# sandyresearch/chipmunk

Measured on AMD Instinct MI355X. Metric: DiT denoise steps/sec at fixed sparsity, higher is better.
Workload: dtype bf16

## Files before the change

### chipmunk_amd/_native.py

```python
from __future__ import annotations

import ctypes
import os

_HERE = os.path.dirname(os.path.abspath(__file__))
LIB_PATH = os.environ.get("CHIPMUNK_HIP_LIB") or os.path.join(_HERE, "lib", "libchipmunk_hip.so")

SYMBOLS = [
    "chipmunk_last_error", "chipmunk_abi_version", "chipmunk_set_option", "chipmunk_set_random_seed",
    "chipmunk_csp_attn", "chipmunk_csp_attn_out", "chipmunk_csp_128_attn", "chipmunk_dense_attn", "chipmunk_dense_colsum_attn",
    "chipmunk_csp_mlp_mm1", "chipmunk_csp_mlp_mm1_scatter", "chipmunk_csp_mlp_mm1_fp8", "chipmunk_csp_mlp_mm2_and_scatter_add", "chipmunk_csp_scatter_add", "chipmunk_csp_mlp_mm2",
    "chipmunk_csp_mlp_mm1_ragged", "chipmunk_csp_mlp_mm1_scatter_ragged", "chipmunk_csp_mlp_mm1_fp8_ragged", "chipmunk_csp_mlp_mm2_ragged",
    "chipmunk_csp_mlp_mm2_and_scatter_add_ragged", "chipmunk_csp_scatter_add_ragged", "chipmunk_block_mean_ragged", "chipmunk_transpose16_pitched",
    "chipmunk_csp_mlp_mm1_batched", "chipmunk_csp_mlp_mm1_scatter_batched", "chipmunk_csp_mlp_mm1_fp8_batched", "chipmunk_csp_mlp_mm2_batched",
    "chipmunk_csp_mlp_mm2_and_scatter_add_batched", "chipmunk_csp_scatter_add_batched",
    "chipmunk_topk_indices", "chipmunk_topk_delta_indices", "chipmunk_topk_mask", "chipmunk_mask_to_indices", "chipmunk_mask_to_sorted_indices", "chipmunk_packed_mask_to_indices", "chipmunk_mask_row_counts", "chipmunk_mask_to_ragged_indices", "chipmunk_copy_indices",
    "chipmunk_bitpack", "chipmunk_bitunpack", "chipmunk_transpose16", "chipmunk_block_mean", "chipmunk_quantize_fp8", "chipmunk_gather_rows", "chipmunk_qkv_split_norm", "chipmunk_split_heads_rownorm", "chipmunk_dense_colsum_topk_mask", "chipmunk_dense_attn_strided", "chipmunk_csp_attn_out_ragged", "chipmunk_compact_indices", "chipmunk_residual_ln_modulate", "chipmunk_dense_colsum_attn_strided", "chipmunk_dense_colsum_topk_mask_strided", "chipmunk_release_scratch", "chipmunk_big_scratch_fallbacks",
    "chipmunk_host_alloc", "chipmunk_host_free", "chipmunk_copy_d2h_async", "chipmunk_copy_h2d_async", "chipmunk_host_bytes",
]

_lib = None


def lib() -> ctypes.CDLL:
    global _lib
    if _lib is None:
        if not os.path.exists(LIB_PATH):
            raise ImportError(
                f"{LIB_PATH} is missing: build it with `python -m chipmunk_amd.build` (hipcc --offload-arch=gfx950). "
                "chipmunk_amd has no CPU fallback.")
        _lib = ctypes.CDLL(LIB_PATH)
        _lib.chipmunk_last_error.restype = ctypes.c_char_p
        _lib.chipmunk_abi_version.restype = ctypes.c_int
        for item in filter(None, os.environ.get("CHIPMUNK_AMD_OPTIONS", "").split(",")):
            name, _, val = item.partition("=")
            if _lib.chipmunk_set_option(name.strip().encode(), int(val)) != 0:
                raise ValueError(f"CHIPMUNK_AMD_OPTIONS: {_lib.chipmunk_last_error().decode()}")
    return _lib


def last_error() -> str:
    return lib().chipmunk_last_error().decode()


def check(rc: int, what: str) -> None:
    if rc != 0:
        raise RuntimeError(f"{what}: {last_error()}")


def set_option(name: str, value: int) -> None:
    check(lib().chipmunk_set_option(name.encode(), int(value)), "chipmunk_set_option")


def manual_seed(seed: int) -> None:
    check(lib().chipmunk_set_random_seed(ctypes.c_uint64(int(seed) & 0xFFFFFFFFFFFFFFFF)), "chipmunk_set_random_seed")


class HostBuffer:

    def __init__(self, numel: int, dtype) -> None:
        import torch
        self.dtype = dtype
        self._numel = int(numel)
        self._itemsize = torch.empty(0, dtype=dtype).element_size()
        self.nbytes = self._numel * self._itemsize
        p = ctypes.c_void_p()
        check(lib().chipmunk_host_alloc(ctypes.c_size_t(max(self.nbytes, 1)), ctypes.byref(p)), "chipmunk_host_alloc")
        self.ptr = p.value

    def numel(self) -> int:
        return self._numel

    def element_size(self) -> int:
        return self._itemsize

    def is_pinned(self) -> bool:
        return True

    def free(self) -> None:
        if getattr(self, "ptr", None):
            lib().chipmunk_host_free(ctypes.c_void_p(self.ptr))
            self.ptr = None

    def __del__(self):
        try:
            self.free()
        except Exception:
            pass


def copy_d2h_async(host_ptr: int, dev_ptr: int, nbytes: int, stream: int) -> None:
    check(lib().chipmunk_copy_d2h_async(ctypes.c_void_p(host_ptr), ctypes.c_void_p(dev_ptr), ctypes.c_size_t(nbytes), ctypes.c_void_p(stream)),
          "chipmunk_copy_d2h_async")


def copy_h2d_async(dev_ptr: int, host_ptr: int, nbytes: int, stream: int) -> None:
    check(lib().chipmunk_copy_h2d_async(ctypes.c_void_p(dev_ptr), ctypes.c_void_p(host_ptr), ctypes.c_size_t(nbytes), ctypes.c_void_p(stream)),
          "chipmunk_copy_h2d_async")


def host_bytes() -> int:
    f = lib().chipmunk_host_bytes
    f.restype = ctypes.c_size_t
    return int(f())
```

### chipmunk_amd/csrc/attn.hip

```cpp
#include "common.h"
#include "attn_params.h"
#include <type_traits>

namespace {

constexpr int QG = 192;
constexpr int QW = 48;
constexpr int KVT = 32;
constexpr int NST = 4;
constexpr int KRING = 8;
constexpr int HD = 128;
constexpr int TILE_BYTES = KVT * HD * 2;
constexpr float SCALE_LOG2E = 0.08838834764f * 1.44269504089f;
constexpr int NSTV = NST + 1;
constexpr int KEY_RING_OFF = (NST + NSTV) * TILE_BYTES;
constexpr int CS_OFF = KEY_RING_OFF + KRING * 256;
constexpr int ATTN_LDS_BYTES = CS_OFF + 2 * 2 * 4 * KVT * 4;

__device__ __forceinline__ f32x4 mfma16(bf16x8 a, bf16x8 b, f32x4 c) {
    return __builtin_amdgcn_mfma_f32_16x16x32_bf16(a, b, c, 0, 0, 0);
}

#ifdef ATTN_PROF
__device__ unsigned long long g_attn_prof[8 * 8];
// ... 1101 lines not shown
    contiguous_strides(p.qs, H, Nq), contiguous_strides(p.os, H, Nq);
    contiguous_strides(p.ks, H, Nk), contiguous_strides(p.vs, H, Nk);
    p.indices = indices, p.counts = counts;
    p.B = B, p.H = H, p.Nq = Nq, p.Nk = Nk, p.G = (Nq + QG - 1) / QG, p.idx_stride = idx_stride;
    p.o_scale = 1.f;
    return launch_attn<true, false, false>(p, (hipStream_t)stream);
}

static int output_strides(int64_t os[3], const int64_t *o_strides, int H, int Nq) {
    if (!o_strides) {
        contiguous_strides(os, H, Nq);
        return CHIPMUNK_OK;
    }
    for (int i = 0; i < 3; ++i) os[i] = o_strides[i];
    return check_strides(o_strides, "o");
}

extern "C" int chipmunk_dense_attn_strided(const void *q, const void *k, const void *v, const int64_t q_strides[3],
                                           const int64_t k_strides[3], const int64_t v_strides[3], void *o,
                                           const int64_t *o_strides, float *l, int B, int H, int Nq, int Nk, void *stream) {
    if (int e = check_common(q, k, v, o, B, H, Nq, Nk)) return e;
    CM_CHECK(l != nullptr, "dense_attn: l output missing");
    if (int e = check_strides(q_strides, "q")) return e;
    if (int e = check_strides(k_strides, "k")) return e;
    if (int e = check_strides(v_strides, "v")) return e;
    AttnParams p = {};
    p.q = (const uint16_t *)q, p.k = (const uint16_t *)k, p.v = (const uint16_t *)v, p.o = (uint16_t *)o;
    for (int i = 0; i < 3; ++i) p.qs[i] = q_strides[i], p.ks[i] = k_strides[i], p.vs[i] = v_strides[i];
    if (int e = output_strides(p.os, o_strides, H, Nq)) return e;
    p.l_out = l;
    p.B = B, p.H = H, p.Nq = Nq, p.Nk = Nk, p.G = (Nq + QG - 1) / QG;
    p.o_scale = 1.f;
    if (use_dense64(B, H, Nq, Nk)) {
        CM_CHECK((int64_t)Nk * p.ks[2] * 2 < (1ll << 32) && (int64_t)Nk * p.vs[2] * 2 < (1ll << 32),
                 "attention: one head's K or V spans more than 4 GiB (32-bit DMA offsets)");
        return chipmunk_dense64_launch(q, k, v, o, l, p.qs, p.ks, p.vs, p.os, B, H, Nq, Nk, (hipStream_t)stream);
    }
    return launch_attn<false, false, true>(p, (hipStream_t)stream);
}

extern "C" int chipmunk_dense_attn(const void *q, const void *k, const void *v, const int64_t q_strides[3],
                                   const int64_t k_strides[3], const int64_t v_strides[3], void *o, float *l, int B,
                                   int H, int Nq, int Nk, void *stream) {
    return chipmunk_dense_attn_strided(q, k, v, q_strides, k_strides, v_strides, o, nullptr, l, B, H, Nq, Nk, stream);
}

extern "C" int chipmunk_dense_colsum_attn_strided(const void *q, const void *k, const void *v, const int64_t q_strides[3],
                                                  const int64_t k_strides[3], const int64_t v_strides[3], const float *pin,
                                                  void *o, const int64_t *o_strides, void *cs, float *l, int B, int H, int Nq,
                                                  int Nk, int cs_stride, void *stream) {
    if (int e = check_common(q, k, v, o, B, H, Nq, Nk)) return e;
    CM_CHECK(l && cs && pin, "dense_colsum_attn: p / cs / l missing");
    CM_CHECK(cs_stride >= Nk, "dense_colsum_attn: cs row stride %d < Nk %d", cs_stride, Nk);
    if (int e = check_strides(q_strides, "q")) return e;
    if (int e = check_strides(k_strides, "k")) return e;
    if (int e = check_strides(v_strides, "v")) return e;
    AttnParams p = {};
    p.q = (const uint16_t *)q, p.k = (const uint16_t *)k, p.v = (const uint16_t *)v, p.o = (uint16_t *)o;
    for (int i = 0; i < 3; ++i) p.qs[i] = q_strides[i], p.ks[i] = k_strides[i], p.vs[i] = v_strides[i];
    if (int e = output_strides(p.os, o_strides, H, Nq)) return e;
    p.l_out = l, p.p_in = pin, p.cs = (uint16_t *)cs, p.cs_stride = cs_stride;
    p.B = B, p.H = H, p.Nq = Nq, p.Nk = Nk, p.G = (Nq + QG - 1) / QG;
    p.o_scale = 1.f;
    hipStream_t st = (hipStream_t)stream;
    int rc;
    if (chipmunk_get_option("attn_fused_colsum") == 5) {
        if (use_colsum64(B, H, Nq, Nk)) return chipmunk_colsum64_launch(p, st);
        return launch_attn<false, false, false, true>(p, st);
    }
    if (use_dense64(B, H, Nq, Nk)) {
        CM_CHECK((int64_t)Nk * p.ks[2] * 2 < (1ll << 32) && (int64_t)Nk * p.vs[2] * 2 < (1ll << 32),
                 "attention: one head's K or V spans more than 4 GiB (32-bit DMA offsets)");
        if (chipmunk_get_option("attn_fused_colsum") != 2) {
            int hc = H;
            uint16_t *part = nullptr;
            const int hc_min = chipmunk_get_option("attn_fused_colsum") == 4 ? 1 : 0;
            if (hc_min) hc = 1;
            for (; hc >= 1; hc /= 2) {
                part = (uint16_t *)chipmunk_big_scratch(st, chipmunk_colsum_part_bytes(hc == H ? B : 1, hc, Nq, Nk));
                if (part) break;
            }
            if (part && hc == H) return chipmunk_dense64_colsum_launch(p, part, st);
            if (part) {
                for (int b = 0; b < B; ++b)
                    for (int h0 = 0; h0 < H; h0 += hc) {
                        AttnParams c = p;
                        const int hn = H - h0 < hc ? H - h0 : hc;
                        const int64_t bh0 = (int64_t)b * H + h0;
                        c.q += b * p.qs[0] + h0 * p.qs[1], c.k += b * p.ks[0] + h0 * p.ks[1], c.v += b * p.vs[0] + h0 * p.vs[1];
                        c.o += b * p.os[0] + h0 * p.os[1];
                        c.l_out += bh0 * Nq, c.p_in += bh0 * Nq, c.cs += bh0 * p.G * (int64_t)cs_stride;
                        c.B = 1, c.H = hn;
                        if (int e = chipmunk_dense64_colsum_launch(c, part, st)) return e;
                    }
                return CHIPMUNK_OK;
            }
        }
        rc = chipmunk_dense64_launch(q, k, v, o, l, p.qs, p.ks, p.vs, p.os, B, H, Nq, Nk, st);
    } else {
        rc = launch_attn<false, false, true>(p, st);
    }
    if (rc != CHIPMUNK_OK) return rc;
    if (use_colsum64(B, H, Nq, Nk)) return chipmunk_colsum64_launch(p, st);
    return launch_attn<false, false, false, true>(p, st);
}

extern "C" int chipmunk_dense_colsum_attn(const void *q, const void *k, const void *v, const int64_t q_strides[3],
                                          const int64_t k_strides[3], const int64_t v_strides[3], const float *pin,
                                          void *o, void *cs, float *l, int B, int H, int Nq, int Nk, int cs_stride,
                                          void *stream) {
    return chipmunk_dense_colsum_attn_strided(q, k, v, q_strides, k_strides, v_strides, pin, o, nullptr, cs, l, B, H, Nq, Nk,
                                              cs_stride, stream);
}

extern "C" int chipmunk_dense_colsum_topk_mask_strided(const void *q, const void *k, const void *v, const int64_t q_strides[3],
                                               const int64_t k_strides[3], const int64_t v_strides[3], const float *pin, void *o,
                                               const int64_t *o_strides, float *l, int B, int H, int Nq, int Nk, const void *static_mask,
                                               int64_t static_stride, int static_rows, const void *group_flags, void *mask,
                                               int topk, double random_amount, void *stream) {
    if (int e = check_common(q, k, v, o, B, H, Nq, Nk)) return e;
    CM_CHECK(l && pin && mask, "dense_colsum_topk_mask: p / l / mask missing");
    if (int e = check_strides(q_strides, "q")) return e;
    if (int e = check_strides(k_strides, "k")) return e;
    if (int e = check_strides(v_strides, "v")) return e;
    hipStream_t st = (hipStream_t)stream;
    if (!use_dense64(B, H, Nq, Nk) || chipmunk_get_option("attn_fused_colsum") == 2 || (Nk & 3) || Nk > CHIPMUNK_TOPK_MASK_MAX_N)
        return CHIPMUNK_ERR_UNSUPPORTED;
    AttnParams p = {};
    p.q = (const uint16_t *)q, p.k = (const uint16_t *)k, p.v = (const uint16_t *)v, p.o = (uint16_t *)o;
    for (int i = 0; i < 3; ++i) p.qs[i] = q_strides[i], p.ks[i] = k_strides[i], p.vs[i] = v_strides[i];
    CM_CHECK((int64_t)Nk * p.ks[2] * 2 < (1ll << 32) && (int64_t)Nk * p.vs[2] * 2 < (1ll << 32),
             "attention: one head's K or V spans more than 4 GiB (32-bit DMA offsets)");
    if (int e = output_strides(p.os, o_strides, H, Nq)) return e;
    p.l_out = l, p.p_in = pin, p.cs = nullptr, p.cs_stride = 0;
    p.B = B, p.H = H, p.Nq = Nq, p.Nk = Nk, p.G = (Nq + QG - 1) / QG;
    p.o_scale = 1.f;
    uint16_t *part = (uint16_t *)chipmunk_big_scratch(st, chipmunk_colsum_part_bytes(B, H, Nq, Nk));
    if (!part) return CHIPMUNK_ERR_UNSUPPORTED;
    if (int e = chipmunk_dense64_colsum_launch(p, part, st)) return e;
    const int nrb = ((Nq + 255) / 256) * 2;
    return chipmunk_topk_mask_parts(part, chipmunk_colsum_part_stride(Nk), nrb, p.G, Nq, static_mask, static_stride, static_rows, group_flags, mask, B * H * p.G, Nk,
                                    topk, random_amount, st);
}

extern "C" int chipmunk_dense_colsum_topk_mask(const void *q, const void *k, const void *v, const int64_t q_strides[3],
                                               const int64_t k_strides[3], const int64_t v_strides[3], const float *pin, void *o,
                                               float *l, int B, int H, int Nq, int Nk, const void *static_mask,
                                               int64_t static_stride, int static_rows, const void *group_flags, void *mask,
                                               int topk, double random_amount, void *stream) {
    return chipmunk_dense_colsum_topk_mask_strided(q, k, v, q_strides, k_strides, v_strides, pin, o, nullptr, l, B, H, Nq, Nk,
                                                   static_mask, static_stride, static_rows, group_flags, mask, topk, random_amount,
                                                   stream);
}
```

### chipmunk_amd/csrc/attn_params.h

```cpp
#pragma once
#include <stdint.h>
#include <hip/hip_runtime.h>

struct AttnParams {
    const uint16_t *q, *k, *v;
    uint16_t *o;
    const uint16_t *o_in;
    int64_t qs[3], ks[3], vs[3], os[3];
    const int32_t *indices, *counts;
    const int64_t *idx_off;
    float *l_out;
    const float *p_in;
    uint16_t *cs;
    int cs_stride;
    int B, H, Nq, Nk, G, idx_stride;
    float o_scale;
    int split_full, nsplit;
    float *ws;
    int32_t *tickets;
    const int32_t *plan;
    int xcd_chunks;
    const float *kmax;
    uint16_t *cs_part;
    int cs_pstride;
    int probe;
};


int chipmunk_csp64_launch(const AttnParams &p, int inplace, int grid, hipStream_t stream);
int chipmunk_dense64_colsum_launch(const AttnParams &p, uint16_t *part, hipStream_t stream);
int chipmunk_topk_mask_parts(const uint16_t *part, int part_stride, int nrb, int groups_per_bh, int Nq, const void *static_mask, int64_t static_stride,
                             int static_rows, const void *group_flags, void *mask, int rows, int n, int k, double random_amount,
                             hipStream_t stream);
size_t chipmunk_colsum_part_bytes(int B, int H, int Nq, int Nk);
int chipmunk_colsum_part_stride(int Nk);
int chipmunk_colsum64_launch(const AttnParams &p, hipStream_t stream);
int chipmunk_csp96_launch(const AttnParams &p, int inplace, int grid, hipStream_t stream);
const float *chipmunk_knorm_max(const uint16_t *k, const int64_t ks[3], int B, int H, int Nk, hipStream_t stream);

__host__ __device__ inline int colsum_part_rows(int j, int nwg, int &r0, int &r1) {
    const int a = (3 * j) >> 2, w0 = 3 * j - 4 * a;
    r0 = 2 * a + (w0 ? 1 : 0);
    r1 = 2 * (a + 1);
    return (w0 >= 2 && a + 1 < nwg) ? 2 : 1;
}

struct IndexRow {
    const int32_t *ptr;
    int width;
};
__device__ __forceinline__ IndexRow index_row(const AttnParams &p, int64_t item) {
    if (p.idx_off) {
        const int64_t o = p.idx_off[item];
        return {p.indices + o, (int)(p.idx_off[item + 1] - o)};
    }
    return {p.indices + item * p.idx_stride, p.idx_stride};
}
```

### chipmunk_amd/csrc/indexed_io.hip

```cpp
#include "common.h"
#include "attn_params.h"

namespace {

__device__ __forceinline__ uint32_t wave_incl_scan(uint32_t x) {
    x += (uint32_t)__builtin_amdgcn_update_dpp(0, (int)x, 0x111, 0xf, 0xf, true);
    x += (uint32_t)__builtin_amdgcn_update_dpp(0, (int)x, 0x112, 0xf, 0xf, true);
    x += (uint32_t)__builtin_amdgcn_update_dpp(0, (int)x, 0x114, 0xf, 0xf, true);
    x += (uint32_t)__builtin_amdgcn_update_dpp(0, (int)x, 0x118, 0xf, 0xf, true);
    x += (uint32_t)__builtin_amdgcn_update_dpp(0, (int)x, 0x142, 0xa, 0xf, false);
    x += (uint32_t)__builtin_amdgcn_update_dpp(0, (int)x, 0x143, 0xc, 0xf, false);
    return x;
}
struct M2IParams {
    const uint8_t *mask;
    int32_t *indices;
    int32_t *counts;
    int n, pad_n, multiple_of;
    const int64_t *offsets;
};

template <bool PACKED, bool SORTED = false, bool RAGGED = false>
__global__ __launch_bounds__(256) void mask_to_indices_kernel(const M2IParams p) {
    extern __shared__ __attribute__((aligned(16))) unsigned char smem[];
// ... 385 lines not shown
        base += tot[256];
        __syncthreads();
    }
    const int kept = base;
    const int mod = kept % p.multiple_of;
    const int pad = mod == 0 ? 0 : p.multiple_of - mod;
    if (tid == 0) p.counts[row] = kept + pad;
    if (pad > 0) {
        int pbase = 0;
        const int slot = compact_slot(my_last_invalid != -1, lane, w, wave_tot, pbase);
        if (slot >= 0 && slot < pad) {
            out[kept + slot] = my_last_invalid;
            if constexpr (DELTA) xc[my_last_invalid] = x[my_last_invalid];
        }
    }
}

template <typename T>
__global__ __launch_bounds__(256) void copy_indices_kernel(const T *src, T *dst, const int32_t *inds,
                                                           const int32_t *counts, int M, int R, int F) {
    const int64_t grow = blockIdx.x;
    const int64_t b = grow / ((int64_t)M * R);
    const int base_m = (int)((grow % ((int64_t)M * R)) / R);
    const int cnt = counts[b * M + base_m];
    const int32_t *ii = inds + (b * M + base_m) * (int64_t)F;
    for (int c = threadIdx.x; c < cnt; c += 256) {
        const int col = ii[c];
        dst[grow * F + col] = src[grow * F + col];
    }
}

__global__ __launch_bounds__(256) void bitpack_kernel(const uint8_t *mask, uint8_t *packed, int64_t n) {
    const int64_t nb = (n + 7) >> 3;
    for (int64_t i = (int64_t)blockIdx.x * 256 + threadIdx.x; i < nb; i += (int64_t)gridDim.x * 256) {
        uint8_t byte = 0;
        if (i * 8 + 8 <= n && ((((uintptr_t)mask) & 7) == 0)) {
            unsigned long long v = *(const unsigned long long *)(mask + i * 8);
#pragma unroll
            for (int j = 0; j < 8; ++j) byte |= (uint8_t)((((v >> (8 * j)) & 0xffull) != 0) << j);
        } else {
            for (int j = 0; j < 8 && i * 8 + j < n; ++j) byte |= (uint8_t)((mask[i * 8 + j] != 0) << j);
        }
        packed[i] = byte;
    }
}
__global__ __launch_bounds__(256) void bitunpack_kernel(const uint8_t *packed, uint8_t *mask, int64_t n) {
    const int64_t nb = (n + 7) >> 3;
    for (int64_t i = (int64_t)blockIdx.x * 256 + threadIdx.x; i < nb; i += (int64_t)gridDim.x * 256) {
        const uint8_t byte = packed[i];
        if (i * 8 + 8 <= n && ((((uintptr_t)mask) & 7) == 0)) {
            unsigned long long v = 0;
#pragma unroll
            for (int j = 0; j < 8; ++j) v |= (unsigned long long)((byte >> j) & 1u) << (8 * j);
            *(unsigned long long *)(mask + i * 8) = v;
        } else {
            for (int j = 0; j < 8 && i * 8 + j < n; ++j) mask[i * 8 + j] = (byte >> j) & 1u;
        }
    }
}

__global__ __launch_bounds__(256) void transpose16_kernel(const uint16_t *src, uint16_t *dst, int R, int C, int ld) {
    __shared__ __attribute__((aligned(16))) uint16_t tile[64][72];
    const int64_t boff = (int64_t)blockIdx.z * R * C;
    const int r0 = blockIdx.y * 64, c0 = blockIdx.x * 64;
    const int tid = threadIdx.x;
#pragma unroll
    for (int i = 0; i < 2; ++i) {
        const int item = i * 256 + tid, r = item >> 3, ch = item & 7;
        u32x4 v = {0u, 0u, 0u, 0u};
        if (r0 + r < R && c0 + ch * 8 + 8 <= C) v = *(const u32x4 *)(src + boff + (int64_t)(r0 + r) * C + c0 + ch * 8);
        else if (r0 + r < R)
            for (int e = 0; e < 8; ++e)
                if (c0 + ch * 8 + e < C) {
                    const uint32_t x = src[boff + (int64_t)(r0 + r) * C + c0 + ch * 8 + e];
                    v[e >> 1] |= x << (16 * (e & 1));
                }
#pragma unroll
        for (int e = 0; e < 4; ++e) {
            tile[ch * 8 + 2 * e][r] = (uint16_t)(v[e] & 0xffffu);
            tile[ch * 8 + 2 * e + 1][r] = (uint16_t)(v[e] >> 16);
        }
    }
    __syncthreads();
#pragma unroll
    for (int i = 0; i < 2; ++i) {
        const int item = i * 256 + tid, c = item >> 3, ch = item & 7;
        if (c0 + c >= C) continue;
        uint16_t *d = dst + (int64_t)blockIdx.z * C * ld + (int64_t)(c0 + c) * ld + r0 + ch * 8;
        if (r0 + ch * 8 + 8 <= ld && ((ld & 7) == 0)) *(u32x4 *)d = *(const u32x4 *)&tile[c][ch * 8];
        else
            for (int e = 0; e < 8; ++e)
                if (r0 + ch * 8 + e < ld) d[e] = tile[c][ch * 8 + e];
    }
}

__global__ __launch_bounds__(256) void compact_indices_kernel(const int32_t *indices, int64_t idx_stride, const int32_t *counts,
                                                             const int64_t *offsets, int32_t *flat) {
    const int64_t r = blockIdx.x;
    const int32_t *src = indices + r * idx_stride;
    const int64_t o = offsets[r];
    int32_t *dst = flat + o;
    const int width = (int)(offsets[r + 1] - o);
    int c = counts[r];
    c = c < 0 ? 0 : (c < width ? c : width);
    c = c < idx_stride ? c : (int)idx_stride;
    if ((((uintptr_t)src | (uintptr_t)dst) & 15) == 0) {
        const int c4 = c >> 2;
        for (int i = threadIdx.x; i < c4; i += 256) ((u32x4 *)dst)[i] = ((const u32x4 *)src)[i];
        for (int i = (c4 << 2) + threadIdx.x; i < c; i += 256) dst[i] = src[i];
    } else {
        for (int i = threadIdx.x; i < c; i += 256) dst[i] = src[i];
    }
    for (int i = c + threadIdx.x; i < width; i += 256) dst[i] = 0;
}

size_t m2i_lds_bytes(int n, bool sorted) {
    const int NI = (n + 31) >> 5, NB = (NI + 63) >> 6;
    if (sorted) return (size_t)NB * 64 * 4 + (size_t)(NB + 1) * 4 + 16;
    return (size_t)NB * 64 * 4 + (size_t)32 * NB * 8 + (size_t)32 * NB * 4 + 33 * 4 + 16;
}

template <bool PACKED, bool SORTED = false, bool RAGGED = false>
int launch_m2i(const void *mask, int32_t *indices, int32_t *counts, int64_t rows, int n, int pad_n, int multiple_of,
               void *stream, const int64_t *offsets = nullptr) {
    CM_CHECK(mask && indices && (RAGGED ? (const void *)offsets : (const void *)counts), "mask_to_indices: null pointer");
    CM_CHECK(rows >= 0 && n > 0 && pad_n >= n && multiple_of > 0, "mask_to_indices: bad sizes rows=%lld n=%d pad_n=%d multiple_of=%d",
             (long long)rows, n, pad_n, multiple_of);
    CM_CHECK(rows < (1ll << 31), "mask_to_indices: too many rows");
    if (PACKED) CM_CHECK(n % 8 == 0, "packed_mask_to_indices: n must be a multiple of 8 (got %d)", n);
    const size_t lds = m2i_lds_bytes(n, SORTED);
    CM_CHECK(lds <= 160 * 1024, "mask_to_indices: row length %d needs %zu B of LDS (> 160 KiB)", n, lds);
    if (rows == 0) return CHIPMUNK_OK;
    auto kern = mask_to_indices_kernel<PACKED, SORTED, RAGGED>;
    if (lds > 64 * 1024) (void)hipFuncSetAttribute((const void *)kern, hipFuncAttributeMaxDynamicSharedMemorySize, (int)lds);
    M2IParams p = {(const uint8_t *)mask, indices, counts, n, pad_n, multiple_of, offsets};
    hipLaunchKernelGGL(kern, dim3((unsigned)rows), dim3(256), lds, (hipStream_t)stream, p);
    CM_LAUNCH_CHECK();
    return CHIPMUNK_OK;
}


struct TopkMaskParams {
    const uint16_t *cs;
    const uint8_t *stat;
    const uint8_t *groups;
    uint8_t *mask;
    int64_t cs_stride, stat_stride;
    int rows, n, k, stat_rows;
    float random_amount;
    uint32_t salt;
    const uint16_t *parts;
    int64_t pstride;
    int nrb, ngroups, nq;
};

__device__ __forceinline__ uint32_t bf16_key(uint32_t u) {
    return (u & 0x8000u) ? (~u & 0xffffu) : (u | 0x8000u);
}

template <int KPT, bool ALIGNED, bool PARTS = false>
__global__ __launch_bounds__(1024) void topk_mask_kernel(const TopkMaskParams p) {
    constexpr int NV = KPT / 4;
    __shared__ int wave_cnt[16];
    const int tid = threadIdx.x, lane = tid & 63, w = tid >> 6;
    const int row = blockIdx.x;
    const int n = p.n;
    const uint16_t *x = nullptr;
    int prow = 1;
    int64_t row1 = 0;
    if constexpr (PARTS) {
        const int bh = row / p.ngroups, g = row - bh * p.ngroups;
        int r0, r1;
        prow = colsum_part_rows(g, p.nrb / 2, r0, r1);
        x = p.parts + ((int64_t)bh * p.nrb + r0) * p.pstride;
        row1 = (int64_t)(r1 - r0) * p.pstride;
    } else {
        x = p.cs + (int64_t)row * p.cs_stride;
    }
    const uint32_t lane_off8 = 8u * (uint32_t)tid;
    const uint32_t lane_off4 = 4u * (uint32_t)tid;
    uint32_t key[NV][2];
    constexpr int LB = NV % 10 == 0 ? 10 : (NV % 8 == 0 ? 8 : (NV % 6 == 0 ? 6 : 4));
    static_assert(NV % LB == 0, "NV must split into whole load batches");
#pragma unroll
    for (int j0 = 0; j0 < NV; j0 += LB) {
        uint32_t raw[LB][2];
#pragma unroll
        for (int jj = 0; jj < LB; ++jj) {
            const int c = 4 * tid + 4096 * (j0 + jj);
            uint32_t v0 = 0xffffffffu, v1 = 0xffffffffu;
            if constexpr (ALIGNED) {
                if (c < n) {
                    const u32x2 v = *(const u32x2 *)((const unsigned char *)(x + 4096 * (j0 + jj)) + lane_off8);
                    v0 = v[0], v1 = v[1];
                    if constexpr (PARTS) {
                        if (prow == 2) {
                            float a0 = __uint_as_float(v0 << 16), a1 = __uint_as_float(v0 & 0xffff0000u);
                            float a2 = __uint_as_float(v1 << 16), a3 = __uint_as_float(v1 & 0xffff0000u);
                            const u32x2 y = *(const u32x2 *)((const unsigned char *)(x + row1 + 4096 * (j0 + jj)) + lane_off8);
                            a0 += __uint_as_float(y[0] << 16), a1 += __uint_as_float(y[0] & 0xffff0000u);
                            a2 += __uint_as_float(y[1] << 16), a3 += __uint_as_float(y[1] & 0xffff0000u);
                            v0 = pack_bf16x2(a0, a1), v1 = pack_bf16x2(a2, a3);
                        }
                    }
                }
            } else if (c < n) {
                v0 = v1 = 0;
#pragma unroll
                for (int e = 0; e < 4; ++e) {
                    const uint32_t u = c + e < n ? x[c + e] : 0xffffu;
                    if (e < 2) v0 |= u << (16 * e);
                    else v1 |= u << (16 * (e - 2));
                }
            }
            raw[jj][0] = v0, raw[jj][1] = v1;
        }
#pragma unroll
        for (int jj = 0; jj < LB; ++jj) {
            key[j0 + jj][0] = bf16_key(raw[jj][0] & 0xffffu) | (bf16_key(raw[jj][0] >> 16) << 16);
            key[j0 + jj][1] = bf16_key(raw[jj][1] & 0xffffu) | (bf16_key(raw[jj][1] >> 16) << 16);
        }
        __builtin_amdgcn_sched_barrier(0);
    }
    auto block_count = [&](int mine) {
#pragma unroll
        for (int d = 32; d > 0; d >>= 1) mine += __shfl_xor(mine, d);
        if (lane == 0) wave_cnt[w] = mine;
        __syncthreads();
        int t = 0;
#pragma unroll
        for (int i = 0; i < 16; ++i) t += wave_cnt[i];
        __syncthreads();
        return t;
    };
    const bool active = p.groups == nullptr || p.groups[row] != 0;
    const int k = p.k < n ? p.k : n;
    uint32_t thr = 0x10000u;
    int ties_to_take = 0;
    if (active && k > 0) {
        uint32_t res = 0;
        for (int bit = 15; bit >= 0; --bit) {
            const uint32_t cand = res | (1u << bit);
            const uint32_t cm1 = (cand - 1u) | ((cand - 1u) << 16);
            const uint32_t one2 = 0x00010001u;
            uint32_t cnt2 = 0;
#pragma unroll
            for (int j = 0; j < NV; ++j)
#pragma unroll
                for (int h = 0; h < 2; ++h) {
                    uint32_t d;
                    asm volatile("v_pk_sub_u16 %0, %1, %2 clamp\n\tv_pk_min_u16 %0, %0, %3" : "=&v"(d) : "v"(key[j][h]), "v"(cm1), "v"(one2));
                    asm volatile("v_pk_add_u16 %0, %0, %1" : "+v"(cnt2) : "v"(d));
                }
            const int mine = (int)(cnt2 & 0xffffu) + (int)(cnt2 >> 16);
            if (block_count(mine) >= k) res = cand;
        }
        thr = res;
        int gt = 0;
#pragma unroll
        for (int j = 0; j < NV; ++j)
#pragma unroll
            for (int h = 0; h < 2; ++h) {
                uint32_t kw = key[j][h];
                asm volatile("" : "+v"(kw));
                gt += ((kw & 0xffffu) > thr ? 1 : 0) + ((kw >> 16) > thr ? 1 : 0);
            }
        ties_to_take = k - block_count(gt);
    }
    int my_ties = 0;
    if (ties_to_take > 0) {
#pragma unroll
        for (int j = 0; j < NV; ++j)
#pragma unroll
            for (int h = 0; h < 2; ++h) {
                uint32_t kw = key[j][h];
                asm volatile("" : "+v"(kw));
                my_ties += ((kw & 0xffffu) == thr ? 1 : 0) + ((kw >> 16) == thr ? 1 : 0);
            }
    }
    int tie_budget = 0;
    {
        int incl = my_ties;
#pragma unroll
        for (int d = 1; d < 64; d <<= 1) {
            const int o = __shfl_up(incl, d);
            if (lane >= d) incl += o;
        }
        if (lane == 63) wave_cnt[w] = incl;
        __syncthreads();
        int before = incl - my_ties;
#pragma unroll
        for (int i = 0; i < 16; ++i) before += i < w ? wave_cnt[i] : 0;
        __syncthreads();
        tie_budget = ties_to_take - before;
    }
    uint8_t *out = p.mask + (int64_t)row * n;
    const uint8_t *st = p.stat ? p.stat + (int64_t)(row % p.stat_rows) * p.stat_stride : nullptr;
    const bool rnd = active && p.random_amount > 0.f;
    auto combined4 = [&](int c0, uint32_t &v0, uint32_t &v1) {
        const u32x2 v = *(const u32x2 *)(x + c0);
        v0 = v[0], v1 = v[1];
        if constexpr (PARTS) {
            float a0 = __uint_as_float(v0 << 16), a1 = __uint_as_float(v0 & 0xffff0000u);
            float a2 = __uint_as_float(v1 << 16), a3 = __uint_as_float(v1 & 0xffff0000u);
            if (prow == 2) {
                const u32x2 y = *(const u32x2 *)(x + row1 + c0);
                a0 += __uint_as_float(y[0] << 16), a1 += __uint_as_float(y[0] & 0xffff0000u);
                a2 += __uint_as_float(y[1] << 16), a3 += __uint_as_float(y[1] & 0xffff0000u);
            }
            v0 = pack_bf16x2(a0, a1), v1 = pack_bf16x2(a2, a3);
        }
    };
    uint32_t first = x[0];
    if constexpr (PARTS) {
        uint32_t f0, f1;
        combined4(0, f0, f1);
        first = f0 & 0xffffu;
    }
    const uint32_t salt = p.salt ^ (first * 0x27D4EB2Fu);
    const int nsteps = (n + 4095) / 4096;
    auto emit = [&](auto keyed, int c, uint32_t v0, uint32_t v1, uint32_t sb) {
        uint32_t bytes = 0;
        if constexpr (decltype(keyed)::value) asm volatile("" : "+v"(v0), "+v"(v1));
#pragma unroll
        for (int e = 0; e < 4; ++e) {
            const uint32_t half = ((e < 2 ? v0 : v1) >> (16 * (e & 1))) & 0xffffu;
            const uint32_t kv = decltype(keyed)::value ? half : bf16_key(half);
            bool keep = kv > thr;
            const bool tie = kv == thr && tie_budget > 0 && c + e < n;
            tie_budget -= tie ? 1 : 0;
            keep = keep || tie;
            if (rnd && !keep) keep = hash_uniform(row, c + e, salt) < p.random_amount;
            keep = keep || ((sb >> (8 * e)) & 0xffu) != 0;
            bytes |= (keep ? 1u : 0u) << (8 * e);
        }
        if constexpr (ALIGNED) {
            *(uint32_t *)(out + c) = bytes;
        } else {
#pragma unroll
            for (int e = 0; e < 4; ++e)
                if (c + e < n) out[c + e] = (uint8_t)(bytes >> (8 * e));
        }
    };
    if constexpr (ALIGNED) {
        constexpr int OB = 5;
#pragma unroll
        for (int j0 = 0; j0 < NV; j0 += OB) {
            uint32_t sbv[OB];
#pragma unroll
            for (int jj = 0; jj < OB; ++jj) {
                const int c = 4 * tid + 4096 * (j0 + jj);
                sbv[jj] = (j0 + jj < NV && st && c < n) ? *(const uint32_t *)(st + c) : 0u;
            }
            __builtin_amdgcn_sched_barrier(0);
#pragma unroll
            for (int jj = 0; jj < OB; ++jj) {
                if constexpr (true) {
                    const int c = 4 * tid + 4096 * (j0 + jj);
                    if (j0 + jj < NV && c < n) emit(std::integral_constant<int, 1>{}, c, key[(j0 + jj) < NV ? (j0 + jj) : 0][0], key[(j0 + jj) < NV ? (j0 + jj) : 0][1], sbv[jj]);
                    asm volatile("" ::: "memory");
                }
            }
            __builtin_amdgcn_sched_barrier(0);
        }
    } else {
        for (int j = 0; j < nsteps; ++j) {
            const int c = 4 * tid + 4096 * j;
            if (c >= n) break;
            uint32_t v0 = 0, v1 = 0, sb = 0;
#pragma unroll
            for (int e = 0; e < 4; ++e) {
                const uint32_t u = c + e < n ? x[c + e] : 0xffffu;
                if (e < 2) v0 |= u << (16 * e);
                else v1 |= u << (16 * (e - 2));
                if (st && c + e < n) sb |= (uint32_t)st[c + e] << (8 * e);
            }
            emit(std::integral_constant<int, 0>{}, c, v0, v1, sb);
        }
    }
}

__device__ __forceinline__ uint32_t bf16_key2(uint32_t u) {
    uint32_t s;
    const uint32_t fifteen2 = 0x000f000fu;
    asm("v_pk_ashrrev_i16 %0, %1, %2" : "=v"(s) : "v"(fifteen2), "v"(u));
    return u ^ (s | 0x80008000u);
}

template <bool ALIGNED, bool PARTS>
__global__ __launch_bounds__(1024) void topk_mask_stream_kernel(const TopkMaskParams p) {
    __shared__ int wave_cnt[16];
    const int tid = threadIdx.x, lane = tid & 63, w = tid >> 6;
    const int row = blockIdx.x;
    const int n = p.n;
    const uint16_t *x = nullptr;
    int prow = 1;
    int64_t row1 = 0;
    if constexpr (PARTS) {
        const int bh = row / p.ngroups, g = row - bh * p.ngroups;
        int r0, r1;
        prow = colsum_part_rows(g, p.nrb / 2, r0, r1);
        x = p.parts + ((int64_t)bh * p.nrb + r0) * p.pstride;
        row1 = (int64_t)(r1 - r0) * p.pstride;
    } else {
        x = p.cs + (int64_t)row * p.cs_stride;
    }
    const uint32_t lane_off8 = 8u * (uint32_t)tid;
    const int nsteps = (n + 4095) / 4096;
    const bool active = p.groups == nullptr || p.groups[row] != 0;
    const int k = p.k < n ? p.k : n;
    const bool select = active && k > 0;
    const bool rnd = active && p.random_amount > 0.f;

    auto combined4 = [&](int c0, uint32_t &v0, uint32_t &v1) {
        const u32x2 v = *(const u32x2 *)(x + c0);
        v0 = v[0], v1 = v[1];
        if constexpr (PARTS) {
            if (prow == 2) {
                float a0 = __uint_as_float(v0 << 16), a1 = __uint_as_float(v0 & 0xffff0000u);
                float a2 = __uint_as_float(v1 << 16), a3 = __uint_as_float(v1 & 0xffff0000u);
                const u32x2 y = *(const u32x2 *)(x + row1 + c0);
                a0 += __uint_as_float(y[0] << 16), a1 += __uint_as_float(y[0] & 0xffff0000u);
                a2 += __uint_as_float(y[1] << 16), a3 += __uint_as_float(y[1] & 0xffff0000u);
                v0 = pack_bf16x2(a0, a1), v1 = pack_bf16x2(a2, a3);
            }
        }
    };
    uint32_t first = 0;
    if (rnd) {
        first = x[0];
        if constexpr (PARTS) {
            uint32_t f0, f1;
            combined4(0, f0, f1);
            first = f0 & 0xffffu;
        }
    }
    const uint32_t salt = p.salt ^ (first * 0x27D4EB2Fu);
    if constexpr (PARTS) {
        __syncthreads();
        if (select) {
            uint16_t *xk = const_cast<uint16_t *>(x);
            for (int j = 0; j < nsteps; ++j) {
                const int c = 4 * tid + 4096 * j;
                if (c < n) {
                    uint32_t v0, v1;
                    combined4(c, v0, v1);
                    u32x2 kk = {bf16_key2(v0), bf16_key2(v1)};
                    *(u32x2 *)(xk + c) = kk;
                }
            }
        }
        __syncthreads();
    }
    auto load_raw = [&](int j, uint32_t &v0, uint32_t &v1) {
        const int c = 4 * tid + 4096 * j;
        if constexpr (ALIGNED) {
            v0 = v1 = PARTS ? 0u : 0xffffffffu;
            if (c < n) {
                const u32x2 v = *(const u32x2 *)((const unsigned char *)(x + 4096 * j) + lane_off8);
                v0 = v[0], v1 = v[1];
            }
        } else {
            v0 = v1 = 0xffffffffu;
            if (c < n) {
                v0 = v1 = 0;
#pragma unroll
                for (int e = 0; e < 4; ++e) {
                    const uint32_t u = c + e < n ? x[c + e] : 0xffffu;
                    if (e < 2) v0 |= u << (16 * e);
                    else v1 |= u << (16 * (e - 2));
                }
            }
        }
    };
    auto to_keys = [&](uint32_t &v0, uint32_t &v1) {
        if constexpr (!PARTS) v0 = bf16_key2(v0), v1 = bf16_key2(v1);
    };
    auto block_count = [&](int mine) {
#pragma unroll
        for (int d = 32; d > 0; d >>= 1) mine += __shfl_xor(mine, d);
        if (lane == 0) wave_cnt[w] = mine;
        __syncthreads();
        int t = 0;
#pragma unroll
        for (int i = 0; i < 16; ++i) t += wave_cnt[i];
        __syncthreads();
        return t;
    };
    constexpr int U = ALIGNED ? 8 : 2;
    uint32_t thr = 0x10000u;
    int ties_to_take = 0, my_ties = 0;
    if (select) {
        uint32_t res = 0;
        for (int bit = 15; bit >= 0; --bit) {
            const uint32_t cand = res | (1u << bit);
            const uint32_t cm1 = (cand - 1u) | ((cand - 1u) << 16);
            const uint32_t one2 = 0x00010001u;
            uint32_t cnt2 = 0;
            for (int j0 = 0; j0 < nsteps; j0 += U) {
                uint32_t kw[U][2];
#pragma unroll
                for (int jj = 0; jj < U; ++jj) load_raw(j0 + jj, kw[jj][0], kw[jj][1]);
#pragma unroll
                for (int jj = 0; jj < U; ++jj) {
                    to_keys(kw[jj][0], kw[jj][1]);
#pragma unroll
                    for (int h = 0; h < 2; ++h) {
                        uint32_t d;
                        asm volatile("v_pk_sub_u16 %0, %1, %2 clamp\n\tv_pk_min_u16 %0, %0, %3" : "=&v"(d) : "v"(kw[jj][h]), "v"(cm1), "v"(one2));
                        asm volatile("v_pk_add_u16 %0, %0, %1" : "+v"(cnt2) : "v"(d));
                    }
                }
            }
            const int mine = (int)(cnt2 & 0xffffu) + (int)(cnt2 >> 16);
            if (block_count(mine) >= k) res = cand;
        }
        thr = res;
        int gt = 0;
        for (int j0 = 0; j0 < nsteps; j0 += U) {
            uint32_t kw[U][2];
#pragma unroll
            for (int jj = 0; jj < U; ++jj) load_raw(j0 + jj, kw[jj][0], kw[jj][1]);
#pragma unroll
            for (int jj = 0; jj < U; ++jj) {
                to_keys(kw[jj][0], kw[jj][1]);
#pragma unroll
                for (int h = 0; h < 2; ++h) {
                    const uint32_t lo = kw[jj][h] & 0xffffu, hi = kw[jj][h] >> 16;
                    gt += (lo > thr ? 1 : 0) + (hi > thr ? 1 : 0);
                    my_ties += (lo == thr ? 1 : 0) + (hi == thr ? 1 : 0);
                }
            }
        }
        ties_to_take = k - block_count(gt);
    }
    int tie_budget = 0;
    {
        int incl = my_ties;
#pragma unroll
        for (int d = 1; d < 64; d <<= 1) {
            const int o = __shfl_up(incl, d);
            if (lane >= d) incl += o;
        }
        if (lane == 63) wave_cnt[w] = incl;
        __syncthreads();
        int before = incl - my_ties;
#pragma unroll
        for (int i = 0; i < 16; ++i) before += i < w ? wave_cnt[i] : 0;
        __syncthreads();
        tie_budget = ties_to_take - before;
    }
    uint8_t *out = p.mask + (int64_t)row * n;
    const uint8_t *st = p.stat ? p.stat + (int64_t)(row % p.stat_rows) * p.stat_stride : nullptr;
    for (int j0 = 0; j0 < nsteps; j0 += U) {
        uint32_t kw[U][2], sbv[U];
#pragma unroll
        for (int jj = 0; jj < U; ++jj) {
            const int c = 4 * tid + 4096 * (j0 + jj);
            kw[jj][0] = kw[jj][1] = 0;
            if (select) load_raw(j0 + jj, kw[jj][0], kw[jj][1]);
            sbv[jj] = 0;
            if constexpr (ALIGNED) {
                if (st && c < n) sbv[jj] = *(const uint32_t *)(st + c);
            } else if (st) {
#pragma unroll
                for (int e = 0; e < 4; ++e)
                    if (c + e < n) sbv[jj] |= (uint32_t)st[c + e] << (8 * e);
            }
        }
#pragma unroll
        for (int jj = 0; jj < U; ++jj) {
            const int c = 4 * tid + 4096 * (j0 + jj);
            if (c >= n) continue;
            if (select) to_keys(kw[jj][0], kw[jj][1]);
            uint32_t bytes = 0;
#pragma unroll
            for (int e = 0; e < 4; ++e) {
                const uint32_t kv = (kw[jj][e >> 1] >> (16 * (e & 1))) & 0xffffu;
                bool keep = kv > thr;
                const bool tie = kv == thr && tie_budget > 0 && c + e < n;
                tie_budget -= tie ? 1 : 0;
                keep = keep || tie;
                if (rnd && !keep) keep = hash_uniform(row, c + e, salt) < p.random_amount;
                keep = keep || ((sbv[jj] >> (8 * e)) & 0xffu) != 0;
                bytes |= (keep ? 1u : 0u) << (8 * e);
            }
            if constexpr (ALIGNED) {
                *(uint32_t *)(out + c) = bytes;
            } else {
#pragma unroll
                for (int e = 0; e < 4; ++e)
                    if (c + e < n) out[c + e] = (uint8_t)(bytes >> (8 * e));
            }
        }
    }
}

}

extern "C" int chipmunk_mask_to_indices(const void *mask, int32_t *indices, int32_t *counts, int64_t rows, int n,
                                        int pad_n, int multiple_of, void *stream) {
    return launch_m2i<false>(mask, indices, counts, rows, n, pad_n, multiple_of, stream);
}

extern "C" int chipmunk_packed_mask_to_indices(const void *packed, int32_t *indices, int32_t *counts, int64_t rows,
                                               int n, int pad_n, int multiple_of, void *stream) {
    return launch_m2i<true>(packed, indices, counts, rows, n, pad_n, multiple_of, stream);
}

static int launch_topk(const void *activation, void *cache, int dtype, int32_t *indices, int32_t *counts, int rows,
                       int cols, double sparsity_amount, int multiple_of, double random_amount, void *stream) {
    CM_CHECK(activation && indices && counts, "topk_indices: null pointer");
    CM_CHECK(rows >= 0 && cols >= 1024, "topk_indices: rows >= 0 and cols >= 1024 required (the quantile is taken over the first 1024 columns); got rows=%d cols=%d", rows, cols);
    CM_CHECK(multiple_of > 0, "topk_indices: multiple_of must be positive");
    CM_CHECK(sparsity_amount >= 0.0 && sparsity_amount <= 1.0, "topk_indices: sparsity_amount must be in [0,1]");
    if (rows == 0) return CHIPMUNK_OK;
    TopkParams p = {activation, cache, indices, counts, rows, cols, multiple_of, (float)sparsity_amount, (float)random_amount,
                    random_amount > 0.0 ? chipmunk_next_random_salt() : 0u};
    hipStream_t s = (hipStream_t)stream;
#define LAUNCH_TOPK(T)                                                                                           \
    do {                                                                                                         \
        if (cache) hipLaunchKernelGGL((topk_indices_kernel<T, true>), dim3(rows), dim3(1024), 0, s, p);          \
        else hipLaunchKernelGGL((topk_indices_kernel<T, false>), dim3(rows), dim3(1024), 0, s, p);               \
    } while (0)
    switch (dtype) {
        case CHIPMUNK_DTYPE_BF16: LAUNCH_TOPK(uint16_t); break;
        case CHIPMUNK_DTYPE_FP16: LAUNCH_TOPK(_Float16); break;
        case CHIPMUNK_DTYPE_FP32: LAUNCH_TOPK(float); break;
        default: CM_CHECK(false, "topk_indices: unsupported dtype code %d", dtype);
    }
#undef LAUNCH_TOPK
    CM_LAUNCH_CHECK();
    return CHIPMUNK_OK;
}

extern "C" int chipmunk_mask_to_sorted_indices(const void *mask, int packed, int32_t *indices, int32_t *counts,
                                               int64_t rows, int n, int pad_n, int multiple_of, void *stream) {
    return packed ? launch_m2i<true, true>(mask, indices, counts, rows, n, pad_n, multiple_of, stream)
                  : launch_m2i<false, true>(mask, indices, counts, rows, n, pad_n, multiple_of, stream);
}

extern "C" int chipmunk_mask_row_counts(const void *mask, int packed, int32_t *counts, int64_t *lengths, int64_t rows, int n,
                                        int pad_n, int multiple_of, void *stream) {
    CM_CHECK(mask && counts && lengths, "mask_row_counts: null pointer");
    CM_CHECK(rows >= 0 && n > 0 && pad_n >= n && multiple_of > 0, "mask_row_counts: bad sizes rows=%lld n=%d pad_n=%d multiple_of=%d",
             (long long)rows, n, pad_n, multiple_of);
    CM_CHECK(rows < (1ll << 31), "mask_row_counts: too many rows");
    CM_CHECK(!packed || n % 8 == 0, "mask_row_counts: n must be a multiple of 8 for a packed mask (got %d)", n);
    const size_t lds = m2i_lds_bytes(n, true);
    CM_CHECK(lds <= 160 * 1024, "mask_to_indices: row length %d needs %zu B of LDS (> 160 KiB)", n, lds);
    if (rows == 0) return CHIPMUNK_OK;
    RowCountParams p = {(const uint8_t *)mask, counts, lengths, rows, n, pad_n, multiple_of};
    const dim3 grid((unsigned)((rows + 3) / 4));
    if (packed) hipLaunchKernelGGL(mask_row_counts_kernel<true>, grid, dim3(256), 0, (hipStream_t)stream, p);
    else hipLaunchKernelGGL(mask_row_counts_kernel<false>, grid, dim3(256), 0, (hipStream_t)stream, p);
    CM_LAUNCH_CHECK();
    return CHIPMUNK_OK;
}

extern "C" int chipmunk_mask_to_ragged_indices(const void *mask, int packed, int sorted, const int64_t *offsets, int32_t *flat,
                                               int64_t rows, int n, int multiple_of, void *stream) {
    if (packed) return sorted ? launch_m2i<true, true, true>(mask, flat, nullptr, rows, n, n, multiple_of, stream, offsets)
                              : launch_m2i<true, false, true>(mask, flat, nullptr, rows, n, n, multiple_of, stream, offsets);
    return sorted ? launch_m2i<false, true, true>(mask, flat, nullptr, rows, n, n, multiple_of, stream, offsets)
                  : launch_m2i<false, false, true>(mask, flat, nullptr, rows, n, n, multiple_of, stream, offsets);
}

extern "C" int chipmunk_topk_indices(const void *activation, int dtype, int32_t *indices, int32_t *counts, int rows,
                                     int cols, double sparsity_amount, int multiple_of, double random_amount,
                                     void *stream) {
    return launch_topk(activation, nullptr, dtype, indices, counts, rows, cols, sparsity_amount, multiple_of,
                       random_amount, stream);
}

extern "C" int chipmunk_topk_delta_indices(const void *activation, void *cache, int dtype, int32_t *indices,
                                           int32_t *counts, int rows, int cols, double sparsity_amount,
                                           int multiple_of, double random_amount, void *stream) {
    CM_CHECK(cache != nullptr, "topk_delta_indices: cache missing");
    return launch_topk(activation, cache, dtype, indices, counts, rows, cols, sparsity_amount, multiple_of,
                       random_amount, stream);
}

extern "C" int chipmunk_copy_indices(const void *src, void *dst, const int32_t *inds, const int32_t *counts, int B,
                                     int M, int R, int F, int elem_size, void *stream) {
    CM_CHECK(src && dst && inds && counts, "copy_indices: null pointer");
    CM_CHECK(B >= 0 && M > 0 && R > 0 && F > 0, "copy_indices: bad sizes");
    CM_CHECK(elem_size == 2 || elem_size == 4, "copy_indices: element size must be 2 or 4 bytes (got %d)", elem_size);
    const int64_t rows = (int64_t)B * M * R;
    if (rows == 0) return CHIPMUNK_OK;
    CM_CHECK(rows < (1ll << 31), "copy_indices: too many rows");
    hipStream_t s = (hipStream_t)stream;
    if (elem_size == 2)
        hipLaunchKernelGGL(copy_indices_kernel<uint16_t>, dim3((unsigned)rows), dim3(256), 0, s, (const uint16_t *)src,
                           (uint16_t *)dst, inds, counts, M, R, F);
    else
        hipLaunchKernelGGL(copy_indices_kernel<uint32_t>, dim3((unsigned)rows), dim3(256), 0, s, (const uint32_t *)src,
                           (uint32_t *)dst, inds, counts, M, R, F);
    CM_LAUNCH_CHECK();
    return CHIPMUNK_OK;
}

extern "C" int chipmunk_bitpack(const void *mask, void *packed, int64_t n, void *stream) {
    CM_CHECK(mask && packed && n >= 0, "bitpack: bad arguments");
    if (n == 0) return CHIPMUNK_OK;
    const int64_t nb = (n + 7) >> 3;
    const unsigned grid = (unsigned)((nb + 255) / 256 < 8192 ? (nb + 255) / 256 : 8192);
    hipLaunchKernelGGL(bitpack_kernel, dim3(grid), dim3(256), 0, (hipStream_t)stream, (const uint8_t *)mask,
                       (uint8_t *)packed, n);
    CM_LAUNCH_CHECK();
    return CHIPMUNK_OK;
}

extern "C" int chipmunk_bitunpack(const void *packed, void *mask, int64_t n, void *stream) {
    CM_CHECK(mask && packed && n >= 0, "bitunpack: bad arguments");
    if (n == 0) return CHIPMUNK_OK;
    const int64_t nb = (n + 7) >> 3;
    const unsigned grid = (unsigned)((nb + 255) / 256 < 8192 ? (nb + 255) / 256 : 8192);
    hipLaunchKernelGGL(bitunpack_kernel, dim3(grid), dim3(256), 0, (hipStream_t)stream, (const uint8_t *)packed,
                       (uint8_t *)mask, n);
    CM_LAUNCH_CHECK();
    return CHIPMUNK_OK;
}

extern "C" int chipmunk_transpose16(const void *src, void *dst, int B, int R, int C, void *stream) {
    CM_CHECK(src && dst && B > 0 && R > 0 && C > 0, "transpose16: bad arguments");
    CM_CHECK((C & 7) == 0 || true, "unreachable");
    hipLaunchKernelGGL(transpose16_kernel, dim3((C + 63) / 64, (R + 63) / 64, B), dim3(256), 0, (hipStream_t)stream,
                       (const uint16_t *)src, (uint16_t *)dst, R, C, R);
    CM_LAUNCH_CHECK();
    return CHIPMUNK_OK;
}

extern "C" int chipmunk_transpose16_pitched(const void *src, void *dst, int B, int R, int C, int ld, void *stream) {
    CM_CHECK(src && dst && B > 0 && R > 0 && C > 0, "transpose16: bad arguments");
    CM_CHECK(ld >= R, "transpose16: the output pitch ld (%d) must be at least R (%d)", ld, R);
    hipLaunchKernelGGL(transpose16_kernel, dim3((C + 63) / 64, (ld + 63) / 64, B), dim3(256), 0, (hipStream_t)stream,
                       (const uint16_t *)src, (uint16_t *)dst, R, C, ld);
    CM_LAUNCH_CHECK();
    return CHIPMUNK_OK;
}

template <typename V>
__global__ __launch_bounds__(256) void gather_rows_kernel(const V *src, V *dst, const int32_t *map, int64_t n_out,
                                                          int64_t n_src, int64_t cpr, int64_t total) {
    for (int64_t idx = (int64_t)blockIdx.x * 256 + threadIdx.x; idx < total; idx += (int64_t)gridDim.x * 256) {
        const int64_t row = idx / cpr, c = idx - row * cpr;
        const int64_t o = row / n_out, r = row - o * n_out;
        dst[idx] = src[(o * n_src + map[r]) * cpr + c];
    }
}

extern "C" int chipmunk_gather_rows(const void *src, void *dst, const int32_t *map, int64_t outer, int64_t n_src,
                                    int64_t n_out, int64_t row_bytes, void *stream) {
    CM_CHECK(src && dst && map, "gather_rows: null pointer");
    CM_CHECK(outer >= 0 && n_src > 0 && n_out >= 0 && row_bytes > 0, "gather_rows: bad sizes");
    if (outer == 0 || n_out == 0) return CHIPMUNK_OK;
    hipStream_t s = (hipStream_t)stream;
    const uintptr_t align = (uintptr_t)src | (uintptr_t)dst | (uintptr_t)row_bytes;
#define LAUNCH_GATHER(V)                                                                                              \
    do {                                                                                                              \
        const int64_t cpr = row_bytes / (int64_t)sizeof(V), total = outer * n_out * cpr;                               \
        const int64_t blocks = (total + 255) / 256;                                                                    \
        hipLaunchKernelGGL((gather_rows_kernel<V>), dim3((unsigned)(blocks > 65536 * 16 ? 65536 * 16 : blocks)),       \
                           dim3(256), 0, s, (const V *)src, (V *)dst, map, n_out, n_src, cpr, total);                  \
    } while (0)
    if ((align & 15) == 0) LAUNCH_GATHER(u32x4);
    else if ((align & 3) == 0) LAUNCH_GATHER(uint32_t);
    else if ((align & 1) == 0) LAUNCH_GATHER(uint16_t);
    else LAUNCH_GATHER(uint8_t);
#undef LAUNCH_GATHER
    CM_LAUNCH_CHECK();
    return CHIPMUNK_OK;
}

int chipmunk_topk_mask_parts(const uint16_t *part, int part_stride, int nrb, int groups_per_bh, int Nq, const void *static_mask, int64_t static_stride,
                             int static_rows, const void *group_flags, void *mask, int rows, int n, int k, double random_amount,
                             hipStream_t s) {
    CM_CHECK(part && mask && rows >= 0 && n > 0 && (n & 3) == 0 && n <= CHIPMUNK_TOPK_MASK_MAX_N && k >= 0 && part_stride >= n && (part_stride & 3) == 0, "topk_mask_parts: bad arguments");
    CM_CHECK(!static_mask || (static_rows > 0 && static_stride >= n && (static_stride & 3) == 0 && ((uintptr_t)static_mask & 3) == 0),
             "topk_mask_parts: bad static mask geometry");
    CM_CHECK(((uintptr_t)mask & 3) == 0 && ((uintptr_t)part & 7) == 0, "topk_mask_parts: unaligned buffers");
    if (rows == 0) return CHIPMUNK_OK;
    TopkMaskParams p = {nullptr, (const uint8_t *)static_mask, (const uint8_t *)group_flags, (uint8_t *)mask, 0, static_stride,
                        rows, n, k, static_mask ? static_rows : 1, (float)random_amount,
                        random_amount > 0.0 ? chipmunk_next_random_salt() : 0u};
    p.parts = part, p.pstride = part_stride, p.nrb = nrb, p.ngroups = groups_per_bh, p.nq = Nq;
    if (n > 1024 * 120 || chipmunk_get_option("topk_mask_stream") == 1) hipLaunchKernelGGL((topk_mask_stream_kernel<true, true>), dim3(rows), dim3(1024), 0, s, p);
    else if (n <= 1024 * 16) hipLaunchKernelGGL((topk_mask_kernel<16, true, true>), dim3(rows), dim3(1024), 0, s, p);
    else if (n <= 1024 * 48) hipLaunchKernelGGL((topk_mask_kernel<48, true, true>), dim3(rows), dim3(1024), 0, s, p);
    else hipLaunchKernelGGL((topk_mask_kernel<120, true, true>), dim3(rows), dim3(1024), 0, s, p);
    CM_LAUNCH_CHECK();
    return CHIPMUNK_OK;
}

__global__ __launch_bounds__(256) void qkv_split_norm_kernel(const uint16_t *qkv, int64_t row_stride, const uint16_t *qw,
                                                             const uint16_t *kw, uint16_t *q, uint16_t *k, uint16_t *v, int64_t n,
                                                             int H, float eps, int64_t segments, const float *fcos, const float *fsin,
                                                             int64_t rope_rows) {
    const int l15 = threadIdx.x & 15;
    u32x4 wq = {0x3f803f80u, 0x3f803f80u, 0x3f803f80u, 0x3f803f80u}, wk = wq;
    if (qw) wq = *(const u32x4 *)(qw + l15 * 8);
    if (kw) wk = *(const u32x4 *)(kw + l15 * 8);
    for (int64_t seg = ((int64_t)blockIdx.x * 256 + threadIdx.x) >> 4; seg < segments; seg += ((int64_t)gridDim.x * 256) >> 4) {
        const int64_t tok = seg / (3 * H);
        const int rem = (int)(seg - tok * 3 * H), which = rem / H, h = rem - which * H;
        u32x4 x = *(const u32x4 *)(qkv + tok * row_stride + (int64_t)rem * 128 + l15 * 8);
        uint16_t *dst = (which == 0 ? q : which == 1 ? k : v) + ((int64_t)h * n + tok) * 128 + l15 * 8;
        if (which < 2) {
            float f[8], ss = 0.f;
#pragma unroll
            for (int e = 0; e < 4; ++e) {
                f[2 * e] = __uint_as_float(x[e] << 16), f[2 * e + 1] = __uint_as_float(x[e] & 0xffff0000u);
                ss = __builtin_fmaf(f[2 * e], f[2 * e], ss);
                ss = __builtin_fmaf(f[2 * e + 1], f[2 * e + 1], ss);
            }
            ss = row16_sum(ss);
            const float r = 1.0f / __builtin_sqrtf(ss * (1.0f / 128.0f) + eps);
            const u32x4 w = which == 0 ? wq : wk;
#pragma unroll
            for (int e = 0; e < 4; ++e) {
                float a = f[2 * e] * r, b = f[2 * e + 1] * r;
                round_bf16_pair(a, b);
                x[e] = pack_bf16x2(a * __uint_as_float(w[e] << 16), b * __uint_as_float(w[e] & 0xffff0000u));
            }
            if (fcos && tok < rope_rows) {
                const f32x4 c0 = *(const f32x4 *)(fcos + tok * 128 + l15 * 8), c1 = *(const f32x4 *)(fcos + tok * 128 + l15 * 8 + 4);
                const f32x4 s0 = *(const f32x4 *)(fsin + tok * 128 + l15 * 8), s1 = *(const f32x4 *)(fsin + tok * 128 + l15 * 8 + 4);
#pragma unroll
                for (int e = 0; e < 4; ++e) {
                    const float re = __uint_as_float(x[e] << 16), im = __uint_as_float(x[e] & 0xffff0000u);
                    const float cr = e < 2 ? c0[2 * e] : c1[2 * e - 4], ci = e < 2 ? c0[2 * e + 1] : c1[2 * e - 3];
                    const float sr = e < 2 ? s0[2 * e] : s1[2 * e - 4], si = e < 2 ? s0[2 * e + 1] : s1[2 * e - 3];
                    x[e] = pack_bf16x2(re * cr + (-im) * sr, im * ci + re * si);
                }
            }
        }
        *(u32x4 *)dst = x;
    }
}

extern "C" int chipmunk_qkv_split_norm(const void *qkv, int64_t row_stride, const void *q_weight, const void *k_weight, void *q,
                                       void *k, void *v, int64_t n, int heads, float eps, const float *freqs_cos,
                                       const float *freqs_sin, int64_t rope_rows, void *stream) {
    CM_CHECK(qkv && q && k && v, "qkv_split_norm: null pointer");
    CM_CHECK(n >= 0 && heads > 0 && row_stride >= (int64_t)3 * heads * 128, "qkv_split_norm: bad sizes");
    CM_CHECK((((uintptr_t)qkv | (uintptr_t)q | (uintptr_t)k | (uintptr_t)v | (uintptr_t)q_weight | (uintptr_t)k_weight) & 15) == 0 &&
                 (row_stride & 7) == 0 && (((uintptr_t)freqs_cos | (uintptr_t)freqs_sin) & 15) == 0,
             "qkv_split_norm: pointers and the row stride must be 16-byte aligned");
    CM_CHECK((freqs_cos == nullptr) == (freqs_sin == nullptr) && rope_rows >= 0 && rope_rows <= n, "qkv_split_norm: bad rotary arguments");
    if (n == 0) return CHIPMUNK_OK;
    const int64_t segments = n * 3 * heads, blocks = (segments + 15) / 16;
    hipLaunchKernelGGL(qkv_split_norm_kernel, dim3((unsigned)(blocks > 256 * 64 ? 256 * 64 : blocks)), dim3(256), 0, (hipStream_t)stream,
                       (const uint16_t *)qkv, row_stride, (const uint16_t *)q_weight, (const uint16_t *)k_weight, (uint16_t *)q,
                       (uint16_t *)k, (uint16_t *)v, n, heads, eps, segments, freqs_cos, freqs_sin, freqs_cos ? rope_rows : 0);
    CM_LAUNCH_CHECK();
    return CHIPMUNK_OK;
}

extern "C" int chipmunk_topk_mask(const void *cs, int64_t cs_stride, const void *static_mask, int64_t static_stride,
                                  int static_rows, const void *group_flags, void *mask, int rows, int n, int k,
                                  double random_amount, void *stream) {
    CM_CHECK(cs && mask, "topk_mask: null pointer");
    CM_CHECK(rows >= 0 && n > 0 && k >= 0, "topk_mask: bad sizes (rows=%d n=%d k=%d)", rows, n, k);
    CM_CHECK(cs_stride >= n, "topk_mask: cs row stride %lld < n %d", (long long)cs_stride, n);
    CM_CHECK(n <= CHIPMUNK_TOPK_MASK_MAX_N, "topk_mask: rows of more than %d columns are not supported (got %d)", CHIPMUNK_TOPK_MASK_MAX_N, n);
    CM_CHECK(!static_mask || (static_rows > 0 && static_stride >= n), "topk_mask: bad static mask geometry");
    CM_CHECK(random_amount >= 0.0 && random_amount <= 1.0, "topk_mask: random_amount must be in [0,1]");
    if (rows == 0) return CHIPMUNK_OK;
    TopkMaskParams p = {(const uint16_t *)cs, (const uint8_t *)static_mask, (const uint8_t *)group_flags, (uint8_t *)mask,
                        cs_stride, static_stride, rows, n, k, static_mask ? static_rows : 1, (float)random_amount,
                        random_amount > 0.0 ? chipmunk_next_random_salt() : 0u};
    hipStream_t s = (hipStream_t)stream;
    const bool aligned = n % 4 == 0 && (((uintptr_t)cs) & 7) == 0 && (cs_stride * 2) % 8 == 0 && (((uintptr_t)mask) & 3) == 0 &&
                         (!static_mask || ((((uintptr_t)static_mask) & 3) == 0 && static_stride % 4 == 0));
#define LAUNCH_TM(KPT)                                                                                       \
    do {                                                                                                     \
        if (aligned) hipLaunchKernelGGL((topk_mask_kernel<KPT, true>), dim3(rows), dim3(1024), 0, s, p);     \
        else hipLaunchKernelGGL((topk_mask_kernel<KPT, false>), dim3(rows), dim3(1024), 0, s, p);            \
    } while (0)
    if (n > 1024 * 120 || chipmunk_get_option("topk_mask_stream") == 1) {
        if (aligned) hipLaunchKernelGGL((topk_mask_stream_kernel<true, false>), dim3(rows), dim3(1024), 0, s, p);
        else hipLaunchKernelGGL((topk_mask_stream_kernel<false, false>), dim3(rows), dim3(1024), 0, s, p);
    } else if (n <= 1024 * 16) LAUNCH_TM(16);
    else if (n <= 1024 * 48) LAUNCH_TM(48);
    else LAUNCH_TM(120);
#undef LAUNCH_TM
    CM_LAUNCH_CHECK();
    return CHIPMUNK_OK;
}

extern "C" int chipmunk_compact_indices(const int32_t *indices, int64_t idx_stride, const int32_t *counts, const int64_t *offsets,
                                        int32_t *flat, int64_t rows, void *stream) {
    CM_CHECK(indices && counts && offsets && flat, "compact_indices: null pointer");
    CM_CHECK(rows >= 0 && rows < (1ll << 31) && idx_stride > 0, "compact_indices: bad sizes rows=%lld idx_stride=%lld", (long long)rows,
             (long long)idx_stride);
    if (rows == 0) return CHIPMUNK_OK;
    hipLaunchKernelGGL(compact_indices_kernel, dim3((unsigned)rows), dim3(256), 0, (hipStream_t)stream, indices, idx_stride, counts,
                       offsets, flat);
    CM_LAUNCH_CHECK();
    return CHIPMUNK_OK;
}
```

### chipmunk_amd/csrc/torch_registry.cpp

```cpp
#include <ATen/ATen.h>
#include <ATen/hip/impl/HIPStreamMasqueradingAsCUDA.h>
#include <Python.h>
#include <c10/core/DeviceGuard.h>
#include <torch/library.h>

#include <vector>

#include "../../include/chipmunk_hip.h"

extern "C" {
PyObject *PyInit_cuda(void) {
    static struct PyModuleDef module_def = {PyModuleDef_HEAD_INIT, "cuda", NULL, -1, NULL};
    return PyModule_Create(&module_def);
}
}

namespace chipmunk {
namespace {

void *cur_stream(const at::Tensor &t) {
    return (void *)c10::hip::getCurrentHIPStreamMasqueradingAsCUDA(t.device().index()).stream();
}
void check(int rc, const char *op) { TORCH_CHECK(rc == 0, "chipmunk::", op, ": ", chipmunk_last_error()); }

// ... 490 lines not shown
    TORCH_CHECK(indices.sizes() == activation.sizes(), "indices must have the shape of activation");
    TORCH_CHECK(counts.numel() == activation.size(0) * activation.size(1), "counts must be [batch, rows]");
    int dtype;
    switch (activation.scalar_type()) {
        case at::kBFloat16: dtype = CHIPMUNK_DTYPE_BF16; break;
        case at::kHalf: dtype = CHIPMUNK_DTYPE_FP16; break;
        case at::kFloat: dtype = CHIPMUNK_DTYPE_FP32; break;
        default: TORCH_CHECK(false, "Unsupported dtype for topk_indices");
    }
    c10::DeviceGuard guard(activation.device());
    check(chipmunk_topk_indices(activation.data_ptr(), dtype, indices.data_ptr<int>(), counts.data_ptr<int>(),
                                (int)(activation.size(0) * activation.size(1)), (int)activation.size(2),
                                sparsity_amount, (int)multiple_of, random_amount, cur_stream(activation)),
          "topk_indices");
}

void topk_delta_indices(at::Tensor activation, at::Tensor cache, at::Tensor indices, at::Tensor counts,
                        double sparsity_amount, int64_t multiple_of, double random_amount) {
    CHECK_DEV(activation); CHECK_DEV(cache); CHECK_DEV(indices); CHECK_DEV(counts);
    CHECK_CONTIG(activation); CHECK_CONTIG(cache); CHECK_CONTIG(indices); CHECK_CONTIG(counts);
    TORCH_CHECK(activation.dim() == 3 && cache.sizes() == activation.sizes(), "activation and cache must be [batch, rows, cols]");
    TORCH_CHECK(cache.scalar_type() == activation.scalar_type(), "activation and cache must have the same dtype");
    CHECK_I32(indices); CHECK_I32(counts);
    TORCH_CHECK(indices.sizes() == activation.sizes(), "indices must have the shape of activation");
    TORCH_CHECK(counts.numel() == activation.size(0) * activation.size(1), "counts must be [batch, rows]");
    int dtype;
    switch (activation.scalar_type()) {
        case at::kBFloat16: dtype = CHIPMUNK_DTYPE_BF16; break;
        case at::kHalf: dtype = CHIPMUNK_DTYPE_FP16; break;
        case at::kFloat: dtype = CHIPMUNK_DTYPE_FP32; break;
        default: TORCH_CHECK(false, "Unsupported dtype for topk_delta_indices");
    }
    c10::DeviceGuard guard(activation.device());
    check(chipmunk_topk_delta_indices(activation.data_ptr(), cache.data_ptr(), dtype, indices.data_ptr<int>(),
                                      counts.data_ptr<int>(), (int)(activation.size(0) * activation.size(1)),
                                      (int)activation.size(2), sparsity_amount, (int)multiple_of, random_amount,
                                      cur_stream(activation)),
          "topk_delta_indices");
}

std::vector<at::Tensor> mask_to_indices(at::Tensor mask, int64_t multiple_of, int64_t pad_to_multiple_of) {
    TORCH_CHECK(mask.dim() == 4, "mask must be 4-dimensional [b, h, m, n]");
    TORCH_CHECK(mask.scalar_type() == at::kBool, "mask must be bool type");
    CHECK_DEV(mask);
    TORCH_CHECK(multiple_of > 0 && pad_to_multiple_of > 0, "multiple_of and pad_to_multiple_of must be positive");
    mask = mask.contiguous();
    const int64_t b = mask.size(0), h = mask.size(1), m = mask.size(2), n = mask.size(3);
    const int64_t pad_n = ((n + pad_to_multiple_of - 1) / pad_to_multiple_of) * pad_to_multiple_of;
    c10::DeviceGuard guard(mask.device());
    at::Tensor indices = at::empty({b, h, m, pad_n}, mask.options().dtype(at::kInt));
    at::Tensor counts = at::empty({b, h, m}, mask.options().dtype(at::kInt));
    check(chipmunk_mask_to_indices(mask.data_ptr(), indices.data_ptr<int>(), counts.data_ptr<int>(), b * h * m, (int)n,
                                   (int)pad_n, (int)multiple_of, cur_stream(mask)),
          "mask_to_indices");
    return {indices, counts};
}

std::vector<at::Tensor> packed_mask_to_indices(at::Tensor packed, at::IntArrayRef shape, int64_t multiple_of,
                                               int64_t pad_to_multiple_of) {
    TORCH_CHECK(packed.scalar_type() == at::kByte && packed.is_contiguous(), "packed must be a contiguous uint8 tensor");
    CHECK_DEV(packed);
    TORCH_CHECK(shape.size() == 4, "shape must be [b, h, m, n]");
    const int64_t b = shape[0], h = shape[1], m = shape[2], n = shape[3];
    TORCH_CHECK(n % 8 == 0, "n must be a multiple of 8");
    TORCH_CHECK(packed.numel() * 8 >= b * h * m * n, "packed is too short for the given shape");
    const int64_t pad_n = ((n + pad_to_multiple_of - 1) / pad_to_multiple_of) * pad_to_multiple_of;
    c10::DeviceGuard guard(packed.device());
    at::Tensor indices = at::empty({b, h, m, pad_n}, packed.options().dtype(at::kInt));
    at::Tensor counts = at::empty({b, h, m}, packed.options().dtype(at::kInt));
    check(chipmunk_packed_mask_to_indices(packed.data_ptr(), indices.data_ptr<int>(), counts.data_ptr<int>(),
                                          b * h * m, (int)n, (int)pad_n, (int)multiple_of, cur_stream(packed)),
          "packed_mask_to_indices");
    return {indices, counts};
}

at::Tensor transpose_last2(at::Tensor x) {
    CHECK_DEV(x);
    TORCH_CHECK(x.dim() >= 2 && x.element_size() == 2, "transpose_last2: need a >=2-D tensor of a 16-bit dtype");
    x = x.contiguous();
    const int64_t R = x.size(-2), C = x.size(-1), B = x.numel() / (R * C);
    auto sizes = x.sizes().vec();
    std::swap(sizes[sizes.size() - 1], sizes[sizes.size() - 2]);
    c10::DeviceGuard guard(x.device());
    at::Tensor out = at::empty(sizes, x.options());
    check(chipmunk_transpose16(x.data_ptr(), out.data_ptr(), (int)B, (int)R, (int)C, cur_stream(x)), "transpose_last2");
    return out;
}

at::Tensor transpose_last2_pitched(at::Tensor x, int64_t ld) {
    CHECK_DEV(x);
    TORCH_CHECK(x.dim() >= 2 && x.element_size() == 2, "transpose_last2_pitched: need a >=2-D tensor of a 16-bit dtype");
    x = x.contiguous();
    const int64_t R = x.size(-2), C = x.size(-1), B = x.numel() / (R * C);
    TORCH_CHECK(ld >= R, "transpose_last2_pitched: ld must be at least the row count");
    auto sizes = x.sizes().vec();
    sizes[sizes.size() - 2] = C;
    sizes[sizes.size() - 1] = ld;
    c10::DeviceGuard guard(x.device());
    at::Tensor out = at::empty(sizes, x.options());
    check(chipmunk_transpose16_pitched(x.data_ptr(), out.data_ptr(), (int)B, (int)R, (int)C, (int)ld, cur_stream(x)), "transpose_last2_pitched");
    return out;
}

at::Tensor block_mean(at::Tensor x, int64_t mbm) {
    CHECK_DEV(x);
    TORCH_CHECK(x.dim() == 3 && x.scalar_type() == at::kBFloat16, "block_mean: need a [b, n, c] bfloat16 tensor");
    TORCH_CHECK(mbm > 0 && x.size(1) > 0, "block_mean: mbm and n must be positive");
    x = x.contiguous();
    c10::DeviceGuard guard(x.device());
    const int64_t n = x.size(1), blocks = (n + mbm - 1) / mbm;
    at::Tensor out = at::empty({x.size(0), blocks, x.size(2)}, x.options());
    if (n % mbm == 0) {
        check(chipmunk_block_mean(x.data_ptr(), out.data_ptr(), x.size(0) * n, (int)x.size(2), (int)mbm, cur_stream(x)), "block_mean");
    } else {
        for (int64_t b = 0; b < x.size(0); ++b)
            check(chipmunk_block_mean_ragged(x[b].data_ptr(), out[b].data_ptr(), n, (int)x.size(2), (int)mbm, cur_stream(x)), "block_mean");
    }
    return out;
}

at::Tensor quantize_fp8(at::Tensor x, at::Tensor scale, double max_value) {
    CHECK_DEV(x); CHECK_DEV(scale);
    TORCH_CHECK(x.scalar_type() == at::kBFloat16, "quantize_fp8: x must be bfloat16");
    TORCH_CHECK(scale.scalar_type() == at::kFloat && scale.numel() == 1, "quantize_fp8: scale must be a one-element float32 tensor");
    TORCH_CHECK(x.numel() % 8 == 0, "quantize_fp8: the element count must be a multiple of 8");
    x = x.contiguous();
    c10::DeviceGuard guard(x.device());
    at::Tensor out = at::empty(x.sizes(), x.options().dtype(at::kFloat8_e4m3fn));
    check(chipmunk_quantize_fp8(x.data_ptr(), scale.data_ptr<float>(), out.data_ptr(), x.numel(), (float)max_value, cur_stream(x)), "quantize_fp8");
    return out;
}

std::vector<at::Tensor> mask_to_sorted_indices(at::Tensor mask, at::IntArrayRef shape, int64_t multiple_of,
                                               int64_t pad_to_multiple_of) {
    CHECK_DEV(mask);
    const bool packed = mask.scalar_type() == at::kByte;
    TORCH_CHECK(packed || mask.scalar_type() == at::kBool, "mask must be bool, or uint8 bit-packed with a shape");
    mask = mask.contiguous();
    std::vector<int64_t> shp = packed ? shape.vec() : mask.sizes().vec();
    TORCH_CHECK(shp.size() == 4, "shape must be [b, h, m, n]");
    const int64_t b = shp[0], h = shp[1], m = shp[2], n = shp[3];
    if (packed) TORCH_CHECK(n % 8 == 0 && mask.numel() * 8 >= b * h * m * n, "bad packed mask");
    const int64_t pad_n = ((n + pad_to_multiple_of - 1) / pad_to_multiple_of) * pad_to_multiple_of;
    c10::DeviceGuard guard(mask.device());
    at::Tensor indices = at::empty({b, h, m, pad_n}, mask.options().dtype(at::kInt));
    at::Tensor counts = at::empty({b, h, m}, mask.options().dtype(at::kInt));
    check(chipmunk_mask_to_sorted_indices(mask.data_ptr(), packed ? 1 : 0, indices.data_ptr<int>(),
                                          counts.data_ptr<int>(), b * h * m, (int)n, (int)pad_n, (int)multiple_of,
                                          cur_stream(mask)),
          "mask_to_sorted_indices");
    return {indices, counts};
}

std::vector<at::Tensor> mask_to_ragged_indices(at::Tensor mask, at::IntArrayRef shape, int64_t multiple_of, int64_t pad_to_multiple_of,
                                               bool sorted) {
    CHECK_DEV(mask);
    const bool packed = mask.scalar_type() == at::kByte;
    TORCH_CHECK(packed || mask.scalar_type() == at::kBool, "mask must be bool, or uint8 bit-packed with a shape");
    TORCH_CHECK(multiple_of > 0 && pad_to_multiple_of > 0, "multiple_of and pad_to_multiple_of must be positive");
    mask = mask.contiguous();
    std::vector<int64_t> shp = packed ? shape.vec() : mask.sizes().vec();
    TORCH_CHECK(shp.size() == 4, "shape must be [b, h, m, n]");
    const int64_t b = shp[0], h = shp[1], m = shp[2], n = shp[3], rows = b * h * m;
    if (packed) TORCH_CHECK(n % 8 == 0 && mask.numel() * 8 >= rows * n, "bad packed mask");
    const int64_t pad_n = ((n + pad_to_multiple_of - 1) / pad_to_multiple_of) * pad_to_multiple_of;
    TORCH_CHECK(n > 0 && pad_n <= INT_MAX, "rows must have between 1 and 2^31 - 1 columns");
    c10::DeviceGuard guard(mask.device());
    at::Tensor counts = at::empty({b, h, m}, mask.options().dtype(at::kInt));
    at::Tensor len = at::empty({rows}, mask.options().dtype(at::kLong));
    check(chipmunk_mask_row_counts(mask.data_ptr(), packed ? 1 : 0, counts.data_ptr<int>(), len.data_ptr<int64_t>(), rows, (int)n,
                                   (int)pad_n, (int)multiple_of, cur_stream(mask)),
          "mask_to_ragged_indices");
    at::Tensor offsets = at::zeros({rows + 1}, len.options());
    if (rows) offsets.narrow(0, 1, rows).copy_(len.cumsum(0));
    const int64_t total = rows ? offsets[rows].item<int64_t>() : 0;
    at::Tensor flat = at::empty({total + 64}, counts.options());
    flat.narrow(0, total, 64).zero_();
    check(chipmunk_mask_to_ragged_indices(mask.data_ptr(), packed ? 1 : 0, sorted ? 1 : 0, offsets.data_ptr<int64_t>(), flat.data_ptr<int>(),
                                          rows, (int)n, (int)multiple_of, cur_stream(mask)),
          "mask_to_ragged_indices");
    return {flat, offsets, counts};
}

std::vector<at::Tensor> dense_colsum_attn_layout(at::Tensor q, at::Tensor k, at::Tensor v, at::Tensor p, bool token_major_o);
at::Tensor topk_mask(at::Tensor cs, int64_t k, double random_amount, const c10::optional<at::Tensor> &groups,
                     const c10::optional<at::Tensor> &static_mask);
std::vector<at::Tensor> dense_colsum_topk_mask(at::Tensor q, at::Tensor k, at::Tensor v, at::Tensor p, int64_t k_top, double random_amount,
                                               const c10::optional<at::Tensor> &groups, const c10::optional<at::Tensor> &static_mask,
                                               bool token_major_o) {
    CHECK_DEV(q); CHECK_DEV(k); CHECK_DEV(v); CHECK_DEV(p);
    CHECK_BF16(q); CHECK_BF16(k); CHECK_BF16(v);
    const bool shapes_ok = q.dim() == 4 && k.dim() == 4 && v.dim() == 4 && q.size(3) == 128 && q.stride(3) == 1 && k.stride(3) == 1 &&
                           v.stride(3) == 1 && p.scalar_type() == at::kFloat && p.is_contiguous();
    if (shapes_ok) {
        const int64_t B = q.size(0), H = q.size(1), Nq = q.size(2), Nk = k.size(2), G = (Nq + 191) / 192;
        const void *st = nullptr, *gf = nullptr;
        int64_t st_stride = 0, st_rows = 1;
        at::Tensor stc, gfc;
        bool ok = p.numel() == B * H * Nq;
        if (ok && static_mask.has_value() && static_mask->defined()) {
            stc = *static_mask;
            ok = stc.is_cuda() && stc.scalar_type() == at::kBool && stc.dim() == 4 && stc.size(3) == Nk && stc.size(2) == G && stc.size(1) == H &&
                 (stc.size(0) == 1 || stc.size(0) == B) && stc.stride(3) == 1 && stc.stride(1) == G * stc.stride(2) &&
                 (stc.size(0) == 1 || stc.stride(0) == H * stc.stride(1));
            if (ok) st = stc.data_ptr(), st_stride = stc.stride(2), st_rows = stc.size(0) * H * G;
        }
        if (ok && groups.has_value() && groups->defined()) {
            gfc = *groups;
            ok = gfc.is_cuda() && gfc.scalar_type() == at::kBool && gfc.dim() == 4 && gfc.size(3) == 1 && gfc.size(2) == G && gfc.size(1) == H &&
                 (gfc.size(0) == 1 || gfc.size(0) == B);
            if (ok) {
                gfc = gfc.expand({B, H, G, 1}).contiguous();
                gf = gfc.data_ptr();
            }
        }
        if (ok) {
            c10::DeviceGuard guard(q.device());
            at::Tensor o = alloc_o(q, q, token_major_o);
            const int64_t os[3] = {o.stride(0), o.stride(1), o.stride(2)};
            at::Tensor l = at::empty({B, H, Nq, 1}, q.options().dtype(at::kFloat));
            at::Tensor mask = at::empty({B, H, G, Nk}, q.options().dtype(at::kBool));
            const int64_t qs[3] = {q.stride(0), q.stride(1), q.stride(2)}, ks[3] = {k.stride(0), k.stride(1), k.stride(2)},
                          vs[3] = {v.stride(0), v.stride(1), v.stride(2)};
            const int rc = chipmunk_dense_colsum_topk_mask_strided(q.data_ptr(), k.data_ptr(), v.data_ptr(), qs, ks, vs, p.data_ptr<float>(), o.data_ptr(),
                                                           os, l.data_ptr<float>(), (int)B, (int)H, (int)Nq, (int)Nk, st, st_stride, (int)st_rows, gf,
                                                           mask.data_ptr(), (int)k_top, random_amount, cur_stream(q));
            if (rc == CHIPMUNK_OK) return {o, mask, l};
            if (rc != CHIPMUNK_ERR_UNSUPPORTED) check(rc, "dense_colsum_topk_mask");
        }
    }
    auto ocl = dense_colsum_attn_layout(q, k, v, p, token_major_o);
    at::Tensor cs = ocl[1];
    const int64_t Nk = k.size(2), G = (q.size(2) + 191) / 192;
    if (cs.size(-1) != Nk || cs.size(-2) != G) cs = cs.slice(-2, 0, G).slice(-1, 0, Nk);
    return {ocl[0], topk_mask(cs, k_top, random_amount, groups, static_mask), ocl[2]};
}

at::Tensor topk_mask(at::Tensor cs, int64_t k, double random_amount, const c10::optional<at::Tensor> &groups,
                     const c10::optional<at::Tensor> &static_mask) {
    CHECK_DEV(cs); CHECK_BF16(cs);
    TORCH_CHECK(cs.dim() == 4 && cs.stride(3) == 1, "cs must be [B, H, G, N] with a contiguous last dim");
    const int64_t B = cs.size(0), H = cs.size(1), G = cs.size(2), N = cs.size(3);
    if (!(cs.stride(1) == G * cs.stride(2) && (B == 1 || cs.stride(0) == H * cs.stride(1)))) cs = cs.contiguous();
    const int64_t rows = B * H * G;
    c10::DeviceGuard guard(cs.device());
    at::Tensor mask = at::empty({B, H, G, N}, cs.options().dtype(at::kBool));
    const void *st = nullptr, *gf = nullptr;
    int64_t st_stride = 0, st_rows = 1;
    at::Tensor stc, gfc;
    if (static_mask.has_value() && static_mask->defined()) {
        stc = *static_mask;
        CHECK_DEV(stc);
        TORCH_CHECK(stc.scalar_type() == at::kBool && stc.dim() == 4 && stc.size(3) == N && stc.size(2) == G &&
                    stc.size(1) == H && (stc.size(0) == 1 || stc.size(0) == B), "static_mask must be bool [1|B, H, G, N]");
        if (!(stc.stride(3) == 1 && stc.stride(1) == G * stc.stride(2) && (stc.size(0) == 1 || stc.stride(0) == H * stc.stride(1))))
            stc = stc.contiguous();
        st = stc.data_ptr(), st_stride = stc.stride(2), st_rows = stc.size(0) * H * G;
    }
    if (groups.has_value() && groups->defined()) {
        gfc = *groups;
        CHECK_DEV(gfc);
        TORCH_CHECK(gfc.scalar_type() == at::kBool && gfc.dim() == 4 && gfc.size(3) == 1 && gfc.size(2) == G &&
                    gfc.size(1) == H && (gfc.size(0) == 1 || gfc.size(0) == B), "groups must be bool [1|B, H, G, 1]");
        gfc = gfc.expand({B, H, G, 1}).contiguous();
        gf = gfc.data_ptr();
    }
    check(chipmunk_topk_mask(cs.data_ptr(), cs.stride(2), st, st_stride, (int)st_rows, gf, mask.data_ptr(), (int)rows, (int)N,
                             (int)k, random_amount, cur_stream(cs)),
          "topk_mask");
    return mask;
}

at::Tensor bitpack(at::Tensor mask) {
    TORCH_CHECK(mask.scalar_type() == at::kBool, "mask must be bool type");
    CHECK_DEV(mask);
    mask = mask.contiguous();
    c10::DeviceGuard guard(mask.device());
    at::Tensor packed = at::empty({(mask.numel() + 7) / 8}, mask.options().dtype(at::kByte));
    check(chipmunk_bitpack(mask.data_ptr(), packed.data_ptr(), mask.numel(), cur_stream(mask)), "bitpack");
    return packed;
}
at::Tensor bitunpack(at::Tensor packed, at::IntArrayRef shape) {
    TORCH_CHECK(packed.scalar_type() == at::kByte && packed.is_contiguous(), "packed must be a contiguous uint8 tensor");
    CHECK_DEV(packed);
    int64_t n = 1;
    for (auto d : shape) n *= d;
    TORCH_CHECK(packed.numel() * 8 >= n, "packed is too short for the given shape");
    c10::DeviceGuard guard(packed.device());
    at::Tensor mask = at::empty(shape, packed.options().dtype(at::kBool));
    check(chipmunk_bitunpack(packed.data_ptr(), mask.data_ptr(), n, cur_stream(packed)), "bitunpack");
    return mask;
}

std::vector<at::Tensor> qkv_split_norm(at::Tensor qkv, const c10::optional<at::Tensor> &q_weight, const c10::optional<at::Tensor> &k_weight,
                                       int64_t heads, double eps, const c10::optional<at::Tensor> &freqs_cos,
                                       const c10::optional<at::Tensor> &freqs_sin) {
    CHECK_DEV(qkv); CHECK_BF16(qkv);
    TORCH_CHECK(qkv.dim() == 2 && qkv.stride(1) == 1 && qkv.size(1) >= 3 * heads * 128, "qkv_split_norm: qkv must be [n, >= 3*heads*128] with a contiguous last dim");
    const void *qw = nullptr, *kw = nullptr;
    at::Tensor qwc, kwc;
    if (q_weight.has_value() && q_weight->defined()) { qwc = q_weight->contiguous(); CHECK_DEV(qwc); CHECK_BF16(qwc); TORCH_CHECK(qwc.numel() == 128); qw = qwc.data_ptr(); }
    if (k_weight.has_value() && k_weight->defined()) { kwc = k_weight->contiguous(); CHECK_DEV(kwc); CHECK_BF16(kwc); TORCH_CHECK(kwc.numel() == 128); kw = kwc.data_ptr(); }
    const int64_t n = qkv.size(0);
    const float *fc = nullptr, *fs = nullptr;
    int64_t rope_rows = 0;
    at::Tensor fcc, fsc;
    if (freqs_cos.has_value() && freqs_cos->defined()) {
        TORCH_CHECK(freqs_sin.has_value() && freqs_sin->defined(), "qkv_split_norm: freqs_cos without freqs_sin");
        fcc = freqs_cos->contiguous(), fsc = freqs_sin->contiguous();
        CHECK_DEV(fcc); CHECK_DEV(fsc);
        TORCH_CHECK(fcc.scalar_type() == at::kFloat && fsc.scalar_type() == at::kFloat && fcc.dim() == 2 && fcc.size(1) == 128 &&
                    fsc.sizes() == fcc.sizes() && fcc.size(0) <= n, "qkv_split_norm: freqs must be float32 [rows <= n, 128]");
        fc = fcc.data_ptr<float>(), fs = fsc.data_ptr<float>(), rope_rows = fcc.size(0);
    }
    c10::DeviceGuard guard(qkv.device());
    at::Tensor out = at::empty({3, 1, heads, n, 128}, qkv.options());
    check(chipmunk_qkv_split_norm(qkv.data_ptr(), qkv.stride(0), qw, kw, out[0].data_ptr(), out[1].data_ptr(), out[2].data_ptr(), n,
                                  (int)heads, (float)eps, fc, fs, rope_rows, cur_stream(qkv)),
          "qkv_split_norm");
    return {out[0], out[1], out[2]};
}

std::vector<at::Tensor> split_heads_rownorm(at::Tensor x, int64_t heads, int64_t parts, const c10::optional<at::Tensor> &w0,
                                            const c10::optional<at::Tensor> &w1, const c10::optional<at::Tensor> &w2, int64_t norm_mask,
                                            int64_t rope_mask, double eps, const c10::optional<at::Tensor> &freqs_cos,
                                            const c10::optional<at::Tensor> &freqs_sin) {
    CHECK_DEV(x); CHECK_BF16(x);
    TORCH_CHECK(parts >= 1 && parts <= 3 && heads >= 1 && heads <= 64, "split_heads_rownorm: parts must be in 1 .. 3 and heads in 1 .. 64");
    TORCH_CHECK((x.dim() == 2 || x.dim() == 3) && x.stride(-1) == 1 && x.size(-1) >= parts * heads * 128,
                "split_heads_rownorm: x must be [B, n, >= parts*heads*128] or [n, >= parts*heads*128] with a contiguous last dim");
    TORCH_CHECK(norm_mask >= 0 && rope_mask >= 0 && (norm_mask >> parts) == 0 && (rope_mask >> parts) == 0, "split_heads_rownorm: a mask names a part past parts");
    const int64_t B = x.dim() == 3 ? x.size(0) : 1, n = x.size(-2), C = heads * 128;
    TORCH_CHECK(B >= 1, "split_heads_rownorm: empty batch");
    const c10::optional<at::Tensor> *ws[3] = {&w0, &w1, &w2};
    at::Tensor wc[3];
    const void *wp[3] = {nullptr, nullptr, nullptr};
    int wd[3] = {0, 0, 0};
    for (int p = 0; p < 3; ++p) {
        if (!(ws[p]->has_value() && (*ws[p])->defined())) continue;
        TORCH_CHECK(p < parts && (norm_mask >> p & 1), "split_heads_rownorm: weight ", p, " belongs to a part that is not normalised");
        wc[p] = (*ws[p])->contiguous();
        CHECK_DEV(wc[p]);
        TORCH_CHECK((wc[p].scalar_type() == at::kBFloat16 || wc[p].scalar_type() == at::kFloat) && wc[p].numel() == C,
                    "split_heads_rownorm: a weight must be bfloat16 or float32 with heads*128 entries");
        wp[p] = wc[p].data_ptr(), wd[p] = wc[p].scalar_type() == at::kFloat ? 2 : 1;
    }
    const float *fc = nullptr, *fs = nullptr;
    int64_t rope_rows = 0;
    at::Tensor fcc, fsc;
    const bool has_cos = freqs_cos.has_value() && freqs_cos->defined(), has_sin = freqs_sin.has_value() && freqs_sin->defined();
    TORCH_CHECK(has_cos == has_sin, "split_heads_rownorm: freqs_cos and freqs_sin come together");
    TORCH_CHECK(rope_mask == 0 || has_cos, "split_heads_rownorm: a rotated part needs freqs_cos / freqs_sin");
    if (has_cos) {
        fcc = freqs_cos->contiguous(), fsc = freqs_sin->contiguous();
        CHECK_DEV(fcc); CHECK_DEV(fsc);
        TORCH_CHECK(fcc.scalar_type() == at::kFloat && fsc.scalar_type() == at::kFloat && fcc.dim() == 2 && fcc.size(1) == 128 &&
                    fsc.sizes() == fcc.sizes() && fcc.size(0) <= n, "split_heads_rownorm: freqs must be float32 [rows <= n, 128]");
        fc = fcc.data_ptr<float>(), fs = fsc.data_ptr<float>(), rope_rows = fcc.size(0);
    }
    c10::DeviceGuard guard(x.device());
    at::Tensor out = at::empty({parts, B, heads, n, 128}, x.options());
    void *op[3] = {nullptr, nullptr, nullptr};
    std::vector<at::Tensor> res;
    for (int p = 0; p < parts; ++p) res.push_back(out[p]), op[p] = res.back().data_ptr();
    if (n == 0) return res;
    check(chipmunk_split_heads_rownorm(x.data_ptr(), x.dim() == 3 ? x.stride(0) : 0, x.stride(-2), (int)parts, wp[0], wd[0], wp[1], wd[1], wp[2],
                                       wd[2], op[0], op[1], op[2], (unsigned)norm_mask, (unsigned)rope_mask, B, n, (int)heads, (float)eps, fc,
                                       fs, rope_rows, cur_stream(x)),
          "split_heads_rownorm");
    return res;
}

at::Tensor gather_rows(at::Tensor src, at::Tensor map) {
    CHECK_DEV(src);
    CHECK_DEV(map);
    TORCH_CHECK(src.dim() >= 2, "gather_rows: src must be [..., n, d]");
    TORCH_CHECK(map.scalar_type() == at::kInt && map.dim() == 1 && map.is_contiguous(), "gather_rows: map must be a contiguous int32 vector");
    src = src.contiguous();
    const int64_t n_src = src.size(-2), d = src.size(-1), n_out = map.numel();
    const int64_t outer = n_src * d == 0 ? 0 : src.numel() / (n_src * d);
    auto sizes = src.sizes().vec();
    sizes[sizes.size() - 2] = n_out;
    c10::DeviceGuard guard(src.device());
    at::Tensor dst = at::empty(sizes, src.options());
    if (dst.numel() == 0) return dst;
    check(chipmunk_gather_rows(src.data_ptr(), dst.data_ptr(), map.data_ptr<int>(), outer, n_src, n_out,
                               d * (int64_t)src.element_size(), cur_stream(src)),
          "gather_rows");
    return dst;
}

}

TORCH_LIBRARY(chipmunk, m) {
    m.def("csp_mlp_mm1(Tensor a, Tensor b_colmajor, Tensor(c!) c, Tensor bias, Tensor pa_cache_colmajor, Tensor indices, Tensor indices_counts) -> ()");
    m.def("csp_mlp_mm2_and_scatter_add(Tensor packed, Tensor(unpacked_colmajor!) unpacked_colmajor, Tensor sp_inds, Tensor sp_counts, Tensor mma_a, Tensor mma_b, Tensor mma_c, int num_sms_scatter_add, int matmul_kernel) -> ()");

    m.def("csp_attn(Tensor q, Tensor k, Tensor v, Tensor o, Tensor indices, Tensor indices_counts, int o_scale) -> ()");
    m.def("csp_128_attn(Tensor q, Tensor k, Tensor v, Tensor indices, Tensor indices_counts) -> Tensor");
    m.def("dense_attn(Tensor q, Tensor k, Tensor v) -> Tensor[]");
    m.def("dense_colsum_attn(Tensor q, Tensor k, Tensor v, Tensor p) -> Tensor[]");

    m.def("copy_indices(Tensor bmfc1, Tensor(bm_mid_cache!) bm_mid_cache, Tensor sp_inds, Tensor sp_counts) -> ()");
    m.def("topk_indices(Tensor activation, Tensor(indices!) indices, Tensor counts, float sparsity_amount, int multiple_of, float random_amount) -> ()");
    m.def("csp_scatter_add(Tensor packed, Tensor(unpacked_colmajor!) unpacked_colmajor, Tensor sp_inds, Tensor sp_counts, int num_sms) -> ()");
    m.def("mask_to_indices(Tensor mask, int multiple_of, int pad_to_multiple_of) -> Tensor[]");

    m.def("csp_attn_out(Tensor q, Tensor k, Tensor v, Tensor o_in, Tensor indices, Tensor indices_counts, int o_scale) -> Tensor");
    m.def("csp_mlp_mm1_scatter(Tensor a, Tensor b_colmajor, Tensor(c!) c, Tensor bias, Tensor(pa_cache_colmajor!) pa_cache_colmajor, Tensor indices, Tensor indices_counts) -> ()");
    m.def("csp_mlp_mm2(Tensor mma_a, Tensor mma_b, Tensor indices, Tensor counts, Tensor(mma_c!) mma_c) -> ()");
    m.def("csp_mlp_mm1_fp8(Tensor a, Tensor b, Tensor(c!) c, Tensor bias, Tensor(pa_cache_colmajor!) pa_cache_colmajor, Tensor indices, Tensor indices_counts, Tensor scale_a, Tensor scale_b, bool update_cache) -> ()");
    m.def("csp_mlp_mm1_fp8_scatter(Tensor a, Tensor b, Tensor(c!) c, Tensor bias, Tensor(pa_cache_colmajor!) pa_cache_colmajor, Tensor indices, Tensor indices_counts, Tensor scale_a, Tensor scale_b) -> ()");
    m.def("topk_delta_indices(Tensor activation, Tensor(cache!) cache, Tensor(indices!) indices, Tensor(counts!) counts, float sparsity_amount, int multiple_of, float random_amount) -> ()");
    m.def("packed_mask_to_indices(Tensor packed, int[] shape, int multiple_of, int pad_to_multiple_of) -> Tensor[]");
    m.def("mask_to_sorted_indices(Tensor mask, int[] shape, int multiple_of, int pad_to_multiple_of) -> Tensor[]");
    m.def("topk_mask(Tensor cs, int k, float random_amount, Tensor? groups, Tensor? static_mask) -> Tensor");
    m.def("dense_colsum_topk_mask(Tensor q, Tensor k, Tensor v, Tensor p, int k_top, float random_amount, Tensor? groups, Tensor? static_mask, bool token_major_o=False) -> Tensor[]");
    m.def("dense_attn_layout(Tensor q, Tensor k, Tensor v, bool token_major_o) -> Tensor[]");
    m.def("dense_colsum_attn_layout(Tensor q, Tensor k, Tensor v, Tensor p, bool token_major_o) -> Tensor[]");
    m.def("compact_indices(Tensor indices, Tensor counts) -> Tensor[]");
    m.def("mask_to_ragged_indices(Tensor mask, int[] shape, int multiple_of, int pad_to_multiple_of, bool sorted) -> Tensor[]");
    m.def("csp_attn_out_ragged(Tensor q, Tensor k, Tensor v, Tensor o_in, Tensor indices, Tensor offsets, Tensor indices_counts, int o_scale) -> Tensor");
    m.def("residual_ln_modulate(Tensor x, Tensor? y, Tensor? gate, Tensor shift, Tensor scale, float eps) -> Tensor[]");
    m.def("transpose_last2(Tensor x) -> Tensor");
    m.def("transpose_last2_pitched(Tensor x, int ld) -> Tensor");
    m.def("block_mean(Tensor x, int mbm) -> Tensor");
    m.def("quantize_fp8(Tensor x, Tensor scale, float max_value) -> Tensor");
    m.def("bitpack(Tensor mask) -> Tensor");
    m.def("bitunpack(Tensor packed, int[] shape) -> Tensor");
    m.def("gather_rows(Tensor src, Tensor map) -> Tensor");
    m.def("qkv_split_norm(Tensor qkv, Tensor? q_weight, Tensor? k_weight, int heads, float eps, Tensor? freqs_cos=None, Tensor? freqs_sin=None) -> Tensor[]");
    m.def("split_heads_rownorm(Tensor x, int heads, int parts, Tensor? w0, Tensor? w1, Tensor? w2, int norm_mask, int rope_mask, float eps, Tensor? freqs_cos=None, Tensor? freqs_sin=None) -> Tensor[]");
}

TORCH_LIBRARY_IMPL(chipmunk, CUDA, m) {
    m.impl("qkv_split_norm", &qkv_split_norm);
    m.impl("split_heads_rownorm", &split_heads_rownorm);
    m.impl("csp_mlp_mm1_fp8_scatter", &csp_mlp_mm1_fp8_scatter);
    m.impl("dense_colsum_topk_mask", &dense_colsum_topk_mask);
    m.impl("csp_mlp_mm1", &csp_mlp_mm1);
    m.impl("csp_mlp_mm2_and_scatter_add", &csp_mlp_mm2_and_scatter_add);
    m.impl("copy_indices", &copy_indices);
    m.impl("topk_indices", &topk_indices);
    m.impl("csp_scatter_add", &csp_scatter_add);
    m.impl("mask_to_indices", &mask_to_indices);
    m.impl("csp_attn", &csp_attn);
    m.impl("csp_128_attn", &csp_128_attn);
    m.impl("dense_attn", &dense_attn);
    m.impl("dense_colsum_attn", &dense_colsum_attn);
    m.impl("compact_indices", &compact_indices);
    m.impl("residual_ln_modulate", &residual_ln_modulate);
    m.impl("csp_attn_out_ragged", &csp_attn_out_ragged);
    m.impl("dense_attn_layout", &dense_attn_layout);
    m.impl("dense_colsum_attn_layout", &dense_colsum_attn_layout);
    m.impl("csp_attn_out", &csp_attn_out);
    m.impl("csp_mlp_mm1_scatter", &csp_mlp_mm1_scatter);
    m.impl("csp_mlp_mm2", &csp_mlp_mm2);
    m.impl("csp_mlp_mm1_fp8", &csp_mlp_mm1_fp8);
    m.impl("topk_delta_indices", &topk_delta_indices);
    m.impl("packed_mask_to_indices", &packed_mask_to_indices);
    m.impl("mask_to_sorted_indices", &mask_to_sorted_indices);
    m.impl("mask_to_ragged_indices", &mask_to_ragged_indices);
    m.impl("topk_mask", &topk_mask);
    m.impl("transpose_last2", &transpose_last2);
    m.impl("transpose_last2_pitched", &transpose_last2_pitched);
    m.impl("block_mean", &block_mean);
    m.impl("quantize_fp8", &quantize_fp8);
    m.impl("bitpack", &bitpack);
    m.impl("bitunpack", &bitunpack);
    m.impl("gather_rows", &gather_rows);
}

}
```

### chipmunk_amd/modules/attn.py

```python
from __future__ import annotations

from typing import Optional, Tuple

import torch
import torch.nn.functional as F
from torch import Tensor, nn

from .. import ops
from ..ops.voxel import get_local_indices_with_text
from ..util.config import GLOBAL_CONFIG, amd_key
from ..util.layer_counter import LayerCounter
from ..util.storage import AttnStorage
from ..util.storage.offloaded_tensor import release_kept_offloaded, release_resident, reserve_kept_offloaded, reserve_resident

singleton_static_mask: Optional[Tensor] = None
singleton_video_query_groups: Optional[Tensor] = None


def _cdiv(a: int, b: int) -> int:
    return (a + b - 1) // b


def _dense_attn_raw(q: Tensor, k: Tensor, v: Tensor, token_major_o: bool):
    return torch.ops.chipmunk.dense_attn_layout(q, k, v, True) if token_major_o else torch.ops.chipmunk.dense_attn(q, k, v)


class SparseDiffAttn(nn.Module):
    def __init__(self, layer_num: int, layer_counter: LayerCounter, storage_slot: int = 0, query_group_offset: int = 0):
        super().__init__()
        self.layer_num = layer_num
        self.layer_counter = layer_counter
        self.query_group_offset = query_group_offset
        self.storage = AttnStorage(layer_num, init_names=["indices", "out_cache"], slot=storage_slot)
        self.mask_shape = [None] * GLOBAL_CONFIG["num_model_invocations_per_inference_step"]
        self._unpacked = [None] * GLOBAL_CONFIG["num_model_invocations_per_inference_step"]

    def initialize_static_mask(self, seq_shape: Tuple, txt_len: int, local_heads_num: int, device: torch.device):
        if len(seq_shape) == 2:
            raise NotImplementedError("Not yet implemented for 2D sequences")
        tt, th, tw = seq_shape
        cfg = GLOBAL_CONFIG["attn"]
        n_video = tt * th * tw
        topk = int(cfg["top_keys"] * n_video)
        lv = cfg["local_voxels"]
        mask, _, _ = get_local_indices_with_text(vid_shape=(tt, th, tw), txt_len=txt_len, voxel_shape=(4, 6, 8),
                                                 local_shape=(lv, lv, lv), rk=cfg["random_keys"], device=device)
        if cfg["local_1d_window"] > 0:
            window = int(cfg["local_1d_window"] * n_video)
            for qg in range(n_video // 192):
                centre = qg * 192 + 96
                mask[qg, max(0, centre - window // 2):min(n_video, centre + window // 2)] = True
        mask = mask[None, None, :, :].expand(1, local_heads_num, -1, -1).contiguous()
        sparse_groups = (mask.sum(dim=-1, keepdim=True) + topk) < (n_video + txt_len)
        global singleton_static_mask, singleton_video_query_groups
        singleton_static_mask = mask
        singleton_video_query_groups = sparse_groups

    def _static(self, heads: int, qg: int, n: int):
        g0 = self.query_group_offset
        assert heads <= singleton_static_mask.shape[1] or singleton_static_mask.shape[1] == 1, (
            f"this module serves {heads} heads but initialize_static_mask() built {singleton_static_mask.shape[1]} head planes "
            "(local_heads_num): build the static mask for the largest head chunk")
        h = min(heads, singleton_static_mask.shape[1])
        return (singleton_static_mask[:, :h, g0:g0 + qg, :n], singleton_video_query_groups[:, :h, g0:g0 + qg, :])

    def random_and_topk(self, cs: Tensor, topk: int) -> Tensor:
        cfg = GLOBAL_CONFIG["attn"]
        qg, n = cs.shape[-2], cs.shape[-1]
        static, groups = self._static(cs.shape[1], qg, n)
        if cs.is_cuda and amd_key("attn", "fused_topk_mask") and cs.dtype == torch.bfloat16 and n <= ops.TOPK_MASK_MAX_N:
            return ops.topk_mask(cs, topk, 0.01, groups, static)
        mask = torch.randint(0, 100, cs.shape, device=cs.device, dtype=torch.uint8) == 0
        mask.scatter_(-1, cs.topk(k=topk, dim=-1).indices, True)
        mask.logical_and_(groups)
        mask.logical_or_(static)
        return mask

    def release_kept_indices(self) -> None:
        for inv, old in enumerate(self._unpacked):
            if old is not None:
                self._release_kept(old)
                self._unpacked[inv] = None

    @staticmethod
    def _release_kept(kept) -> None:
        release_resident(kept[3])
        if kept[4]:
            release_kept_offloaded(kept[3])

    def __del__(self):
        try:
            self.release_kept_indices()
        except Exception:
            pass

    @torch.compiler.disable
    def _remember_indices(self, inds: Optional[Tensor], counts: Tensor, ragged=None) -> None:
        inv = self.layer_counter.cur_model_invocation_per_step
        old, self._unpacked[inv] = self._unpacked[inv], None
        if old is not None:
            self._release_kept(old)
        self.storage.indices.suppress_current(False)
        if not (counts.is_cuda and amd_key("attn", "keep_unpacked_indices") and amd_key("attn", "fused_residual")
                and (self.storage.indices.is_resident() or amd_key("attn", "keep_unpacked_indices_offloaded"))):
            return
        if not reserve_resident(0):
            return
        flat, offsets = ragged if ragged is not None else ops.compact_indices(inds, counts)
        nbytes = 4 * flat.numel() + 8 * offsets.numel() + 4 * counts.numel()
        off_mode = not self.storage.indices.is_resident()
        if off_mode and not reserve_kept_offloaded(nbytes):
            return
        if not reserve_resident(nbytes):
            if off_mode:
                release_kept_offloaded(nbytes)
            return
        self._unpacked[inv] = (flat, offsets, counts, nbytes, off_mode)
        self.storage.indices.suppress_current(off_mode and bool(GLOBAL_CONFIG["attn"]["recompute_mask"]))

    def _kept_indices(self):
        kept = self._unpacked[self.layer_counter.cur_model_invocation_per_step]
        if kept is not None and GLOBAL_CONFIG["attn"]["should_compress_indices"] and (
                self.storage.indices.is_resident() or amd_key("attn", "keep_unpacked_indices_offloaded")):
            return kept[:3]
        return None

    def _stored_mask(self):
        if self.storage.indices.is_suppressed():
            self.storage.indices.suppress_current(False)
            self.storage.indices.load_async()
            self.storage.indices.load_async_wait()
        return self.storage.get_indices(), self.mask_shape[self.layer_counter.cur_model_invocation_per_step]

    @staticmethod
    def _ragged_enabled(x: Tensor) -> bool:
        return bool(x.is_cuda and GLOBAL_CONFIG["attn"]["should_compress_indices"] and amd_key("attn", "fused_residual")
                    and amd_key("attn", "fused_packed_mask_to_indices") and amd_key("attn", "ragged_mask_to_indices"))

    @torch.compiler.disable
    def _ragged_indices(self, packed: Tensor, shape, multiple_of: int, bm: int, mask: Optional[Tensor] = None):
        if shape[-1] % 8 != 0:
            packed = mask if mask is not None else ops.bitunpack(packed, shape)
        return ops.mask_to_ragged_indices(packed, shape, multiple_of, bm, bool(amd_key("attn", "sorted_indices")))

    def _stored_indices(self, multiple_of: int, bm: int):
        cfg = GLOBAL_CONFIG["attn"]
        if cfg["should_compress_indices"]:
            packed, shape = self._stored_mask()
            if amd_key("attn", "fused_packed_mask_to_indices") and packed.is_cuda and shape[-1] % 8 == 0:
                if amd_key("attn", "sorted_indices"):
                    return ops.mask_to_sorted_indices(packed, shape, multiple_of, bm)
                return ops.packed_mask_to_indices(packed, shape, multiple_of, bm)
            return ops.mask_to_indices(ops.bitunpack(packed, shape), multiple_of, bm)
        return self.storage.get_indices(), self.storage.get_counts()

    def _fast_attention(self, q: Tensor, k: Tensor, v: Tensor, inference_step: int, do_full_step: bool) -> Tensor:
        cfg = GLOBAL_CONFIG["attn"]
        bm = cfg["mbm"]
        assert bm == 192, "The kernel was written for BM=192. You may need to change the kernel."
        do_padding = cfg["pad_qkv_before_kernel"]
        multiple_of = 128 if do_padding else cfg["counts_multiple_of"]

        tm = bool(q.is_cuda and amd_key("attn", "token_major_output"))
        use_ragged = self._ragged_enabled(q)
        if self.layer_num < cfg["first_n_dense_layers"]:
            o, _ = ops.dense_attn(q, k, v, tm)
            return o

        if do_full_step:
            if inference_step == 0:
                o, lse = ops.dense_attn(q, k, v, tm) if do_padding else _dense_attn_raw(q, k, v, tm)
                lse[..., k.shape[-2]:, :] = 0
                self.storage.set_lse_constants(lse)
                return o

            ragged = None
            if inference_step == 1 or cfg["recompute_mask"]:
                prev_lse = self.storage.get_lse_constants()
                tk = int(multiple_of * round((cfg["top_keys"] * k.shape[-2]) / multiple_of))
                mask = bs = None
                if (q.is_cuda and cfg["should_compress_indices"] and tk > 0 and amd_key("attn", "fused_colsum_topk")
                        and amd_key("attn", "fused_topk_mask") and k.shape[-2] <= ops.TOPK_MASK_MAX_N):
                    static, groups = self._static(q.shape[1], _cdiv(q.shape[-2], bm), k.shape[-2])
                    o, mask, lse = ops.dense_colsum_topk_mask(q, k, v, prev_lse, tk, 0.01, groups, static, tm)
                elif do_padding:
                    o, bs, lse = ops.dense_colsum_attn(q, k, v, prev_lse, tm)
                else:
                    o, bs, lse = (torch.ops.chipmunk.dense_colsum_attn_layout(q, k, v, prev_lse, True) if tm else
                                  torch.ops.chipmunk.dense_colsum_attn(q, k, v, prev_lse))
                lse[..., k.shape[-2]:, :] = 0
                self.storage.set_lse_constants(lse)
                if cfg["should_compress_indices"]:
                    if mask is not None:
                        pass
                    elif tk > 0:
                        mask = self.random_and_topk(bs, tk)
                    else:
                        mask = self._static(bs.shape[1], bs.shape[-2], bs.shape[-1])[0]
                    packed, mask_shape = ops.bitpack(mask)
                    self.mask_shape[self.layer_counter.cur_model_invocation_per_step] = mask_shape
                    self.storage.set_indices(packed)
                    if use_ragged:
                        ragged = self._ragged_indices(packed, mask_shape, multiple_of, bm, mask)
                        self._remember_indices(None, ragged[2], ragged[:2])
                    else:
                        if mask.is_cuda and amd_key("attn", "fused_packed_mask_to_indices") and amd_key("attn", "sorted_indices"):
                            inds, counts = ops.mask_to_sorted_indices(mask, mask.shape, multiple_of, bm)
                        else:
                            inds, counts = ops.mask_to_indices(mask, multiple_of, bm)
                        self._remember_indices(inds, counts)
                else:
                    kseq = k.shape[-2]
                    bs = bs[..., :_cdiv(kseq, bm), :kseq]
                    inds = torch.topk(bs, k=tk, dim=-1).indices
                    counts = torch.full((q.shape[0], q.shape[1], _cdiv(q.shape[-2], bm)), tk, device=q.device,
                                        dtype=torch.int32)
                    pad = torch.empty((*counts.shape, q.shape[-2] - tk), device=q.device, dtype=torch.int32)
                    inds = torch.cat([inds, pad], dim=-1).to(torch.int32)
                    self.storage.set_indices(inds)
                    self.storage.set_counts(counts)
            else:
                o, _ = ops.dense_attn(q, k, v, tm)

            if use_ragged:
                if ragged is None:
                    ragged = self._ragged_indices(*self._stored_mask(), multiple_of, bm)
            elif not cfg["recompute_mask"]:
                inds, counts = self._stored_indices(multiple_of, bm)

            if ragged is not None:
                o_cache = ops.csp_attn_out_ragged(q, k, v, o, ragged[0], ragged[1], ragged[2], -1)
            elif o.is_cuda and amd_key("attn", "fused_residual"):
                o_cache = ops.csp_attn_out(q, k, v, o, inds, counts, -1)
            elif do_padding:
                o_cache = o - ops.csp_attn(q, k, v, inds, counts)
            else:
                o_cache = o.clone()
                ops.csp_attn_inplace(q, k, v, o_cache, inds, counts, -1)
            self.storage.set_out_cache(o_cache)
            return o

        o = self.storage.get_out_cache()
        kept = self._kept_indices() if (o.is_cuda and amd_key("attn", "fused_residual")) else None
        if kept is not None:
            return ops.csp_attn_out_ragged(q, k, v, o, kept[0], kept[1], kept[2], 1)
        if use_ragged:
            flat, offsets, counts = self._ragged_indices(*self._stored_mask(), multiple_of, bm)
            return ops.csp_attn_out_ragged(q, k, v, o, flat, offsets, counts, 1)
        inds, counts = self._stored_indices(multiple_of, bm)
        if do_padding:
            if o.is_cuda and amd_key("attn", "fused_residual"):
                return ops.csp_attn_out(q, k, v, o, inds, counts, 1)
            return o + ops.csp_attn(q, k, v, inds, counts)
        persistent = self.storage.out_cache.is_resident()
        if o.is_cuda and amd_key("attn", "fused_residual") and persistent:
            return ops.csp_attn_out(q, k, v, o, inds, counts, 1)
        if persistent:
            o = o.clone()
        ops.csp_attn_inplace(q, k, v, o, inds, counts, 1)
        return o

    def forward(self, q: Tensor, k: Tensor, v: Tensor) -> Tensor:
        if not GLOBAL_CONFIG["attn"]["is_enabled"]:
            return F.scaled_dot_product_attention(q, k, v)
        do_full_step = self.layer_counter.should_do_full_attn_step()
        out = self._fast_attention(q, k, v, self.layer_counter.cur_inference_step, do_full_step)
        self.layer_counter.increment()
        return out

    def __call__(self, *args, **kwargs):
        return self.forward(*args, **kwargs)
```

### chipmunk_amd/ops/_fake.py

```python
import torch


def _o_like(q, token_major):
    B, H, N, D = q.shape
    return q.new_empty((B, N, H, D)).permute(0, 2, 1, 3) if token_major else q.new_empty((B, H, N, D))


def _register():
    lib = torch.library

    @lib.register_fake("chipmunk::csp_128_attn")
    def _(q, k, v, indices, indices_counts):
        return torch.empty_like(q)

    @lib.register_fake("chipmunk::csp_attn_out")
    def _(q, k, v, o_in, indices, indices_counts, o_scale):
        return torch.empty_like(o_in)

    @lib.register_fake("chipmunk::residual_ln_modulate")
    def _(x, y, gate, shift, scale, eps):
        return [torch.empty_like(x), torch.empty_like(x)] if y is not None else [torch.empty_like(x)]

    @lib.register_fake("chipmunk::csp_attn_out_ragged")
    def _(q, k, v, o_in, indices, offsets, indices_counts, o_scale):
        return torch.empty_like(o_in)

    @lib.register_fake("chipmunk::dense_attn")
    def _(q, k, v):
        return [_o_like(q, False), q.new_empty((q.shape[0], q.shape[1], q.shape[2], 1), dtype=torch.float32)]

    @lib.register_fake("chipmunk::dense_attn_layout")
    def _(q, k, v, token_major_o):
        return [_o_like(q, token_major_o), q.new_empty((q.shape[0], q.shape[1], q.shape[2], 1), dtype=torch.float32)]

    @lib.register_fake("chipmunk::dense_colsum_attn_layout")
    def _(q, k, v, p, token_major_o):
        groups = (q.shape[2] + 191) // 192
        return [_o_like(q, token_major_o),
                q.new_empty((q.shape[0], q.shape[1], groups, max(q.shape[2], k.shape[2]))),
                q.new_empty((q.shape[0], q.shape[1], q.shape[2], 1), dtype=torch.float32)]

    @lib.register_fake("chipmunk::dense_colsum_attn")
    def _(q, k, v, p):
        groups = (q.shape[2] + 191) // 192
        return [_o_like(q, False),
                q.new_empty((q.shape[0], q.shape[1], groups, max(q.shape[2], k.shape[2]))),
                q.new_empty((q.shape[0], q.shape[1], q.shape[2], 1), dtype=torch.float32)]

    @lib.register_fake("chipmunk::mask_to_indices")
    def _(mask, multiple_of, pad_to_multiple_of):
        b, h, m, n = mask.shape
        pad_n = (n + pad_to_multiple_of - 1) // pad_to_multiple_of * pad_to_multiple_of
        return [mask.new_empty((b, h, m, pad_n), dtype=torch.int32), mask.new_empty((b, h, m), dtype=torch.int32)]

    @lib.register_fake("chipmunk::packed_mask_to_indices")
    def _(packed, shape, multiple_of, pad_to_multiple_of):
        b, h, m, n = shape
        pad_n = (n + pad_to_multiple_of - 1) // pad_to_multiple_of * pad_to_multiple_of
        return [packed.new_empty((b, h, m, pad_n), dtype=torch.int32), packed.new_empty((b, h, m), dtype=torch.int32)]

    @lib.register_fake("chipmunk::topk_mask")
    def _(cs, k, random_amount, groups, static_mask):
        return cs.new_empty(cs.shape, dtype=torch.bool)

    @lib.register_fake("chipmunk::block_mean")
    def _(x, mbm):
        return x.new_empty((x.shape[0], (x.shape[1] + mbm - 1) // mbm, x.shape[2]))

    @lib.register_fake("chipmunk::transpose_last2")
    def _(x):
        return x.new_empty(x.shape[:-2] + (x.shape[-1], x.shape[-2]))

    @lib.register_fake("chipmunk::transpose_last2_pitched")
    def _(x, ld):
        return x.new_empty(x.shape[:-2] + (x.shape[-1], ld))

    @lib.register_fake("chipmunk::quantize_fp8")
    def _(x, scale, max_value):
        return x.new_empty(x.shape, dtype=torch.float8_e4m3fn)

    @lib.register_fake("chipmunk::bitpack")
    def _(mask):
        return mask.new_empty(((mask.numel() + 7) // 8,), dtype=torch.uint8)

    @lib.register_fake("chipmunk::bitunpack")
    def _(packed, shape):
        return packed.new_empty(tuple(shape), dtype=torch.bool)

    @lib.register_fake("chipmunk::gather_rows")
    def _(src, map):
        shape = list(src.shape)
        shape[-2] = map.shape[0]
        return src.new_empty(shape)

    @lib.register_fake("chipmunk::dense_colsum_topk_mask")
    def _(q, k, v, p, k_top, random_amount, groups, static_mask, token_major_o=False):
        B, H, Nq, D = q.shape
        G = (Nq + 191) // 192
        return [_o_like(q, token_major_o), q.new_empty((B, H, G, k.shape[2]), dtype=torch.bool),
                q.new_empty((B, H, Nq, 1), dtype=torch.float32)]

    @lib.register_fake("chipmunk::qkv_split_norm")
    def _(qkv, q_weight, k_weight, heads, eps, freqs_cos=None, freqs_sin=None):
        out = qkv.new_empty((3, 1, heads, qkv.shape[0], 128))
        return [out[0], out[1], out[2]]

    @lib.register_fake("chipmunk::split_heads_rownorm")
    def _(x, heads, parts, w0, w1, w2, norm_mask, rope_mask, eps, freqs_cos=None, freqs_sin=None):
        out = x.new_empty((parts, x.shape[0] if x.dim() == 3 else 1, heads, x.shape[-2], 128))
        return [out[p] for p in range(parts)]


_register()
```

### chipmunk_amd/ops/attn.py

```python
from __future__ import annotations

from typing import Tuple

import torch
import torch.nn.functional as F

PM = 192


def _pad_len(n: int) -> int:
    return ((n + PM - 1) // PM) * PM


def _last_dim_contiguous(t: torch.Tensor) -> torch.Tensor:
    return t if t.stride(-1) == 1 else t.contiguous()


def dense_attn(q: torch.Tensor, k: torch.Tensor, v: torch.Tensor, token_major_o: bool = False) -> Tuple[torch.Tensor, torch.Tensor]:
    n = q.shape[-2]
    q, k, v = _last_dim_contiguous(q), _last_dim_contiguous(k), _last_dim_contiguous(v)
    o, l = torch.ops.chipmunk.dense_attn_layout(q, k, v, True) if token_major_o else torch.ops.chipmunk.dense_attn(q, k, v)
    padded = _pad_len(n)
    if padded != n:
        l = F.pad(l, (0, 0, 0, padded - n))
    return o, l


def dense_colsum_attn(q: torch.Tensor, k: torch.Tensor, v: torch.Tensor, p: torch.Tensor, token_major_o: bool = False
                      ) -> Tuple[torch.Tensor, torch.Tensor, torch.Tensor]:
    n = q.shape[-2]
    padded = _pad_len(n)
    assert p.shape[-2] in (n, padded), "p must be the l vector of the previous full step"
    p_rows = p[..., :n, :].contiguous()
    q, k, v = _last_dim_contiguous(q), _last_dim_contiguous(k), _last_dim_contiguous(v)
    if token_major_o:
        o, cs, l = torch.ops.chipmunk.dense_colsum_attn_layout(q, k, v, p_rows, True)
    else:
        o, cs, l = torch.ops.chipmunk.dense_colsum_attn(q, k, v, p_rows)
    if padded != n:
        l = F.pad(l, (0, 0, 0, padded - n))
    kseq = k.shape[-2]
    kgroups = (kseq + PM - 1) // PM
    if cs.shape[-2] != kgroups or cs.shape[-1] != kseq:
        cs = cs[..., :kgroups, :kseq]
    return o, cs, l


def dense_colsum_topk_mask(q: torch.Tensor, k: torch.Tensor, v: torch.Tensor, p: torch.Tensor, k_top: int, random_amount: float,
                           groups, static_mask, token_major_o: bool = False) -> Tuple[torch.Tensor, torch.Tensor, torch.Tensor]:
    n = q.shape[-2]
    padded = _pad_len(n)
    assert p.shape[-2] in (n, padded), "p must be the l vector of the previous full step"
    o, mask, l = torch.ops.chipmunk.dense_colsum_topk_mask(_last_dim_contiguous(q), _last_dim_contiguous(k), _last_dim_contiguous(v),
                                                           p[..., :n, :].contiguous(), k_top, random_amount, groups, static_mask,
                                                           token_major_o)
    if padded != n:
        l = F.pad(l, (0, 0, 0, padded - n))
    return o, mask, l


def csp_attn(q: torch.Tensor, k: torch.Tensor, v: torch.Tensor, indices: torch.Tensor,
             indices_counts: torch.Tensor) -> torch.Tensor:
    return torch.ops.chipmunk.csp_128_attn(q.contiguous(), k.contiguous(), v.contiguous(), indices.contiguous(),
                                           indices_counts.contiguous())


def csp_attn_inplace(q: torch.Tensor, k: torch.Tensor, v: torch.Tensor, o: torch.Tensor, indices: torch.Tensor,
                     indices_counts: torch.Tensor, o_scale: int) -> None:
    torch.ops.chipmunk.csp_attn(q, k, v, o, indices, indices_counts, o_scale)


def csp_attn_out(q: torch.Tensor, k: torch.Tensor, v: torch.Tensor, o_in: torch.Tensor, indices: torch.Tensor,
                 indices_counts: torch.Tensor, o_scale: int) -> torch.Tensor:
    return torch.ops.chipmunk.csp_attn_out(q, k, v, o_in, indices, indices_counts, o_scale)


def compact_indices(indices: torch.Tensor, indices_counts: torch.Tensor) -> Tuple[torch.Tensor, torch.Tensor]:
    return tuple(torch.ops.chipmunk.compact_indices(indices.contiguous(), indices_counts.contiguous()))


def csp_attn_out_ragged(q: torch.Tensor, k: torch.Tensor, v: torch.Tensor, o_in: torch.Tensor, indices: torch.Tensor,
                        offsets: torch.Tensor, indices_counts: torch.Tensor, o_scale: int) -> torch.Tensor:
    return torch.ops.chipmunk.csp_attn_out_ragged(q, k, v, o_in, indices, offsets, indices_counts, o_scale)


__all__ = ["csp_attn", "csp_attn_inplace", "csp_attn_out", "csp_attn_out_ragged", "compact_indices", "dense_attn", "dense_colsum_attn",
           "dense_colsum_topk_mask"]
```

### chipmunk_amd/ops/indexed_io.py

```python
from __future__ import annotations

from typing import List, Optional, Sequence

import torch

TOPK_MASK_MAX_N = 1024 * 512


def copy_indices(bm_fc1: torch.Tensor, bm_mid_cache: torch.Tensor, indices: torch.Tensor, counts: torch.Tensor) -> None:
    torch.ops.chipmunk.copy_indices(bm_fc1, bm_mid_cache, indices, counts)


def topk_indices(activations: torch.Tensor, indices_out: torch.Tensor, counts_out: torch.Tensor,
                 sparsity_amount: float, multiple_of: int, rk: float) -> None:
    torch.ops.chipmunk.topk_indices(activations, indices_out, counts_out, sparsity_amount, multiple_of, rk)


def scatter_add(packed: torch.Tensor, unpacked: torch.Tensor, indices: torch.Tensor, counts: torch.Tensor,
                num_sms: int) -> None:
    if packed.ndim == 3:
        torch.ops.chipmunk.csp_scatter_add(packed, unpacked, indices, counts, num_sms)
        return
    torch.ops.chipmunk.csp_scatter_add(packed.unsqueeze(0), unpacked.unsqueeze(0), indices.unsqueeze(0),
                                       counts.unsqueeze(0), num_sms)


def mask_to_indices(mask: torch.Tensor, multiple_of: int, pad_to_multiple_of: int) -> List[torch.Tensor]:
    return torch.ops.chipmunk.mask_to_indices(mask, multiple_of, pad_to_multiple_of)


def packed_mask_to_indices(packed: torch.Tensor, shape: Sequence[int], multiple_of: int,
                           pad_to_multiple_of: int) -> List[torch.Tensor]:
    return torch.ops.chipmunk.packed_mask_to_indices(packed, list(shape), multiple_of, pad_to_multiple_of)


def mask_to_sorted_indices(mask: torch.Tensor, shape: Sequence[int], multiple_of: int,
                           pad_to_multiple_of: int) -> List[torch.Tensor]:
    return torch.ops.chipmunk.mask_to_sorted_indices(mask, list(shape), multiple_of, pad_to_multiple_of)


def mask_to_ragged_indices(mask: torch.Tensor, shape: Sequence[int], multiple_of: int, pad_to_multiple_of: int,
                           sorted: bool = True) -> List[torch.Tensor]:
    if mask.is_cuda:
        return torch.ops.chipmunk.mask_to_ragged_indices(mask, list(shape), multiple_of, pad_to_multiple_of, sorted)
    if mask.dtype == torch.uint8:
        from .bitpack import bitunpack
        mask = bitunpack(mask, shape)
    b, h, m, n = mask.shape
    pad_n = (n + pad_to_multiple_of - 1) // pad_to_multiple_of * pad_to_multiple_of
    rows = mask.reshape(-1, n) != 0
    kept = rows.sum(dim=1)
    counts = (kept + multiple_of - 1) // multiple_of * multiple_of
    lengths = (counts.clamp(max=pad_n) + 31) // 32 * 32
    offsets = torch.zeros(rows.shape[0] + 1, dtype=torch.int64)
    offsets[1:] = lengths.cumsum(0)
    flat = torch.zeros(int(offsets[-1]) + 64, dtype=torch.int32)
    cols = torch.arange(n, dtype=torch.int32)
    for r in range(rows.shape[0]):
        true = cols[rows[r]]
        if not sorted:
            true = true[torch.argsort(true % 32, stable=True)]
        row = torch.cat([true, cols[~rows[r]][:int(counts[r] - kept[r])]])
        flat[int(offsets[r]):int(offsets[r]) + row.numel()] = row
    return [flat, offsets, counts.to(torch.int32).view(b, h, m)]


def topk_mask(cs: torch.Tensor, k: int, random_amount: float = 0.0, groups: Optional[torch.Tensor] = None,
              static_mask: Optional[torch.Tensor] = None) -> torch.Tensor:
    return torch.ops.chipmunk.topk_mask(cs, k, random_amount, groups, static_mask)


def manual_seed(seed: int) -> None:
    from .._native import manual_seed as _seed
    _seed(seed)
```

### chipmunk_amd/util/config.py

```python
from __future__ import annotations

import copy
from typing import Any, Dict

import yaml

BASE_CONFIG: Dict[str, Any] = {
    "num_model_invocations_per_inference_step": 1,
    "should_profile": False,
    "generation_index": 0,
    "steps": 50,
    "world_size": 1,
    "mlp": {
        "is_enabled": True,
        "is_fp8": False,
        "top_keys": "dd",
        "random_keys": 0.05,
        "full_step_every": 10,
        "block_mask_cache": 2,
        "first_n_dense_layers": 2,
        "counts_multiple_of": 256,
        "bm": 128,
        "mbm": 128,
    },
    "patchify": {
        "is_enabled": True,
        "chunk_size_1": 8,
        "chunk_size_2": 4,
    },
    "attn": {
        "is_enabled": True,
        "top_keys": 0.05,
        "random_keys": 0.01,
        "local_voxels": 0,
        "local_1d_window": 0,
        "first_n_dense_layers": 2,
        "full_step_every": 10,
        "full_step_schedule": None,
        "recompute_mask": True,
        "should_compress_indices": True,
        "counts_multiple_of": 128,
        "pad_qkv_before_kernel": True,
        "mbm": 192,
    },
    "offloading": {
        "global_disable_offloading": False,
        "mlp.out_cache": False,
        "mlp.indices": False,
        "mlp.counts": False,
        "mlp.sparse_act_T": False,
        "mlp.blockmean_mid_cache": False,
        "attn.out_cache": True,
        "attn.indices": True,
        "attn.counts": False,
        "attn.lse_constants": False,
        "text_encoders": True,
    },
    "step_caching": {
        "is_enabled": True,
        "skip_step_schedule": {7, 11, 13, 14, 15, 17, 18, 19, 21, 22, 23, 25, 26, 27, 29, 31, 33, 34, 35, 37, 38, 39,
                               41, 42, 43},
    },
}

AMD_EXTRA_KEYS: Dict[str, Any] = {
    "offloading.keep_resident_if_fits": False,
    "offloading.hbm_budget_gb": 200.0,
    "offloading.native_host_pool": True,
    "attn.fused_packed_mask_to_indices": True,
    "attn.sorted_indices": True,
    "mlp.fused_topk_delta": True,
    "mlp.fused_block_mean": True,
    "mlp.fused_fp8_quantize": True,
    "attn.fused_residual": True,
    "attn.fused_topk_mask": True,
    "attn.fused_colsum_topk": True,
    "mlp.fused_scatter": True,
    "attn.token_major_output": False,
    "attn.keep_unpacked_indices": True,
    "attn.keep_unpacked_indices_offloaded": True,
    "attn.kept_indices_offloaded_budget_gb": 8.0,
    "attn.ragged_mask_to_indices": True,
}
BASE_CONFIG["offloading"]["keep_resident_if_fits"] = AMD_EXTRA_KEYS["offloading.keep_resident_if_fits"]
BASE_CONFIG["offloading"]["hbm_budget_gb"] = AMD_EXTRA_KEYS["offloading.hbm_budget_gb"]
BASE_CONFIG["offloading"]["native_host_pool"] = AMD_EXTRA_KEYS["offloading.native_host_pool"]
BASE_CONFIG["attn"]["fused_packed_mask_to_indices"] = AMD_EXTRA_KEYS["attn.fused_packed_mask_to_indices"]
BASE_CONFIG["attn"]["sorted_indices"] = AMD_EXTRA_KEYS["attn.sorted_indices"]
BASE_CONFIG["mlp"]["fused_topk_delta"] = AMD_EXTRA_KEYS["mlp.fused_topk_delta"]
BASE_CONFIG["attn"]["fused_residual"] = AMD_EXTRA_KEYS["attn.fused_residual"]
BASE_CONFIG["attn"]["fused_topk_mask"] = AMD_EXTRA_KEYS["attn.fused_topk_mask"]
BASE_CONFIG["attn"]["fused_colsum_topk"] = AMD_EXTRA_KEYS["attn.fused_colsum_topk"]
BASE_CONFIG["mlp"]["fused_scatter"] = AMD_EXTRA_KEYS["mlp.fused_scatter"]
BASE_CONFIG["attn"]["token_major_output"] = AMD_EXTRA_KEYS["attn.token_major_output"]
BASE_CONFIG["attn"]["keep_unpacked_indices"] = AMD_EXTRA_KEYS["attn.keep_unpacked_indices"]
BASE_CONFIG["attn"]["keep_unpacked_indices_offloaded"] = AMD_EXTRA_KEYS["attn.keep_unpacked_indices_offloaded"]
BASE_CONFIG["attn"]["kept_indices_offloaded_budget_gb"] = AMD_EXTRA_KEYS["attn.kept_indices_offloaded_budget_gb"]
BASE_CONFIG["attn"]["ragged_mask_to_indices"] = AMD_EXTRA_KEYS["attn.ragged_mask_to_indices"]

GLOBAL_CONFIG: Dict[str, Any] = copy.deepcopy(BASE_CONFIG)


def amd_key(section: str, key: str) -> Any:
    return GLOBAL_CONFIG.get(section, {}).get(key, AMD_EXTRA_KEYS[f"{section}.{key}"])


def update_global_config(config: Dict[str, Any]) -> None:
    GLOBAL_CONFIG.update(config)


def _deep_update(dst: Dict[str, Any], src: Dict[str, Any]) -> None:
    for key, value in src.items():
        if isinstance(value, dict) and isinstance(dst.get(key), dict):
            _deep_update(dst[key], value)
        else:
            dst[key] = value


def load_from_file(config_file: str) -> None:
    with open(config_file, "r") as f:
        loaded = yaml.safe_load(f)
    if loaded:
        _deep_update(GLOBAL_CONFIG, loaded)
        print(f"CHIPMUNK: using config file {config_file}")


def reset_to_base() -> None:
    fresh = copy.deepcopy(BASE_CONFIG)
    GLOBAL_CONFIG.clear()
    GLOBAL_CONFIG.update(fresh)
```

### include/chipmunk_hip.h

```cpp
#ifndef CHIPMUNK_HIP_H
#define CHIPMUNK_HIP_H

#include <stdint.h>

#ifdef __cplusplus
extern "C" {
#endif

#define CHIPMUNK_OK 0
#define CHIPMUNK_ERR_INVALID 1
#define CHIPMUNK_ERR_LAUNCH 2
#define CHIPMUNK_ERR_UNSUPPORTED 3

#define CHIPMUNK_DTYPE_BF16 0
#define CHIPMUNK_DTYPE_FP16 1
#define CHIPMUNK_DTYPE_FP32 2

const char *chipmunk_last_error(void);
int chipmunk_abi_version(void);
int chipmunk_set_option(const char *name, int value);
int chipmunk_set_random_seed(uint64_t seed);

int chipmunk_csp_attn(const void *q, const void *k, const void *v, void *o, const int64_t q_strides[3],
                      const int64_t k_strides[3], const int64_t v_strides[3], const int64_t o_strides[3],
                      const int32_t *indices, const int32_t *counts, int B, int H, int Nq, int Nk, int idx_stride,
                      int o_scale, void *stream);

int chipmunk_csp_attn_out(const void *q, const void *k, const void *v, const void *o_in, void *o_out,
                          const int64_t q_strides[3], const int64_t k_strides[3], const int64_t v_strides[3],
                          const int64_t o_strides[3], const int32_t *indices, const int32_t *counts, int B, int H,
                          int Nq, int Nk, int idx_stride, int o_scale, void *stream);

int chipmunk_csp_attn_out_ragged(const void *q, const void *k, const void *v, const void *o_in, void *o_out,
                                 const int64_t q_strides[3], const int64_t k_strides[3], const int64_t v_strides[3],
                                 const int64_t o_strides[3], const int32_t *indices, const int64_t *idx_offsets,
                                 const int32_t *counts, int B, int H, int Nq, int Nk, int o_scale, void *stream);
int chipmunk_compact_indices(const int32_t *indices, int64_t idx_stride, const int32_t *counts, const int64_t *offsets,
                             int32_t *flat, int64_t rows, void *stream);

int chipmunk_csp_128_attn(const void *q, const void *k, const void *v, void *o, const int32_t *indices,
                          const int32_t *counts, int B, int H, int Nq, int Nk, int idx_stride, void *stream);

int chipmunk_dense_attn(const void *q, const void *k, const void *v, const int64_t q_strides[3],
                        const int64_t k_strides[3], const int64_t v_strides[3], void *o, float *l, int B, int H,
                        int Nq, int Nk, void *stream);

int chipmunk_dense_attn_strided(const void *q, const void *k, const void *v, const int64_t q_strides[3],
                                const int64_t k_strides[3], const int64_t v_strides[3], void *o, const int64_t *o_strides,
                                float *l, int B, int H, int Nq, int Nk, void *stream);
int chipmunk_dense_colsum_attn_strided(const void *q, const void *k, const void *v, const int64_t q_strides[3],
                                       const int64_t k_strides[3], const int64_t v_strides[3], const float *p, void *o,
                                       const int64_t *o_strides, void *cs, float *l, int B, int H, int Nq, int Nk,
                                       int cs_stride, void *stream);
int chipmunk_dense_colsum_topk_mask_strided(const void *q, const void *k, const void *v, const int64_t q_strides[3],
                                            const int64_t k_strides[3], const int64_t v_strides[3], const float *p, void *o,
                                            const int64_t *o_strides, float *l, int B, int H, int Nq, int Nk,
                                            const void *static_mask, int64_t static_stride, int static_rows,
                                            const void *group_flags, void *mask, int k_top, double random_amount, void *stream);

int chipmunk_dense_colsum_attn(const void *q, const void *k, const void *v, const int64_t q_strides[3],
                               const int64_t k_strides[3], const int64_t v_strides[3], const float *p, void *o,
                               void *cs, float *l, int B, int H, int Nq, int Nk, int cs_stride, void *stream);

int chipmunk_residual_ln_modulate(const void *x, const void *y, const void *gate, const void *shift, const void *scale,
                                  void *x_out, void *xm, int64_t rows, int cols, double eps, void *stream);

int chipmunk_csp_mlp_mm1(const void *a, const void *b, void *c, const void *bias, const void *pa_cache,
                         const int32_t *indices, const int32_t *counts, int M, int K, int F, void *stream);

int chipmunk_csp_mlp_mm1_scatter(const void *a, const void *b, void *c, const void *bias, void *pa_cache,
                                 const int32_t *indices, const int32_t *counts, int M, int K, int F, void *stream);

int chipmunk_csp_mlp_mm1_fp8(const void *a, const void *b, void *c, const void *bias, void *pa_cache,
                             const int32_t *indices, const int32_t *counts, const float *scale_a,
                             const float *scale_b, int M, int K, int F, int update_cache, void *stream);

int chipmunk_csp_mlp_mm2_and_scatter_add(const void *packed, void *unpacked_colmajor, const int32_t *indices,
                                         const int32_t *counts, const void *mma_a, const void *mma_b, void *mma_c,
                                         int M, int F, int N2, int num_sms_scatter_add, void *stream);

int chipmunk_csp_scatter_add(const void *packed, void *unpacked_colmajor, const int32_t *indices,
                             const int32_t *counts, int M, int F, int num_sms, void *stream);

int chipmunk_csp_mlp_mm2(const void *mma_a, const void *mma_b, void *mma_c, const int32_t *indices,
                         const int32_t *counts, int M, int F, int N2, void *stream);

int chipmunk_csp_mlp_mm1_ragged(const void *a, const void *b, void *c, const void *bias, const void *pa_cache,
                                const int32_t *indices, const int32_t *counts, int M, int K, int F, int ldc, void *stream);
int chipmunk_csp_mlp_mm1_scatter_ragged(const void *a, const void *b, void *c, const void *bias, void *pa_cache,
                                        const int32_t *indices, const int32_t *counts, int M, int K, int F, int ldc,
                                        void *stream);
int chipmunk_csp_mlp_mm1_fp8_ragged(const void *a, const void *b, void *c, const void *bias, void *pa_cache,
                                    const int32_t *indices, const int32_t *counts, const float *scale_a,
                                    const float *scale_b, int M, int K, int F, int ldc, int update_cache, void *stream);
int chipmunk_csp_mlp_mm2_ragged(const void *mma_a, const void *mma_b, void *mma_c, const int32_t *indices,
                                const int32_t *counts, int M, int F, int N2, void *stream);
int chipmunk_csp_mlp_mm2_and_scatter_add_ragged(const void *packed, void *unpacked_colmajor, const int32_t *indices,
                                                const int32_t *counts, const void *mma_a, const void *mma_b, void *mma_c,
                                                int M, int F, int N2, int ldc, void *stream);
int chipmunk_csp_scatter_add_ragged(const void *packed, void *unpacked_colmajor, const int32_t *indices,
                                    const int32_t *counts, int M, int F, int ldc, void *stream);

int chipmunk_csp_mlp_mm1_batched(const void *a, const void *b, void *c, const void *bias, const void *pa_cache,
                                 const int32_t *indices, const int32_t *counts, int M, int K, int F, int ldc, int B,
                                 int64_t cache_batch_stride, void *stream);
int chipmunk_csp_mlp_mm1_scatter_batched(const void *a, const void *b, void *c, const void *bias, void *pa_cache,
                                         const int32_t *indices, const int32_t *counts, int M, int K, int F, int ldc, int B,
                                         int64_t cache_batch_stride, void *stream);
int chipmunk_csp_mlp_mm1_fp8_batched(const void *a, const void *b, void *c, const void *bias, void *pa_cache,
                                     const int32_t *indices, const int32_t *counts, const float *scale_a, const float *scale_b,
                                     int M, int K, int F, int ldc, int update_cache, int B, int64_t cache_batch_stride,
                                     void *stream);
int chipmunk_csp_mlp_mm2_batched(const void *mma_a, const void *mma_b, void *mma_c, const int32_t *indices,
                                 const int32_t *counts, int M, int F, int N2, int B, void *stream);
int chipmunk_csp_mlp_mm2_and_scatter_add_batched(const void *packed, void *unpacked_colmajor, const int32_t *indices,
                                                 const int32_t *counts, const void *mma_a, const void *mma_b, void *mma_c,
                                                 int M, int F, int N2, int ldc, int B, int64_t cache_batch_stride,
                                                 void *stream);
int chipmunk_csp_scatter_add_batched(const void *packed, void *unpacked_colmajor, const int32_t *indices,
                                     const int32_t *counts, int M, int F, int ldc, int B, int64_t cache_batch_stride,
                                     void *stream);

int chipmunk_topk_indices(const void *activation, int dtype, int32_t *indices, int32_t *counts, int rows, int cols,
                          double sparsity_amount, int multiple_of, double random_amount, void *stream);

int chipmunk_topk_delta_indices(const void *activation, void *cache, int dtype, int32_t *indices, int32_t *counts,
                                int rows, int cols, double sparsity_amount, int multiple_of, double random_amount,
                                void *stream);

int chipmunk_dense_colsum_topk_mask(const void *q, const void *k, const void *v, const int64_t q_strides[3],
                                    const int64_t k_strides[3], const int64_t v_strides[3], const float *p, void *o, float *l,
                                    int B, int H, int Nq, int Nk, const void *static_mask, int64_t static_stride, int static_rows,
                                    const void *group_flags, void *mask, int k_top, double random_amount, void *stream);

int chipmunk_topk_mask(const void *cs, int64_t cs_stride, const void *static_mask, int64_t static_stride,
                       int static_rows, const void *group_flags, void *mask, int rows, int n, int k,
                       double random_amount, void *stream);

int chipmunk_mask_to_indices(const void *mask, int32_t *indices, int32_t *counts, int64_t rows, int n, int pad_n,
                             int multiple_of, void *stream);

int chipmunk_packed_mask_to_indices(const void *packed, int32_t *indices, int32_t *counts, int64_t rows, int n,
                                    int pad_n, int multiple_of, void *stream);

int chipmunk_mask_to_sorted_indices(const void *mask, int packed, int32_t *indices, int32_t *counts, int64_t rows,
                                    int n, int pad_n, int multiple_of, void *stream);

int chipmunk_mask_row_counts(const void *mask, int packed, int32_t *counts, int64_t *lengths, int64_t rows, int n, int pad_n,
                             int multiple_of, void *stream);
int chipmunk_mask_to_ragged_indices(const void *mask, int packed, int sorted, const int64_t *offsets, int32_t *flat, int64_t rows,
                                    int n, int multiple_of, void *stream);

int chipmunk_copy_indices(const void *src, void *dst, const int32_t *inds, const int32_t *counts, int B, int M, int R,
                          int F, int elem_size, void *stream);

int chipmunk_transpose16(const void *src, void *dst, int B, int R, int C, void *stream);
int chipmunk_transpose16_pitched(const void *src, void *dst, int B, int R, int C, int ld, void *stream);

int chipmunk_block_mean(const void *x, void *out, int64_t rows, int C, int mbm, void *stream);
int chipmunk_block_mean_ragged(const void *x, void *out, int64_t rows, int C, int mbm, void *stream);

int chipmunk_quantize_fp8(const void *x, const float *scale, void *out, int64_t n, float max_value, void *stream);

int chipmunk_bitpack(const void *mask, void *packed, int64_t n, void *stream);
int chipmunk_bitunpack(const void *packed, void *mask, int64_t n, void *stream);

int chipmunk_gather_rows(const void *src, void *dst, const int32_t *map, int64_t outer, int64_t n_src, int64_t n_out,
                         int64_t row_bytes, void *stream);

int chipmunk_host_alloc(size_t bytes, void **host_ptr);
int chipmunk_host_free(void *host_ptr);
int chipmunk_copy_d2h_async(void *host_dst, const void *dev_src, size_t bytes, void *stream);
int chipmunk_copy_h2d_async(void *dev_dst, const void *host_src, size_t bytes, void *stream);
size_t chipmunk_host_bytes(void);

int chipmunk_release_scratch(void);
int chipmunk_big_scratch_fallbacks(void);

int chipmunk_qkv_split_norm(const void *qkv, int64_t row_stride, const void *q_weight, const void *k_weight, void *q, void *k,
                            void *v, int64_t n, int heads, float eps, const float *freqs_cos, const float *freqs_sin,
                            int64_t rope_rows, void *stream);

int chipmunk_split_heads_rownorm(const void *x, int64_t batch_stride, int64_t row_stride, int parts, const void *w0, int w0_dtype,
                                 const void *w1, int w1_dtype, const void *w2, int w2_dtype, void *out0, void *out1, void *out2,
                                 unsigned norm_mask, unsigned rope_mask, int64_t B, int64_t n, int heads, float eps,
                                 const float *freqs_cos, const float *freqs_sin, int64_t rope_rows, void *stream);

#ifdef __cplusplus
}
#endif
#endif
```

Baseline: 0.5759.

## Emit bit-packed top-k mask with row counts directly from fused colsum kernel

Adds packed variants of the top-k mask kernels that write a 1-bit-per-key mask using DPP nibble merging and also compute per-row padded counts and lengths. The fused dense colsum attention path now produces this packed mask when ragged indices are in use. A counted mask-to-ragged-indices op then consumes it without a separate row-count pass. This is meant to cut mask memory traffic eightfold and remove the bool-mask, pack and count steps, at the cost of more kernel variants and new ABI entry points.

```diff
diff --git a/chipmunk_amd/_native.py b/chipmunk_amd/_native.py
--- a/chipmunk_amd/_native.py
+++ b/chipmunk_amd/_native.py
@@ -15,7 +15,7 @@
     "chipmunk_csp_mlp_mm1_batched", "chipmunk_csp_mlp_mm1_scatter_batched", "chipmunk_csp_mlp_mm1_fp8_batched", "chipmunk_csp_mlp_mm2_batched",
     "chipmunk_csp_mlp_mm2_and_scatter_add_batched", "chipmunk_csp_scatter_add_batched",
     "chipmunk_topk_indices", "chipmunk_topk_delta_indices", "chipmunk_topk_mask", "chipmunk_mask_to_indices", "chipmunk_mask_to_sorted_indices", "chipmunk_packed_mask_to_indices", "chipmunk_mask_row_counts", "chipmunk_mask_to_ragged_indices", "chipmunk_copy_indices",
-    "chipmunk_bitpack", "chipmunk_bitunpack", "chipmunk_transpose16", "chipmunk_block_mean", "chipmunk_quantize_fp8", "chipmunk_gather_rows", "chipmunk_qkv_split_norm", "chipmunk_split_heads_rownorm", "chipmunk_dense_colsum_topk_mask", "chipmunk_dense_attn_strided", "chipmunk_csp_attn_out_ragged", "chipmunk_compact_indices", "chipmunk_residual_ln_modulate", "chipmunk_dense_colsum_attn_strided", "chipmunk_dense_colsum_topk_mask_strided", "chipmunk_release_scratch", "chipmunk_big_scratch_fallbacks",
+    "chipmunk_bitpack", "chipmunk_bitunpack", "chipmunk_transpose16", "chipmunk_block_mean", "chipmunk_quantize_fp8", "chipmunk_gather_rows", "chipmunk_qkv_split_norm", "chipmunk_split_heads_rownorm", "chipmunk_dense_colsum_topk_mask", "chipmunk_dense_attn_strided", "chipmunk_csp_attn_out_ragged", "chipmunk_compact_indices", "chipmunk_residual_ln_modulate", "chipmunk_dense_colsum_attn_strided", "chipmunk_dense_colsum_topk_mask_strided", "chipmunk_topk_mask_packed", "chipmunk_dense_colsum_topk_packed_strided", "chipmunk_release_scratch", "chipmunk_big_scratch_fallbacks",
     "chipmunk_host_alloc", "chipmunk_host_free", "chipmunk_copy_d2h_async", "chipmunk_copy_h2d_async", "chipmunk_host_bytes",
 ]
 
diff --git a/chipmunk_amd/csrc/attn.hip b/chipmunk_amd/csrc/attn.hip
--- a/chipmunk_amd/csrc/attn.hip
+++ b/chipmunk_amd/csrc/attn.hip
@@ -1277,3 +1277,37 @@
                                                    static_mask, static_stride, static_rows, group_flags, mask, topk, random_amount,
                                                    stream);
 }
+
+extern "C" int chipmunk_dense_colsum_topk_packed_strided(const void *q, const void *k, const void *v, const int64_t q_strides[3],
+                                                         const int64_t k_strides[3], const int64_t v_strides[3], const float *pin, void *o,
+                                                         const int64_t *o_strides, float *l, int B, int H, int Nq, int Nk,
+                                                         const void *static_bits, int64_t static_stride, int static_rows,
+                                                         const void *group_flags, void *packed, int32_t *counts, int64_t *lengths,
+                                                         int topk, int pad_n, int multiple_of, double random_amount, void *stream) {
+    if (int e = check_common(q, k, v, o, B, H, Nq, Nk)) return e;
+    CM_CHECK(l && pin && packed && counts && lengths, "dense_colsum_topk_packed: p / l / packed / counts / lengths missing");
+    CM_CHECK(Nk % 8 == 0, "dense_colsum_topk_packed: Nk must be a multiple of 8 for a packed mask (got %d)", Nk);
+    if (int e = check_strides(q_strides, "q")) return e;
+    if (int e = check_strides(k_strides, "k")) return e;
+    if (int e = check_strides(v_strides, "v")) return e;
+    hipStream_t st = (hipStream_t)stream;
+    if (!use_dense64(B, H, Nq, Nk) || chipmunk_get_option("attn_fused_colsum") == 2 || Nk > CHIPMUNK_TOPK_MASK_MAX_N)
+        return CHIPMUNK_ERR_UNSUPPORTED;
+    AttnParams p = {};
+    p.q = (const uint16_t *)q, p.k = (const uint16_t *)k, p.v = (const uint16_t *)v, p.o = (uint16_t *)o;
+    for (int i = 0; i < 3; ++i) p.qs[i] = q_strides[i], p.ks[i] = k_strides[i], p.vs[i] = v_strides[i];
+    CM_CHECK((int64_t)Nk * p.ks[2] * 2 < (1ll << 32) && (int64_t)Nk * p.vs[2] * 2 < (1ll << 32),
+             "attention: one head's K or V spans more than 4 GiB (32-bit DMA offsets)");
+    if (int e = output_strides(p.os, o_strides, H, Nq)) return e;
+    p.l_out = l, p.p_in = pin, p.cs = nullptr, p.cs_stride = 0;
+    p.B = B, p.H = H, p.Nq = Nq, p.Nk = Nk, p.G = (Nq + QG - 1) / QG;
+    p.o_scale = 1.f;
+    CM_CHECK(pad_n >= Nk && multiple_of > 0 && topk >= 0 && (!static_bits || (static_rows > 0 && static_stride >= Nk / 8)),
+             "dense_colsum_topk_packed: bad sizes pad_n=%d multiple_of=%d topk=%d", pad_n, multiple_of, topk);
+    uint16_t *part = (uint16_t *)chipmunk_big_scratch(st, chipmunk_colsum_part_bytes(B, H, Nq, Nk));
+    if (!part) return CHIPMUNK_ERR_UNSUPPORTED;
+    if (int e = chipmunk_dense64_colsum_launch(p, part, st)) return e;
+    const int nrb = ((Nq + 255) / 256) * 2;
+    return chipmunk_topk_mask_parts_packed(part, chipmunk_colsum_part_stride(Nk), nrb, p.G, Nq, static_bits, static_stride, static_rows,
+                                           group_flags, packed, counts, lengths, B * H * p.G, Nk, topk, pad_n, multiple_of, random_amount, st);
+}
diff --git a/chipmunk_amd/csrc/attn_params.h b/chipmunk_amd/csrc/attn_params.h
--- a/chipmunk_amd/csrc/attn_params.h
+++ b/chipmunk_amd/csrc/attn_params.h
@@ -32,6 +32,10 @@
 int chipmunk_topk_mask_parts(const uint16_t *part, int part_stride, int nrb, int groups_per_bh, int Nq, const void *static_mask, int64_t static_stride,
                              int static_rows, const void *group_flags, void *mask, int rows, int n, int k, double random_amount,
                              hipStream_t stream);
+int chipmunk_topk_mask_parts_packed(const uint16_t *part, int part_stride, int nrb, int groups_per_bh, int Nq, const void *static_bits,
+                                    int64_t static_stride, int static_rows, const void *group_flags, void *packed, int32_t *counts,
+                                    int64_t *lengths, int rows, int n, int k, int pad_n, int multiple_of, double random_amount,
+                                    hipStream_t stream);
 size_t chipmunk_colsum_part_bytes(int B, int H, int Nq, int Nk);
 int chipmunk_colsum_part_stride(int Nk);
 int chipmunk_colsum64_launch(const AttnParams &p, hipStream_t stream);
diff --git a/chipmunk_amd/csrc/indexed_io.hip b/chipmunk_amd/csrc/indexed_io.hip
--- a/chipmunk_amd/csrc/indexed_io.hip
+++ b/chipmunk_amd/csrc/indexed_io.hip
@@ -561,14 +561,39 @@
     const uint16_t *parts;
     int64_t pstride;
     int nrb, ngroups, nq;
+    int32_t *counts;
+    int64_t *lengths;
+    int pad_n, multiple_of;
 };
+
+__device__ __forceinline__ uint32_t quad_nibbles_to_u16(uint32_t nib, int tid) {
+    uint32_t v = nib << (4 * (tid & 3));
+    v |= (uint32_t)__builtin_amdgcn_update_dpp(0, (int)v, 0xB1, 0xf, 0xf, true);
+    v |= (uint32_t)__builtin_amdgcn_update_dpp(0, (int)v, 0x4E, 0xf, 0xf, true);
+    return v;
+}
+__device__ __forceinline__ void store_quad_bits(uint8_t *row_bits, uint32_t v, int c, int n, bool even) {
+    uint8_t *d = row_bits + (c >> 3);
+    if (even && c + 16 <= n) {
+        *(uint16_t *)d = (uint16_t)v;
+    } else {
+        d[0] = (uint8_t)v;
+        if (c + 8 < n) d[1] = (uint8_t)(v >> 8);
+    }
+}
+__device__ __forceinline__ void store_row_counts(const TopkMaskParams &p, int row, int kept) {
+    const int64_t padded = (((int64_t)kept + p.multiple_of - 1) / p.multiple_of) * p.multiple_of;
+    p.counts[row] = (int32_t)padded;
+    p.lengths[row] = (min(padded, (int64_t)p.pad_n) + 31) / 32 * 32;
+}
 
 __device__ __forceinline__ uint32_t bf16_key(uint32_t u) {
     return (u & 0x8000u) ? (~u & 0xffffu) : (u | 0x8000u);
 }
 
-template <int KPT, bool ALIGNED, bool PARTS = false>
+template <int KPT, bool ALIGNED, bool PARTS = false, bool PACKED = false>
 __global__ __launch_bounds__(1024) void topk_mask_kernel(const TopkMaskParams p) {
+    static_assert(!PACKED || ALIGNED, "the packed form is an aligned form");
     constexpr int NV = KPT / 4;
     __shared__ int wave_cnt[16];
     const int tid = threadIdx.x, lane = tid & 63, w = tid >> 6;
@@ -751,7 +776,56 @@
                 if (c + e < n) out[c + e] = (uint8_t)(bytes >> (8 * e));
         }
     };
-    if constexpr (ALIGNED) {
+    auto emit_bits = [&](int c, uint32_t v0, uint32_t v1, uint32_t sb) {
+        uint32_t nib = 0;
+        asm volatile("" : "+v"(v0), "+v"(v1));
+#pragma unroll
+        for (int e = 0; e < 4; ++e) {
+            const uint32_t kv = ((e < 2 ? v0 : v1) >> (16 * (e & 1))) & 0xffffu;
+            bool keep = kv > thr;
+            const bool tie = kv == thr && tie_budget > 0 && c + e < n;
+            tie_budget -= tie ? 1 : 0;
+            keep = keep || tie;
+            if (rnd && !keep) keep = hash_uniform(row, c + e, salt) < p.random_amount;
+            keep = keep || ((sb >> e) & 1u) != 0;
+            nib |= (keep ? 1u : 0u) << e;
+        }
+        return nib;
+    };
+    if constexpr (PACKED) {
+        uint8_t *bits = p.mask + (((int64_t)row * n) >> 3);
+        const bool even = ((uintptr_t)bits & 1) == 0;
+        const int nsh = 4 * (tid & 1);
+        int kept = 0;
+        constexpr int OB = 5;
+#pragma unroll
+        for (int j0 = 0; j0 < NV; j0 += OB) {
+            uint32_t sbv[OB];
+#pragma unroll
+            for (int jj = 0; jj < OB; ++jj) {
+                const int c = 4 * tid + 4096 * (j0 + jj);
+                sbv[jj] = (j0 + jj < NV && st && c < n) ? (uint32_t)st[c >> 3] : 0u;
+            }
+            __builtin_amdgcn_sched_barrier(0);
+#pragma unroll
+            for (int jj = 0; jj < OB; ++jj) {
+                if constexpr (true) {
+                    const int c = 4 * tid + 4096 * (j0 + jj);
+                    if (j0 + jj < NV && 4096 * (j0 + jj) < n) {
+                        uint32_t nib = 0;
+                        if (c < n) nib = emit_bits(c, key[(j0 + jj) < NV ? (j0 + jj) : 0][0], key[(j0 + jj) < NV ? (j0 + jj) : 0][1], (sbv[jj] >> nsh) & 0xfu);
+                        kept += __popc(nib);
+                        const uint32_t v = quad_nibbles_to_u16(nib, tid);
+                        if ((tid & 3) == 0 && c < n) store_quad_bits(bits, v, c, n, even);
+                    }
+                    asm volatile("" ::: "memory");
+                }
+            }
+            __builtin_amdgcn_sched_barrier(0);
+        }
+        const int total = block_count(kept);
+        if (tid == 0) store_row_counts(p, row, total);
+    } else if constexpr (ALIGNED) {
         constexpr int OB = 5;
 #pragma unroll
         for (int j0 = 0; j0 < NV; j0 += OB) {
@@ -796,8 +870,9 @@
     return u ^ (s | 0x80008000u);
 }
 
-template <bool ALIGNED, bool PARTS>
+template <bool ALIGNED, bool PARTS, bool PACKED = false>
 __global__ __launch_bounds__(1024) void topk_mask_stream_kernel(const TopkMaskParams p) {
+    static_assert(!PACKED || ALIGNED, "the packed form is an aligned form");
     __shared__ int wave_cnt[16];
     const int tid = threadIdx.x, lane = tid & 63, w = tid >> 6;
     const int row = blockIdx.x;
@@ -961,6 +1036,49 @@
     }
     uint8_t *out = p.mask + (int64_t)row * n;
     const uint8_t *st = p.stat ? p.stat + (int64_t)(row % p.stat_rows) * p.stat_stride : nullptr;
+    if constexpr (PACKED) {
+        uint8_t *bits = p.mask + (((int64_t)row * n) >> 3);
+        const bool even = ((uintptr_t)bits & 1) == 0;
+        const int nsh = 4 * (tid & 1);
+        int kept = 0;
+        for (int j0 = 0; j0 < nsteps; j0 += U) {
+            uint32_t kw[U][2], sbv[U];
+#pragma unroll
+            for (int jj = 0; jj < U; ++jj) {
+                const int c = 4 * tid + 4096 * (j0 + jj);
+                kw[jj][0] = kw[jj][1] = 0;
+                if (select) load_raw(j0 + jj, kw[jj][0], kw[jj][1]);
+                sbv[jj] = (st && c < n) ? (uint32_t)st[c >> 3] : 0u;
+            }
+#pragma unroll
+            for (int jj = 0; jj < U; ++jj) {
+                const int c = 4 * tid + 4096 * (j0 + jj);
+                if (4096 * (j0 + jj) >= n) continue;
+                uint32_t nib = 0;
+                if (c < n) {
+                    if (select) to_keys(kw[jj][0], kw[jj][1]);
+                    const uint32_t sb = (sbv[jj] >> nsh) & 0xfu;
+#pragma unroll
+                    for (int e = 0; e < 4; ++e) {
+                        const uint32_t kv = (kw[jj][e >> 1] >> (16 * (e & 1))) & 0xffffu;
+                        bool keep = kv > thr;
+                        const bool tie = kv == thr && tie_budget > 0 && c + e < n;
+                        tie_budget -= tie ? 1 : 0;
+                        keep = keep || tie;
+                        if (rnd && !keep) keep = hash_uniform(row, c + e, salt) < p.random_amount;
+                        keep = keep || ((sb >> e) & 1u) != 0;
+                        nib |= (keep ? 1u : 0u) << e;
+                    }
+                }
+                kept += __popc(nib);
+                const uint32_t v = quad_nibbles_to_u16(nib, tid);
+                if ((tid & 3) == 0 && c < n) store_quad_bits(bits, v, c, n, even);
+            }
+        }
+        const int total = block_count(kept);
+        if (tid == 0) store_row_counts(p, row, total);
+        return;
+    }
     for (int j0 = 0; j0 < nsteps; j0 += U) {
         uint32_t kw[U][2], sbv[U];
 #pragma unroll
@@ -1198,6 +1316,60 @@
     else if (n <= 1024 * 16) hipLaunchKernelGGL((topk_mask_kernel<16, true, true>), dim3(rows), dim3(1024), 0, s, p);
     else if (n <= 1024 * 48) hipLaunchKernelGGL((topk_mask_kernel<48, true, true>), dim3(rows), dim3(1024), 0, s, p);
     else hipLaunchKernelGGL((topk_mask_kernel<120, true, true>), dim3(rows), dim3(1024), 0, s, p);
+    CM_LAUNCH_CHECK();
+    return CHIPMUNK_OK;
+}
+
+static int check_topk_mask_packed(const void *static_bits, int64_t static_stride, int static_rows, void *packed, int32_t *counts,
+                                  int64_t *lengths, int rows, int n, int k, int pad_n, int multiple_of, double random_amount) {
+    CM_CHECK(packed && counts && lengths, "topk_mask_packed: null pointer");
+    CM_CHECK(rows >= 0 && n > 0 && k >= 0, "topk_mask_packed: bad sizes (rows=%d n=%d k=%d)", rows, n, k);
+    CM_CHECK(n % 8 == 0, "topk_mask_packed: n must be a multiple of 8 for a packed mask (got %d)", n);
+    CM_CHECK(n <= CHIPMUNK_TOPK_MASK_MAX_N, "topk_mask_packed: rows of more than %d columns are not supported (got %d)", CHIPMUNK_TOPK_MASK_MAX_N, n);
+    CM_CHECK(pad_n >= n && multiple_of > 0, "topk_mask_packed: bad sizes pad_n=%d multiple_of=%d (n=%d)", pad_n, multiple_of, n);
+    CM_CHECK(!static_bits || (static_rows > 0 && static_stride >= n / 8), "topk_mask_packed: bad static mask geometry");
+    CM_CHECK(random_amount >= 0.0 && random_amount <= 1.0, "topk_mask_packed: random_amount must be in [0,1]");
+    return CHIPMUNK_OK;
+}
+
+template <bool PARTS>
+static void launch_topk_mask_packed(const TopkMaskParams &p, hipStream_t s) {
+    const int rows = p.rows, n = p.n;
+    if (n > 1024 * 120 || chipmunk_get_option("topk_mask_stream") == 1) hipLaunchKernelGGL((topk_mask_stream_kernel<true, PARTS, true>), dim3(rows), dim3(1024), 0, s, p);
+    else if (n <= 1024 * 16) hipLaunchKernelGGL((topk_mask_kernel<16, true, PARTS, true>), dim3(rows), dim3(1024), 0, s, p);
+    else if (n <= 1024 * 48) hipLaunchKernelGGL((topk_mask_kernel<48, true, PARTS, true>), dim3(rows), dim3(1024), 0, s, p);
+    else hipLaunchKernelGGL((topk_mask_kernel<120, true, PARTS, true>), dim3(rows), dim3(1024), 0, s, p);
+}
+
+int chipmunk_topk_mask_parts_packed(const uint16_t *part, int part_stride, int nrb, int groups_per_bh, int Nq, const void *static_bits,
+                                    int64_t static_stride, int static_rows, const void *group_flags, void *packed, int32_t *counts,
+                                    int64_t *lengths, int rows, int n, int k, int pad_n, int multiple_of, double random_amount, hipStream_t s) {
+    if (int e = check_topk_mask_packed(static_bits, static_stride, static_rows, packed, counts, lengths, rows, n, k, pad_n, multiple_of, random_amount)) return e;
+    CM_CHECK(part && part_stride >= n && (part_stride & 3) == 0 && ((uintptr_t)part & 7) == 0, "topk_mask_parts_packed: bad partial rows");
+    if (rows == 0) return CHIPMUNK_OK;
+    TopkMaskParams p = {nullptr, (const uint8_t *)static_bits, (const uint8_t *)group_flags, (uint8_t *)packed, 0, static_stride,
+                        rows, n, k, static_bits ? static_rows : 1, (float)random_amount,
+                        random_amount > 0.0 ? chipmunk_next_random_salt() : 0u};
+    p.parts = part, p.pstride = part_stride, p.nrb = nrb, p.ngroups = groups_per_bh, p.nq = Nq;
+    p.counts = counts, p.lengths = lengths, p.pad_n = pad_n, p.multiple_of = multiple_of;
+    launch_topk_mask_packed<true>(p, s);
+    CM_LAUNCH_CHECK();
+    return CHIPMUNK_OK;
+}
+
+extern "C" int chipmunk_topk_mask_packed(const void *cs, int64_t cs_stride, const void *static_bits, int64_t static_stride, int static_rows,
+                                         const void *group_flags, void *packed, int32_t *counts, int64_t *lengths, int rows, int n, int k,
+                                         int pad_n, int multiple_of, double random_amount, void *stream) {
+    CM_CHECK(cs, "topk_mask_packed: null pointer");
+    if (int e = check_topk_mask_packed(static_bits, static_stride, static_rows, packed, counts, lengths, rows, n, k, pad_n, multiple_of, random_amount)) return e;
+    CM_CHECK(cs_stride >= n, "topk_mask_packed: cs row stride %lld < n %d", (long long)cs_stride, n);
+    CM_CHECK((((uintptr_t)cs) & 7) == 0 && (cs_stride & 3) == 0, "topk_mask_packed: cs and its row stride must be 8-byte aligned");
+    if (rows == 0) return CHIPMUNK_OK;
+    TopkMaskParams p = {(const uint16_t *)cs, (const uint8_t *)static_bits, (const uint8_t *)group_flags, (uint8_t *)packed,
+                        cs_stride, static_stride, rows, n, k, static_bits ? static_rows : 1, (float)random_amount,
+                        random_amount > 0.0 ? chipmunk_next_random_salt() : 0u};
+    p.counts = counts, p.lengths = lengths, p.pad_n = pad_n, p.multiple_of = multiple_of;
+    launch_topk_mask_packed<false>(p, (hipStream_t)stream);
     CM_LAUNCH_CHECK();
     return CHIPMUNK_OK;
 }
diff --git a/chipmunk_amd/csrc/torch_registry.cpp b/chipmunk_amd/csrc/torch_registry.cpp
--- a/chipmunk_amd/csrc/torch_registry.cpp
+++ b/chipmunk_amd/csrc/torch_registry.cpp
@@ -666,6 +666,19 @@
     return {indices, counts};
 }
 
+static std::vector<at::Tensor> ragged_rows_from_counts(const at::Tensor &mask, bool packed, bool sorted, const at::Tensor &counts,
+                                                       const at::Tensor &len, int64_t rows, int64_t n, int64_t multiple_of) {
+    at::Tensor offsets = at::zeros({rows + 1}, len.options());
+    if (rows) offsets.narrow(0, 1, rows).copy_(len.cumsum(0));
+    const int64_t total = rows ? offsets[rows].item<int64_t>() : 0;
+    at::Tensor flat = at::empty({total + 64}, counts.options());
+    flat.narrow(0, total, 64).zero_();
+    check(chipmunk_mask_to_ragged_indices(mask.data_ptr(), packed ? 1 : 0, sorted ? 1 : 0, offsets.data_ptr<int64_t>(), flat.data_ptr<int>(),
+                                          rows, (int)n, (int)multiple_of, cur_stream(mask)),
+          "mask_to_ragged_indices");
+    return {flat, offsets, counts};
+}
+
 std::vector<at::Tensor> mask_to_ragged_indices(at::Tensor mask, at::IntArrayRef shape, int64_t multiple_of, int64_t pad_to_multiple_of,
                                                bool sorted) {
     CHECK_DEV(mask);
@@ -685,15 +698,25 @@
     check(chipmunk_mask_row_counts(mask.data_ptr(), packed ? 1 : 0, counts.data_ptr<int>(), len.data_ptr<int64_t>(), rows, (int)n,
                                    (int)pad_n, (int)multiple_of, cur_stream(mask)),
           "mask_to_ragged_indices");
-    at::Tensor offsets = at::zeros({rows + 1}, len.options());
-    if (rows) offsets.narrow(0, 1, rows).copy_(len.cumsum(0));
-    const int64_t total = rows ? offsets[rows].item<int64_t>() : 0;
-    at::Tensor flat = at::empty({total + 64}, counts.options());
-    flat.narrow(0, total, 64).zero_();
-    check(chipmunk_mask_to_ragged_indices(mask.data_ptr(), packed ? 1 : 0, sorted ? 1 : 0, offsets.data_ptr<int64_t>(), flat.data_ptr<int>(),
-                                          rows, (int)n, (int)multiple_of, cur_stream(mask)),
-          "mask_to_ragged_indices");
-    return {flat, offsets, counts};
+    return ragged_rows_from_counts(mask, packed, sorted, counts, len, rows, n, multiple_of);
+}
+
+std::vector<at::Tensor> mask_to_ragged_indices_counted(at::Tensor mask, at::IntArrayRef shape, at::Tensor counts, at::Tensor len,
+                                                       int64_t multiple_of, bool sorted) {
+    CHECK_DEV(mask); CHECK_DEV(counts); CHECK_DEV(len);
+    const bool packed = mask.scalar_type() == at::kByte;
+    TORCH_CHECK(packed || mask.scalar_type() == at::kBool, "mask must be bool, or uint8 bit-packed with a shape");
+    TORCH_CHECK(multiple_of > 0, "multiple_of must be positive");
+    mask = mask.contiguous();
+    std::vector<int64_t> shp = packed ? shape.vec() : mask.sizes().vec();
+    TORCH_CHECK(shp.size() == 4, "shape must be [b, h, m, n]");
+    const int64_t rows = shp[0] * shp[1] * shp[2], n = shp[3];
+    if (packed) TORCH_CHECK(n % 8 == 0 && mask.numel() * 8 >= rows * n, "bad packed mask");
+    TORCH_CHECK(n > 0 && n <= INT_MAX, "rows must have between 1 and 2^31 - 1 columns");
+    TORCH_CHECK(counts.scalar_type() == at::kInt && counts.numel() == rows && counts.is_contiguous() && len.scalar_type() == at::kLong &&
+                len.numel() == rows && len.is_contiguous(), "counts must be int32 and len int64, one entry per mask row");
+    c10::DeviceGuard guard(mask.device());
+    return ragged_rows_from_counts(mask, packed, sorted, counts, len, rows, n, multiple_of);
 }
 
 std::vector<at::Tensor> dense_colsum_attn_layout(at::Tensor q, at::Tensor k, at::Tensor v, at::Tensor p, bool token_major_o);
@@ -750,6 +773,68 @@
     return {ocl[0], topk_mask(cs, k_top, random_amount, groups, static_mask), ocl[2]};
 }
 
+std::vector<at::Tensor> dense_colsum_topk_packed(at::Tensor q, at::Tensor k, at::Tensor v, at::Tensor p, int64_t k_top, double random_amount,
+                                                 const c10::optional<at::Tensor> &groups, const c10::optional<at::Tensor> &static_bits,
+                                                 int64_t multiple_of, int64_t pad_to_multiple_of, bool token_major_o) {
+    CHECK_DEV(q); CHECK_DEV(k); CHECK_DEV(v); CHECK_DEV(p);
+    CHECK_BF16(q); CHECK_BF16(k); CHECK_BF16(v);
+    TORCH_CHECK(q.dim() == 4 && k.dim() == 4 && v.dim() == 4, "q, k, v must be [B, H, N, 128]");
+    const int64_t B = q.size(0), H = q.size(1), Nq = q.size(2), Nk = k.size(2), G = (Nq + 191) / 192, rows = B * H * G;
+    TORCH_CHECK(Nk % 8 == 0, "dense_colsum_topk_packed: the key count must be a multiple of 8 for a packed mask (got ", Nk, ")");
+    TORCH_CHECK(multiple_of > 0 && pad_to_multiple_of > 0 && k_top >= 0, "multiple_of and pad_to_multiple_of must be positive, k_top >= 0");
+    const int64_t pad_n = ((Nk + pad_to_multiple_of - 1) / pad_to_multiple_of) * pad_to_multiple_of;
+    TORCH_CHECK(pad_n <= INT_MAX && rows <= INT_MAX, "too many columns or rows");
+    const void *st = nullptr, *gf = nullptr;
+    int64_t st_stride = 0, st_rows = 1;
+    at::Tensor stc, gfc;
+    if (static_bits.has_value() && static_bits->defined()) {
+        stc = *static_bits;
+        CHECK_DEV(stc);
+        TORCH_CHECK(stc.scalar_type() == at::kByte && stc.dim() == 2 && stc.size(1) == Nk / 8 && stc.stride(1) == 1 &&
+                    (stc.size(0) == G || stc.size(0) == H * G || stc.size(0) == rows), "static_bits must be uint8 [G | H*G | B*H*G, Nk / 8] bit-packed rows");
+        st = stc.data_ptr(), st_stride = stc.stride(0), st_rows = stc.size(0);
+    }
+    if (groups.has_value() && groups->defined()) {
+        gfc = *groups;
+        CHECK_DEV(gfc);
+        TORCH_CHECK(gfc.scalar_type() == at::kBool && gfc.dim() == 4 && gfc.size(3) == 1 && gfc.size(2) == G &&
+                    gfc.size(1) == H && (gfc.size(0) == 1 || gfc.size(0) == B), "groups must be bool [1|B, H, G, 1]");
+        gfc = gfc.expand({B, H, G, 1}).contiguous();
+        gf = gfc.data_ptr();
+    }
+    c10::DeviceGuard guard(q.device());
+    at::Tensor packed = at::empty({rows * Nk / 8}, q.options().dtype(at::kByte));
+    at::Tensor counts = at::empty({B, H, G}, q.options().dtype(at::kInt));
+    at::Tensor len = at::empty({rows}, q.options().dtype(at::kLong));
+    const bool shapes_ok = q.size(3) == 128 && q.stride(3) == 1 && k.stride(3) == 1 && v.stride(3) == 1 && p.scalar_type() == at::kFloat &&
+                           p.is_contiguous() && p.numel() == B * H * Nq;
+    if (shapes_ok) {
+        at::Tensor o = alloc_o(q, q, token_major_o);
+        const int64_t os[3] = {o.stride(0), o.stride(1), o.stride(2)};
+        at::Tensor l = at::empty({B, H, Nq, 1}, q.options().dtype(at::kFloat));
+        const int64_t qs[3] = {q.stride(0), q.stride(1), q.stride(2)}, ks[3] = {k.stride(0), k.stride(1), k.stride(2)},
+                      vs[3] = {v.stride(0), v.stride(1), v.stride(2)};
+        const int rc = chipmunk_dense_colsum_topk_packed_strided(q.data_ptr(), k.data_ptr(), v.data_ptr(), qs, ks, vs, p.data_ptr<float>(),
+                                                                 o.data_ptr(), os, l.data_ptr<float>(), (int)B, (int)H, (int)Nq, (int)Nk, st,
+                                                                 st_stride, (int)st_rows, gf, packed.data_ptr(), counts.data_ptr<int>(),
+                                                                 len.data_ptr<int64_t>(), (int)k_top, (int)pad_n, (int)multiple_of,
+                                                                 random_amount, cur_stream(q));
+        if (rc == CHIPMUNK_OK) return {o, packed, l, counts, len};
+        if (rc != CHIPMUNK_ERR_UNSUPPORTED) check(rc, "dense_colsum_topk_packed");
+    }
+    auto ocl = dense_colsum_attn_layout(q, k, v, p, token_major_o);
+    at::Tensor cs = ocl[1];
+    if (cs.size(-1) != Nk || cs.size(-2) != G) cs = cs.slice(-2, 0, G).slice(-1, 0, Nk);
+    if (!(cs.stride(3) == 1 && cs.stride(2) % 4 == 0 && cs.stride(1) == G * cs.stride(2) && (B == 1 || cs.stride(0) == H * cs.stride(1)) &&
+          ((uintptr_t)cs.data_ptr() & 7) == 0))
+        cs = cs.contiguous();
+    check(chipmunk_topk_mask_packed(cs.data_ptr(), cs.stride(2), st, st_stride, (int)st_rows, gf, packed.data_ptr(), counts.data_ptr<int>(),
+                                    len.data_ptr<int64_t>(), (int)rows, (int)Nk, (int)k_top, (int)pad_n, (int)multiple_of, random_amount,
+                                    cur_stream(q)),
+          "dense_colsum_topk_packed");
+    return {ocl[0], packed, ocl[2], counts, len};
+}
+
 at::Tensor topk_mask(at::Tensor cs, int64_t k, double random_amount, const c10::optional<at::Tensor> &groups,
                      const c10::optional<at::Tensor> &static_mask) {
     CHECK_DEV(cs); CHECK_BF16(cs);
@@ -934,6 +1019,8 @@
     m.def("dense_colsum_attn_layout(Tensor q, Tensor k, Tensor v, Tensor p, bool token_major_o) -> Tensor[]");
     m.def("compact_indices(Tensor indices, Tensor counts) -> Tensor[]");
     m.def("mask_to_ragged_indices(Tensor mask, int[] shape, int multiple_of, int pad_to_multiple_of, bool sorted) -> Tensor[]");
+    m.def("mask_to_ragged_indices_counted(Tensor mask, int[] shape, Tensor counts, Tensor len, int multiple_of, bool sorted) -> Tensor[]");
+    m.def("dense_colsum_topk_packed(Tensor q, Tensor k, Tensor v, Tensor p, int k_top, float random_amount, Tensor? groups, Tensor? static_bits, int multiple_of, int pad_to_multiple_of, bool token_major_o=False) -> Tensor[]");
     m.def("csp_attn_out_ragged(Tensor q, Tensor k, Tensor v, Tensor o_in, Tensor indices, Tensor offsets, Tensor indices_counts, int o_scale) -> Tensor");
     m.def("residual_ln_modulate(Tensor x, Tensor? y, Tensor? gate, Tensor shift, Tensor scale, float eps) -> Tensor[]");
     m.def("transpose_last2(Tensor x) -> Tensor");
@@ -975,6 +1062,8 @@
     m.impl("packed_mask_to_indices", &packed_mask_to_indices);
     m.impl("mask_to_sorted_indices", &mask_to_sorted_indices);
     m.impl("mask_to_ragged_indices", &mask_to_ragged_indices);
+    m.impl("mask_to_ragged_indices_counted", &mask_to_ragged_indices_counted);
+    m.impl("dense_colsum_topk_packed", &dense_colsum_topk_packed);
     m.impl("topk_mask", &topk_mask);
     m.impl("transpose_last2", &transpose_last2);
     m.impl("transpose_last2_pitched", &transpose_last2_pitched);
diff --git a/chipmunk_amd/modules/attn.py b/chipmunk_amd/modules/attn.py
--- a/chipmunk_amd/modules/attn.py
+++ b/chipmunk_amd/modules/attn.py
@@ -15,6 +15,7 @@
 
 singleton_static_mask: Optional[Tensor] = None
 singleton_video_query_groups: Optional[Tensor] = None
+singleton_static_bits: Optional[Tuple[Tensor, Tensor]] = None
 
 
 def _cdiv(a: int, b: int) -> int:
@@ -50,11 +51,15 @@
             for qg in range(n_video // 192):
                 centre = qg * 192 + 96
                 mask[qg, max(0, centre - window // 2):min(n_video, centre + window // 2)] = True
+        bits = None
+        if mask.is_cuda and mask.shape[-1] % 8 == 0:
+            bits = ops.bitpack(mask)[0].view(mask.shape[0], mask.shape[-1] // 8)
         mask = mask[None, None, :, :].expand(1, local_heads_num, -1, -1).contiguous()
         sparse_groups = (mask.sum(dim=-1, keepdim=True) + topk) < (n_video + txt_len)
-        global singleton_static_mask, singleton_video_query_groups
+        global singleton_static_mask, singleton_video_query_groups, singleton_static_bits
         singleton_static_mask = mask
         singleton_video_query_groups = sparse_groups
+        singleton_static_bits = None if bits is None else (mask, bits)
 
     def _static(self, heads: int, qg: int, n: int):
         g0 = self.query_group_offset
@@ -63,6 +68,14 @@
             "(local_heads_num): build the static mask for the largest head chunk")
         h = min(heads, singleton_static_mask.shape[1])
         return (singleton_static_mask[:, :h, g0:g0 + qg, :n], singleton_video_query_groups[:, :h, g0:g0 + qg, :])
+
+    def _static_bits(self, qg: int, n: int) -> Optional[Tensor]:
+        if singleton_static_bits is None or singleton_static_bits[0] is not singleton_static_mask or n % 8 != 0:
+            return None
+        bits, g0 = singleton_static_bits[1], self.query_group_offset
+        if g0 + qg > bits.shape[0] or n > bits.shape[1] * 8:
+            return None
+        return bits[g0:g0 + qg, :n // 8]
 
     def random_and_topk(self, cs: Tensor, topk: int) -> Tensor:
         cfg = GLOBAL_CONFIG["attn"]
@@ -178,11 +191,18 @@
             if inference_step == 1 or cfg["recompute_mask"]:
                 prev_lse = self.storage.get_lse_constants()
                 tk = int(multiple_of * round((cfg["top_keys"] * k.shape[-2]) / multiple_of))
-                mask = bs = None
+                mask = bs = packed_out = None
                 if (q.is_cuda and cfg["should_compress_indices"] and tk > 0 and amd_key("attn", "fused_colsum_topk")
                         and amd_key("attn", "fused_topk_mask") and k.shape[-2] <= ops.TOPK_MASK_MAX_N):
-                    static, groups = self._static(q.shape[1], _cdiv(q.shape[-2], bm), k.shape[-2])
-                    o, mask, lse = ops.dense_colsum_topk_mask(q, k, v, prev_lse, tk, 0.01, groups, static, tm)
+                    qg = _cdiv(q.shape[-2], bm)
+                    static, groups = self._static(q.shape[1], qg, k.shape[-2])
+                    bits = self._static_bits(qg, k.shape[-2]) if (use_ragged and amd_key("attn", "packed_topk_mask")) else None
+                    if bits is not None:
+                        o, packed, lse, counts, lengths = ops.dense_colsum_topk_mask(q, k, v, prev_lse, tk, 0.01, groups, bits, tm,
+                                                                                     (multiple_of, bm))
+                        packed_out = (packed, torch.Size((q.shape[0], q.shape[1], qg, k.shape[-2])), (counts, lengths))
+                    else:
+                        o, mask, lse = ops.dense_colsum_topk_mask(q, k, v, prev_lse, tk, 0.01, groups, static, tm)
                 elif do_padding:
                     o, bs, lse = ops.dense_colsum_attn(q, k, v, prev_lse, tm)
                 else:
@@ -190,7 +210,14 @@
                                   torch.ops.chipmunk.dense_colsum_attn(q, k, v, prev_lse))
                 lse[..., k.shape[-2]:, :] = 0
                 self.storage.set_lse_constants(lse)
-                if cfg["should_compress_indices"]:
+                if packed_out is not None:
+                    packed, mask_shape, counts_len = packed_out
+                    self.mask_shape[self.layer_counter.cur_model_invocation_per_step] = mask_shape
+                    self.storage.set_indices(packed)
+                    ragged = ops.mask_to_ragged_indices(packed, mask_shape, multiple_of, bm, bool(amd_key("attn", "sorted_indices")),
+                                                        counts_len=counts_len)
+                    self._remember_indices(None, ragged[2], ragged[:2])
+                elif cfg["should_compress_indices"]:
                     if mask is not None:
                         pass
                     elif tk > 0:
diff --git a/chipmunk_amd/ops/_fake.py b/chipmunk_amd/ops/_fake.py
--- a/chipmunk_amd/ops/_fake.py
+++ b/chipmunk_amd/ops/_fake.py
@@ -100,6 +100,15 @@
         return [_o_like(q, token_major_o), q.new_empty((B, H, G, k.shape[2]), dtype=torch.bool),
                 q.new_empty((B, H, Nq, 1), dtype=torch.float32)]
 
+    @lib.register_fake("chipmunk::dense_colsum_topk_packed")
+    def _(q, k, v, p, k_top, random_amount, groups, static_bits, multiple_of, pad_to_multiple_of, token_major_o=False):
+        B, H, Nq, D = q.shape
+        G = (Nq + 191) // 192
+        return [_o_like(q, token_major_o), q.new_empty((B * H * G * k.shape[2] // 8,), dtype=torch.uint8),
+                q.new_empty((B, H, Nq, 1), dtype=torch.float32), q.new_empty((B, H, G), dtype=torch.int32),
+                q.new_empty((B * H * G,), dtype=torch.int64)]
+
+
     @lib.register_fake("chipmunk::qkv_split_norm")
     def _(qkv, q_weight, k_weight, heads, eps, freqs_cos=None, freqs_sin=None):
         out = qkv.new_empty((3, 1, heads, qkv.shape[0], 128))
diff --git a/chipmunk_amd/ops/attn.py b/chipmunk_amd/ops/attn.py
--- a/chipmunk_amd/ops/attn.py
+++ b/chipmunk_amd/ops/attn.py
@@ -1,6 +1,6 @@
 from __future__ import annotations
 
-from typing import Tuple
+from typing import Optional, Tuple
 
 import torch
 import torch.nn.functional as F
@@ -47,10 +47,17 @@
 
 
 def dense_colsum_topk_mask(q: torch.Tensor, k: torch.Tensor, v: torch.Tensor, p: torch.Tensor, k_top: int, random_amount: float,
-                           groups, static_mask, token_major_o: bool = False) -> Tuple[torch.Tensor, torch.Tensor, torch.Tensor]:
+                           groups, static_mask, token_major_o: bool = False, packed_counts: Optional[Tuple[int, int]] = None):
     n = q.shape[-2]
     padded = _pad_len(n)
     assert p.shape[-2] in (n, padded), "p must be the l vector of the previous full step"
+    if packed_counts is not None:
+        o, packed, l, counts, length = torch.ops.chipmunk.dense_colsum_topk_packed(
+            _last_dim_contiguous(q), _last_dim_contiguous(k), _last_dim_contiguous(v), p[..., :n, :].contiguous(), k_top, random_amount,
+            groups, static_mask, packed_counts[0], packed_counts[1], token_major_o)
+        if padded != n:
+            l = F.pad(l, (0, 0, 0, padded - n))
+        return o, packed, l, counts, length
     o, mask, l = torch.ops.chipmunk.dense_colsum_topk_mask(_last_dim_contiguous(q), _last_dim_contiguous(k), _last_dim_contiguous(v),
                                                            p[..., :n, :].contiguous(), k_top, random_amount, groups, static_mask,
                                                            token_major_o)
diff --git a/chipmunk_amd/ops/indexed_io.py b/chipmunk_amd/ops/indexed_io.py
--- a/chipmunk_amd/ops/indexed_io.py
+++ b/chipmunk_amd/ops/indexed_io.py
@@ -40,7 +40,9 @@
 
 
 def mask_to_ragged_indices(mask: torch.Tensor, shape: Sequence[int], multiple_of: int, pad_to_multiple_of: int,
-                           sorted: bool = True) -> List[torch.Tensor]:
+                           sorted: bool = True, counts_len=None) -> List[torch.Tensor]:
+    if mask.is_cuda and counts_len is not None:
+        return torch.ops.chipmunk.mask_to_ragged_indices_counted(mask, list(shape), counts_len[0], counts_len[1], multiple_of, sorted)
     if mask.is_cuda:
         return torch.ops.chipmunk.mask_to_ragged_indices(mask, list(shape), multiple_of, pad_to_multiple_of, sorted)
     if mask.dtype == torch.uint8:
diff --git a/chipmunk_amd/util/config.py b/chipmunk_amd/util/config.py
--- a/chipmunk_amd/util/config.py
+++ b/chipmunk_amd/util/config.py
@@ -81,6 +81,7 @@
     "attn.keep_unpacked_indices_offloaded": True,
     "attn.kept_indices_offloaded_budget_gb": 8.0,
     "attn.ragged_mask_to_indices": True,
+    "attn.packed_topk_mask": True,
 }
 BASE_CONFIG["offloading"]["keep_resident_if_fits"] = AMD_EXTRA_KEYS["offloading.keep_resident_if_fits"]
 BASE_CONFIG["offloading"]["hbm_budget_gb"] = AMD_EXTRA_KEYS["offloading.hbm_budget_gb"]
@@ -97,6 +98,7 @@
 BASE_CONFIG["attn"]["keep_unpacked_indices_offloaded"] = AMD_EXTRA_KEYS["attn.keep_unpacked_indices_offloaded"]
 BASE_CONFIG["attn"]["kept_indices_offloaded_budget_gb"] = AMD_EXTRA_KEYS["attn.kept_indices_offloaded_budget_gb"]
 BASE_CONFIG["attn"]["ragged_mask_to_indices"] = AMD_EXTRA_KEYS["attn.ragged_mask_to_indices"]
+BASE_CONFIG["attn"]["packed_topk_mask"] = AMD_EXTRA_KEYS["attn.packed_topk_mask"]
 
 GLOBAL_CONFIG: Dict[str, Any] = copy.deepcopy(BASE_CONFIG)
 
diff --git a/include/chipmunk_hip.h b/include/chipmunk_hip.h
--- a/include/chipmunk_hip.h
+++ b/include/chipmunk_hip.h
@@ -137,6 +137,16 @@
                        int static_rows, const void *group_flags, void *mask, int rows, int n, int k,
                        double random_amount, void *stream);
 
+int chipmunk_topk_mask_packed(const void *cs, int64_t cs_stride, const void *static_bits, int64_t static_stride, int static_rows,
+                              const void *group_flags, void *packed, int32_t *counts, int64_t *lengths, int rows, int n, int k,
+                              int pad_n, int multiple_of, double random_amount, void *stream);
+int chipmunk_dense_colsum_topk_packed_strided(const void *q, const void *k, const void *v, const int64_t q_strides[3],
+                                              const int64_t k_strides[3], const int64_t v_strides[3], const float *p, void *o,
+                                              const int64_t *o_strides, float *l, int B, int H, int Nq, int Nk,
+                                              const void *static_bits, int64_t static_stride, int static_rows,
+                                              const void *group_flags, void *packed, int32_t *counts, int64_t *lengths, int k_top,
+                                              int pad_n, int multiple_of, double random_amount, void *stream);
+
 int chipmunk_mask_to_indices(const void *mask, int32_t *indices, int32_t *counts, int64_t rows, int n, int pad_n,
                              int multiple_of, void *stream);
 
```

Result: no change. 0.5756, median of 2 (-0.1%).
